# Whisper-6/DynamicTreeAttn

Measured on AMD Instinct MI355X. Metric: tree-attn fwd+bwd tokens/sec, Qwen3-0.6B tau2-16k tries, higher is better.
Workload: dtype bf16

## Files before the change

### dynamictreeattn_amd/_lib.py

```python
from __future__ import annotations

import ctypes as C
import os

from .build import LIB

_lib = None
_i32, _i64, _f32, _vp = C.c_int32, C.c_int64, C.c_float, C.c_void_p

_PROTOS = {
    "dta_version": ([], C.c_int),
    "dta_take_pending_error": ([C.c_char_p, _i32], C.c_int),
    "dta_lcp_adjacent": ([_vp, _vp, _vp, _i32, _vp, _vp, _vp], C.c_int),
    "dta_leafize": ([_vp, _vp, _i32, _vp, _vp, _vp, _vp, _vp], C.c_int),
    "dta_preorder_meta": ([_vp] * 8 + [_i32, _i32] + [_vp] * 4 + [_vp], C.c_int),
    "dta_tree_attn_fwd": ([_vp] * 8 + [_i32] * 6 + [_i64] * 8 + [_f32, _i32] + [_vp, _i32, _f32, _vp], C.c_int),
    "dta_tree_attn_bwd": ([_vp] * 14 + [_i32] * 6 + [_i64] * 12 + [_f32, _i32, _i32, _i32] + [_vp, _i32, _vp, _i32, _vp]
                          + [_vp, _i32, _f32, _vp], C.c_int),
    "dta_window_lo": ([_vp] * 4 + [_i32, _i32, _i32, _vp, _vp], C.c_int),
    "dta_logprob_entropy_fwd": ([_vp] * 8 + [_i32, _i32, _i64, _f32, _i32, _f32, _vp], C.c_int),
    "dta_logprob_entropy_shard_stats": ([_vp] * 6 + [_i32, _i32, _i64, _f32, _i32, _f32, _vp], C.c_int),
    "dta_logprob_entropy_bwd": ([_vp] * 10 + [_i32, _i32, _i64, _i64, _f32, _i32, _f32, _vp], C.c_int),
    "dta_rmsnorm_fwd": ([_vp] * 6 + [_i32, _i32, _f32, _f32, _i32, _vp], C.c_int),
    "dta_rmsnorm_bwd_blocks": ([_i32], C.c_int),
    "dta_rmsnorm_bwd": ([_vp] * 7 + [_i32, _i32, _f32, _i32, _vp], C.c_int),
    "dta_layernorm_fwd": ([_vp] * 8 + [_i32, _i32, _f32, _i32, _vp], C.c_int),
    "dta_layernorm_bwd_blocks": ([_i32], C.c_int),
    "dta_layernorm_bwd": ([_vp] * 8 + [_i32, _i32, _i32, _vp], C.c_int),
    "dta_qk_norm_rope_fwd": ([_vp] * 5 + [_i32, _i32, _i32, _i64, _f32, _i32, _vp], C.c_int),
    "dta_qk_norm_rope_bwd_blocks": ([_i64], C.c_int),
    "dta_qk_norm_rope_bwd": ([_vp] * 7 + [_i32, _i32, _i32, _i64, _i64, _i64, _i64, _i32, _vp], C.c_int),
    "dta_rope_partial_fwd": ([_vp] * 3 + [_i32] * 5 + [_i64, _i32, _vp], C.c_int),
    "dta_rope_partial_bwd": ([_vp] * 3 + [_i32] * 5 + [_i64, _i64, _i64, _i32, _vp], C.c_int),
    "dta_wide_qk_norm_rope_fwd": ([_vp] * 5 + [_i32, _i32, _i32, _i64, _f32, _i32, _vp], C.c_int),
    "dta_wide_qk_norm_rope_bwd_blocks": ([_i32], C.c_int),
    "dta_wide_qk_norm_rope_bwd": ([_vp] * 7 + [_i32, _i32, _i32, _i64, _i64, _i64, _i64, _i32, _vp], C.c_int),
    "dta_rmsnorm_add_fwd": ([_vp] * 6 + [_i32, _i32, _f32, _i32, _vp], C.c_int),
    "dta_swiglu_fwd": ([_vp] * 3 + [_i64, _i32, _i64, _i32, _vp], C.c_int),
    "dta_swiglu_bwd": ([_vp] * 5 + [_i64, _i32, _i64, _i64, _i32, _vp], C.c_int),
    "dta_geglu_fwd": ([_vp] * 3 + [_i64, _i32, _i64, _i32, _vp], C.c_int),
    "dta_geglu_bwd": ([_vp] * 5 + [_i64, _i32, _i64, _i64, _i32, _vp], C.c_int),
    "dta_transpose": ([_vp, _vp, _i64, _i64, _i64, _i64, _i32, _vp], C.c_int),
    "dta_sum_slabs": ([_vp, _i64, _i64, _i64, _vp, _vp, _i32, _vp], C.c_int),
    "dta_moe_router_fwd": ([_vp] * 4 + [_i32] * 5 + [_vp], C.c_int),
    "dta_moe_router_bwd": ([_vp] * 5 + [_i32] * 5 + [_vp], C.c_int),
    "dta_moe_permute_workspace": ([_i32, _i32], C.c_int),
    "dta_moe_tile_bound": ([_i32, _i32], C.c_int),
    "dta_moe_permute": ([_vp, _i32, _i32, _i32] + [_vp] * 5 + [_vp], C.c_int),
    "dta_moe_grouped_gemm": ([_i32] + [_vp] * 7 + [_i32] * 5 + [_vp], C.c_int),
    "dta_moe_combine_fwd": ([_vp] * 4 + [_i32] * 4 + [_vp], C.c_int),
    "dta_moe_combine_bwd": ([_vp] * 6 + [_i32] * 4 + [_vp], C.c_int),
    "dta_lora_down": ([_vp, _i64, _vp, _i64, _vp, _i64, _vp, _i32, _i32, _i32, _i32, _vp], C.c_int),
    "dta_lora_wgrad_slabs": ([_i32, _i32], C.c_int),
    "dta_lora_wgrad": ([_vp, _i64, _vp, _i64, _vp, _vp, _i32, _i32, _i32, _i32, _vp], C.c_int),
    "dta_policy_loss_blocks": ([_i32], C.c_int),
    "dta_policy_loss": ([_vp] * 10 + [_i32] + [_vp] * 5 + [_i32, _i32] + [_f32] * 4 + [_i32, _f32, _i32, _f32, _vp], C.c_int),
    "dta_policy_loss_seq_blocks": ([_i32, _i32], C.c_int),
    "dta_policy_loss_seq": ([_vp] * 14 + [_i32] + [_vp] * 6 + [_i32] * 4 + [_f32] * 4 + [_i32, _f32, _i32, _f32, _vp], C.c_int),
    "dta_preference_loss_blocks": ([_i32, _i32, _i32], C.c_int),
    "dta_preference_loss": ([_vp] * 21 + [_i32] * 6 + [_f32] * 3 + [_i32, _i32, _f32, _f32, _vp], C.c_int),
}
EXPORTS = tuple(_PROTOS)
_ERR = {-1: "DTA_EINVAL", -2: "DTA_EUNSUPPORTED", -3: "DTA_EALIGN", -4: "DTA_ELAUNCH", -5: "DTA_EPRIOR"}


def _hip_runtimes_mapped():
    try:
        with open("/proc/self/maps") as f:
            return sorted({line.split()[-1] for line in f if "libamdhip64" in line})
    except OSError:
        return []


def lib():
    global _lib
    if _lib is None:
        if not os.path.exists(LIB):
            raise RuntimeError(f"{LIB} is missing: run `python -m dynamictreeattn_amd.build` (hipcc, gfx950). "
                               "There is no CPU fallback for the hot path.")
        import torch
        l = C.CDLL(LIB)
        rts = _hip_runtimes_mapped()
        if len(rts) > 1:
            raise RuntimeError("more than one libamdhip64 is mapped into this process: " + ", ".join(rts) +
                               " — libdta_mi355x.so must resolve to the HIP runtime torch ships")
        for name, (args, res) in _PROTOS.items():
            fn = getattr(l, name)
            fn.argtypes, fn.restype = args, res
        _lib = l
    return _lib


def check(status: int, what: str):
    if status == 0:
        return
    if status == -5:
        buf = C.create_string_buffer(256)
        code = lib().dta_take_pending_error(buf, 256)
        raise RuntimeError(f"{what}: not launched, a HIP error was already pending on this thread: {buf.value.decode() or code} "
                           f"(hipError {code}; now cleared — after an asynchronous kernel fault the GPU context stays unusable)")
    raise RuntimeError(f"{what} failed: {_ERR.get(status, status)}")


def ptr(t):
    return None if t is None else t.data_ptr()
```

### dynamictreeattn_amd/csrc/elementwise_kernels.hip

```cpp
#include <hip/hip_runtime.h>
#include <stdint.h>
#include "dta_common.h"
#include "dta_device.h"

#ifndef DTA_EW_NT
#define DTA_EW_NT 1
#endif
#if DTA_EW_NT
#define DTA_SAVED_LOAD(P) __builtin_nontemporal_load(P)
#else
#define DTA_SAVED_LOAD(P) (*(P))
#endif

namespace {


template <int DT, int NA, bool OFF = false>
__global__ __launch_bounds__(256) void rmsnorm_fwd_kernel(const void* __restrict__ x_, const void* __restrict__ delta_, const void* __restrict__ w_,
                                                          void* __restrict__ xout_, void* __restrict__ y_,
                                                          float* __restrict__ rstd, int R, int H, float eps, float w_off = 0.f) {
  using e = typename Ty<DT>::e; using v8 = typename Ty<DT>::v8;
  const int lane = threadIdx.x & 63, wave = threadIdx.x >> 6;
  const e* w = reinterpret_cast<const e*>(w_);
  const int nv = H >> 3;
// ... 491 lines not shown
}

template <int DT, int NA, int D, int WPT>
__global__ __launch_bounds__(256) void wide_qk_norm_rope_fwd_kernel(const void* __restrict__ x_, const void* __restrict__ w_, const float* __restrict__ cs,
                                                                    void* __restrict__ y_, float* __restrict__ rstd, int T, int n,
                                                                    int64_t x_st, float eps) {
  using e = typename Ty<DT>::e; using v8 = typename Ty<DT>::v8;
  constexpr int LPH = D / 8, L = 64 * WPT, TPB = 4 / WPT;
  __shared__ float slot[4];
  const int lane = WPT == 1 ? (threadIdx.x & 63) : threadIdx.x, sub = lane & (LPH - 1);
  const e* w = reinterpret_cast<const e*>(w_);
  const int nv = n >> 3;
  const int per_lane = (nv + L - 1) / L;
  for (int tok = blockIdx.x * TPB + (WPT == 1 ? (threadIdx.x >> 6) : 0); tok < T; tok += gridDim.x * TPB) {
    const e* x = reinterpret_cast<const e*>(x_) + (int64_t)tok * x_st;
    e* y = reinterpret_cast<e*>(y_) + (int64_t)tok * n;
    const float* c = cs + (int64_t)tok * D + 8 * (sub & (LPH / 2 - 1));
    float cj[8], sj[8];
#pragma unroll
    for (int j = 0; j < 8; ++j) { cj[j] = c[j]; sj[j] = sub < LPH / 2 ? -c[D / 2 + j] : c[D / 2 + j]; }
    v8 keep[NA];
    float ss = 0.f;
#pragma unroll
    for (int a = 0; a < NA; ++a) {
      const int i = lane + L * a;
      if (a < per_lane && i < nv) {
        const v8 v = *reinterpret_cast<const v8*>(x + 8 * i);
#pragma unroll
        for (int j = 0; j < 8; ++j) { const float f = (float)v[j]; ss = __builtin_fmaf(f, f, ss); }
        keep[a] = v;
      }
    }
    ss = token_sum<WPT>(ss, slot);
    const float r = __builtin_amdgcn_rsqf(ss / (float)n + eps);
    if (lane == 0) rstd[tok] = r;
#pragma unroll
    for (int a = 0; a < NA; ++a) {
      if (a < per_lane) {
        const int i = lane + L * a;
        const bool live = i < nv;
        float av[8];
        if (live) {
          const v8 wv = *reinterpret_cast<const v8*>(w + 8 * i);
#pragma unroll
          for (int j = 0; j < 8; ++j) av[j] = (float)(e)((float)wv[j] * ((float)keep[a][j] * r));
        } else {
#pragma unroll
          for (int j = 0; j < 8; ++j) av[j] = 0.f;
        }
        v8 o;
#pragma unroll
        for (int j = 0; j < 8; ++j) {
          const float other = __shfl_xor(av[j], LPH / 2);
          o[j] = (e)(av[j] * cj[j] + other * sj[j]);
        }
        if (live) *reinterpret_cast<v8*>(y + 8 * i) = o;
      }
    }
  }
}

template <int DT, int NA, int D, int WPT>
__global__ __launch_bounds__(256) void wide_qk_norm_rope_bwd_kernel(const void* __restrict__ x_, const void* __restrict__ w_, const float* __restrict__ cs,
                                                                    const void* dy_, const float* __restrict__ rstd, void* dx_,
                                                                    float* __restrict__ dw_part, int T, int n, int64_t x_st, int64_t dy_st_t,
                                                                    int64_t dy_st_h, int64_t dx_st) {
  using e = typename Ty<DT>::e; using v8 = typename Ty<DT>::v8;
  constexpr int LPH = D / 8, LSH = D == 128 ? 4 : 3, L = 64 * WPT, TPB = 4 / WPT;
  __shared__ float red[WPT == 1 ? 4 * 64 * 8 : 4];
  const int lane = WPT == 1 ? (threadIdx.x & 63) : threadIdx.x, wave = threadIdx.x >> 6, sub = lane & (LPH - 1);
  const e* w = reinterpret_cast<const e*>(w_);
  const int nv = n >> 3;
  const int per_lane = (nv + L - 1) / L;
  float acc[NA][8];
#pragma unroll
  for (int a = 0; a < NA; ++a)
#pragma unroll
    for (int j = 0; j < 8; ++j) acc[a][j] = 0.f;
  for (int tok = blockIdx.x * TPB + (WPT == 1 ? wave : 0); tok < T; tok += gridDim.x * TPB) {
    const e* x = reinterpret_cast<const e*>(x_) + (int64_t)tok * x_st;
    const e* dy = reinterpret_cast<const e*>(dy_) + (int64_t)tok * dy_st_t + 8 * sub;
    e* dx = reinterpret_cast<e*>(dx_) + (int64_t)tok * dx_st;
    const float* c = cs + (int64_t)tok * D + 8 * (sub & (LPH / 2 - 1));
    float cj[8], sj[8];
#pragma unroll
    for (int j = 0; j < 8; ++j) { cj[j] = c[j]; sj[j] = sub < LPH / 2 ? c[D / 2 + j] : -c[D / 2 + j]; }
    const float r = rstd[tok];
    float dot = 0.f;
    v8 kx[NA], kg[NA];
#pragma unroll
    for (int a = 0; a < NA; ++a) {
      if (a < per_lane) {
        const int i = lane + L * a;
        const bool live = i < nv;
        v8 v, g;
        if (live) { v = DTA_SAVED_LOAD(reinterpret_cast<const v8*>(x + 8 * i)); g = *reinterpret_cast<const v8*>(dy + (int64_t)(i >> LSH) * dy_st_h); }
        else {
#pragma unroll
          for (int j = 0; j < 8; ++j) { v[j] = (e)0.f; g[j] = (e)0.f; }
        }
        if (live) {
          const v8 wv = *reinterpret_cast<const v8*>(w + 8 * i);
#pragma unroll
          for (int j = 0; j < 8; ++j) {
            const float gj = (float)g[j];
            const float da = gj * cj[j] + __shfl_xor(gj, LPH / 2) * sj[j];
            const float t = (float)v[j] * r;
            dot = __builtin_fmaf(da * (float)wv[j], t, dot); acc[a][j] = __builtin_fmaf(da, t, acc[a][j]);
          }
        }
        kx[a] = v; kg[a] = g;
      }
    }
    dot = token_sum<WPT>(dot, red) / (float)n;
#pragma unroll
    for (int a = 0; a < NA; ++a) {
      if (a < per_lane) {
        const int i = lane + L * a;
        const bool live = i < nv;
        const v8 v = kx[a], g = kg[a];
        float da[8];
#pragma unroll
        for (int j = 0; j < 8; ++j) { const float gj = (float)g[j]; da[j] = gj * cj[j] + __shfl_xor(gj, LPH / 2) * sj[j]; }
        if (live) {
          const v8 wv = *reinterpret_cast<const v8*>(w + 8 * i);
          v8 o;
#pragma unroll
          for (int j = 0; j < 8; ++j) { const float t = (float)v[j] * r; o[j] = (e)(r * (da[j] * (float)wv[j] - t * dot)); }
          *reinterpret_cast<v8*>(dx + 8 * i) = o;
        }
      }
    }
  }
  if (!dw_part) return;
  float* out = dw_part + (int64_t)blockIdx.x * n;
  if constexpr (WPT == 4) {
#pragma unroll
    for (int a = 0; a < NA; ++a) {
      const int i = lane + L * a;
      if (a < per_lane && i < nv) {
#pragma unroll
        for (int j = 0; j < 8; ++j) out[8 * i + j] = acc[a][j];
      }
    }
  } else {
#pragma unroll
    for (int a = 0; a < NA; ++a) {
      if (a < per_lane) {
        __syncthreads();
#pragma unroll
        for (int j = 0; j < 8; ++j) red[(wave * 64 + lane) * 8 + j] = acc[a][j];
        __syncthreads();
        if (wave == 0) {
          const int i = lane + 64 * a;
          if (i < nv) {
#pragma unroll
            for (int j = 0; j < 8; ++j) out[8 * i + j] = red[lane * 8 + j] + red[(64 + lane) * 8 + j] + red[(128 + lane) * 8 + j] + red[(192 + lane) * 8 + j];
          }
        }
      }
    }
  }
}

template <int DT, int NA>
__global__ __launch_bounds__(256) void rmsnorm_add_fwd_kernel(const void* __restrict__ y_, const void* __restrict__ w_, const void* __restrict__ res_,
                                                              void* __restrict__ out_, void* __restrict__ yn_, float* __restrict__ rstd,
                                                              int R, int H, float eps) {
  using e = typename Ty<DT>::e; using v8 = typename Ty<DT>::v8;
  const int lane = threadIdx.x & 63, wave = threadIdx.x >> 6;
  const e* w = reinterpret_cast<const e*>(w_);
  const int nv = H >> 3;
  for (int row = blockIdx.x * 4 + wave; row < R; row += gridDim.x * 4) {
    const e* y = reinterpret_cast<const e*>(y_) + (int64_t)row * H;
    const e* res = reinterpret_cast<const e*>(res_) + (int64_t)row * H;
    e* out = reinterpret_cast<e*>(out_) + (int64_t)row * H;
    e* yn = yn_ ? reinterpret_cast<e*>(yn_) + (int64_t)row * H : nullptr;
    float ss = 0.f;
    auto finish = [&](int i, const v8& v, float r) {
      const v8 wv = *reinterpret_cast<const v8*>(w + 8 * i);
      const v8 rv = *reinterpret_cast<const v8*>(res + 8 * i);
      v8 n8, o;
#pragma unroll
      for (int j = 0; j < 8; ++j) { n8[j] = (e)((float)wv[j] * ((float)v[j] * r)); o[j] = (e)((float)rv[j] + (float)n8[j]); }
      if (yn) *reinterpret_cast<v8*>(yn + 8 * i) = n8;
      *reinterpret_cast<v8*>(out + 8 * i) = o;
    };
    if constexpr (NA > 0) {
      v8 keep[NA];
#pragma unroll
      for (int a = 0; a < NA; ++a) {
        const int i = lane + 64 * a;
        if (i < nv) {
          const v8 v = *reinterpret_cast<const v8*>(y + 8 * i);
#pragma unroll
          for (int j = 0; j < 8; ++j) { const float f = (float)v[j]; ss = __builtin_fmaf(f, f, ss); }
          keep[a] = v;
        }
      }
      ss = wave_sum(ss);
      const float r = __builtin_amdgcn_rsqf(ss / (float)H + eps);
      if (lane == 0) rstd[row] = r;
#pragma unroll
      for (int a = 0; a < NA; ++a) {
        const int i = lane + 64 * a;
        if (i < nv) finish(i, keep[a], r);
      }
    } else {
      for (int i = lane; i < nv; i += 64) {
        const v8 v = *reinterpret_cast<const v8*>(y + 8 * i);
#pragma unroll
        for (int j = 0; j < 8; ++j) { const float f = (float)v[j]; ss = __builtin_fmaf(f, f, ss); }
      }
      ss = wave_sum(ss);
      const float r = __builtin_amdgcn_rsqf(ss / (float)H + eps);
      if (lane == 0) rstd[row] = r;
      for (int i = lane; i < nv; i += 64) finish(i, *reinterpret_cast<const v8*>(y + 8 * i), r);
    }
  }
}

template <int DT>
__global__ __launch_bounds__(256) void swiglu_fwd_kernel(const void* __restrict__ g_, const void* __restrict__ u_, void* __restrict__ y_,
                                                         int64_t n8, int c8, int64_t ld) {
  using e = typename Ty<DT>::e; using v8 = typename Ty<DT>::v8;
  for (int64_t i = (int64_t)blockIdx.x * 256 + threadIdx.x; i < n8; i += (int64_t)gridDim.x * 256) {
    const int64_t row = i / c8; const int col = (int)(i - row * c8) * 8;
    const v8 g = *reinterpret_cast<const v8*>(reinterpret_cast<const e*>(g_) + row * ld + col);
    const v8 u = *reinterpret_cast<const v8*>(reinterpret_cast<const e*>(u_) + row * ld + col);
    v8 o;
#pragma unroll
    for (int j = 0; j < 8; ++j) { const float x = (float)g[j]; const e s = (e)(x / (1.f + __expf(-x))); o[j] = (e)((float)s * (float)u[j]); }
    reinterpret_cast<v8*>(y_)[i] = o;
  }
}

template <int DT>
__global__ __launch_bounds__(256) void swiglu_bwd_kernel(const void* __restrict__ g_, const void* __restrict__ u_, const void* __restrict__ dy_,
                                                         void* __restrict__ dg_, void* __restrict__ du_, int64_t n8, int c8, int64_t ld, int64_t ldg) {
  using e = typename Ty<DT>::e; using v8 = typename Ty<DT>::v8;
  for (int64_t i = (int64_t)blockIdx.x * 256 + threadIdx.x; i < n8; i += (int64_t)gridDim.x * 256) {
    const int64_t row = i / c8; const int col = (int)(i - row * c8) * 8;
    const v8 g = DTA_SAVED_LOAD(reinterpret_cast<const v8*>(reinterpret_cast<const e*>(g_) + row * ld + col));
    const v8 u = DTA_SAVED_LOAD(reinterpret_cast<const v8*>(reinterpret_cast<const e*>(u_) + row * ld + col));
    const v8 dy = reinterpret_cast<const v8*>(dy_)[i];
    v8 dg, du;
#pragma unroll
    for (int j = 0; j < 8; ++j) {
      const float x = (float)g[j], sg = 1.f / (1.f + __expf(-x)), d = (float)dy[j];
      du[j] = (e)(d * x * sg);
      dg[j] = (e)(d * (float)u[j] * sg * (1.f + x * (1.f - sg)));
    }
    *reinterpret_cast<v8*>(reinterpret_cast<e*>(dg_) + row * ldg + col) = dg;
    *reinterpret_cast<v8*>(reinterpret_cast<e*>(du_) + row * ldg + col) = du;
  }
}

__device__ __forceinline__ float gelu_gate(float x, float* dgelu) {
  constexpr float K0 = 0.7978845608028654f, K1 = 0.044715f;
  const float x2 = x * x;
  const float z2 = 2.f * K0 * x * __builtin_fmaf(K1, x2, 1.f);
  const float E = __expf(fminf(-z2, 80.f));
  const float s = 1.f / (1.f + E);
  if (dgelu) *dgelu = s + x * s * (E * s) * (2.f * K0 * __builtin_fmaf(3.f * K1, x2, 1.f));
  return x * s;
}

template <int DT>
__global__ __launch_bounds__(256) void geglu_fwd_kernel(const void* __restrict__ g_, const void* __restrict__ u_, void* __restrict__ y_,
                                                        int64_t n8, int c8, int64_t ld) {
  using e = typename Ty<DT>::e; using v8 = typename Ty<DT>::v8;
  for (int64_t i = (int64_t)blockIdx.x * 256 + threadIdx.x; i < n8; i += (int64_t)gridDim.x * 256) {
    const int64_t row = i / c8; const int col = (int)(i - row * c8) * 8;
    const v8 g = *reinterpret_cast<const v8*>(reinterpret_cast<const e*>(g_) + row * ld + col);
    const v8 u = *reinterpret_cast<const v8*>(reinterpret_cast<const e*>(u_) + row * ld + col);
    v8 o;
#pragma unroll
    for (int j = 0; j < 8; ++j) { const e s = (e)gelu_gate((float)g[j], nullptr); o[j] = (e)((float)s * (float)u[j]); }
    reinterpret_cast<v8*>(y_)[i] = o;
  }
}

template <int DT>
__global__ __launch_bounds__(256) void geglu_bwd_kernel(const void* __restrict__ g_, const void* __restrict__ u_, const void* __restrict__ dy_,
                                                        void* __restrict__ dg_, void* __restrict__ du_, int64_t n8, int c8, int64_t ld, int64_t ldg) {
  using e = typename Ty<DT>::e; using v8 = typename Ty<DT>::v8;
  for (int64_t i = (int64_t)blockIdx.x * 256 + threadIdx.x; i < n8; i += (int64_t)gridDim.x * 256) {
    const int64_t row = i / c8; const int col = (int)(i - row * c8) * 8;
    const v8 g = DTA_SAVED_LOAD(reinterpret_cast<const v8*>(reinterpret_cast<const e*>(g_) + row * ld + col));
    const v8 u = DTA_SAVED_LOAD(reinterpret_cast<const v8*>(reinterpret_cast<const e*>(u_) + row * ld + col));
    const v8 dy = reinterpret_cast<const v8*>(dy_)[i];
    v8 dg, du;
#pragma unroll
    for (int j = 0; j < 8; ++j) {
      float dgl; const float ge = gelu_gate((float)g[j], &dgl), d = (float)dy[j];
      du[j] = (e)(d * ge);
      dg[j] = (e)(d * (float)u[j] * dgl);
    }
    *reinterpret_cast<v8*>(reinterpret_cast<e*>(dg_) + row * ldg + col) = dg;
    *reinterpret_cast<v8*>(reinterpret_cast<e*>(du_) + row * ldg + col) = du;
  }
}

template <int ESZ>
__global__ __launch_bounds__(256) void transpose_kernel(const char* __restrict__ in, char* __restrict__ out, int64_t rows, int64_t cols, int64_t ld_in, int64_t ld_out) {
  constexpr int TS = 64;
  constexpr int WPR = ESZ == 2 ? TS / 2 : TS;
  constexpr int PITCH = WPR + 4;
  __shared__ __attribute__((aligned(16))) uint32_t tile[TS * PITCH];
  const int64_t r0 = (int64_t)blockIdx.y * TS, c0 = (int64_t)blockIdx.x * TS;
  const int tid = threadIdx.x;
  if (ESZ == 2) {
    const int rp = tid >> 3, ch = tid & 7, r = 2 * rp, c = 8 * ch;
    uint4 a = make_uint4(0, 0, 0, 0), b = make_uint4(0, 0, 0, 0);
    if (c0 + c < cols) {
      if (r0 + r < rows) a = *reinterpret_cast<const uint4*>(in + ((r0 + r) * ld_in + c0 + c) * 2);
      if (r0 + r + 1 < rows) b = *reinterpret_cast<const uint4*>(in + ((r0 + r + 1) * ld_in + c0 + c) * 2);
    }
    const uint32_t aw[4] = {a.x, a.y, a.z, a.w}, bw[4] = {b.x, b.y, b.z, b.w};
#pragma unroll
    for (int j = 0; j < 4; ++j) {
      tile[(c + 2 * j) * PITCH + rp] = (aw[j] & 0xffffu) | (bw[j] << 16);
      tile[(c + 2 * j + 1) * PITCH + rp] = (aw[j] >> 16) | (bw[j] & 0xffff0000u);
    }
    __syncthreads();
    for (int i = tid; i < TS * 8; i += 256) {
      const int oc = i >> 3, k = i & 7;
      if (c0 + oc < cols && r0 + 8 * k < rows)
        *reinterpret_cast<uint4*>(out + ((c0 + oc) * ld_out + r0 + 8 * k) * 2) = *reinterpret_cast<const uint4*>(&tile[oc * PITCH + 4 * k]);
    }
  } else {
    for (int i = tid; i < TS * 16; i += 256) {
      const int r = i >> 4, c = 4 * (i & 15);
      uint4 a = make_uint4(0, 0, 0, 0);
      if (r0 + r < rows && c0 + c < cols) a = *reinterpret_cast<const uint4*>(in + ((r0 + r) * ld_in + c0 + c) * 4);
      tile[(c + 0) * PITCH + r] = a.x; tile[(c + 1) * PITCH + r] = a.y; tile[(c + 2) * PITCH + r] = a.z; tile[(c + 3) * PITCH + r] = a.w;
    }
    __syncthreads();
    for (int i = tid; i < TS * 16; i += 256) {
      const int oc = i >> 4, k = i & 15;
      if (c0 + oc < cols && r0 + 4 * k < rows)
        *reinterpret_cast<uint4*>(out + ((c0 + oc) * ld_out + r0 + 4 * k) * 4) = *reinterpret_cast<const uint4*>(&tile[oc * PITCH + 4 * k]);
    }
  }
}

template <int DT>
__global__ __launch_bounds__(1024) void sum_slabs_tall_kernel(const float* __restrict__ part, int64_t slabs, int64_t n, int64_t stride,
                                                              const float* __restrict__ extra, void* __restrict__ out_) {
  using e = typename Ty<DT>::e;
  __shared__ float red[16 * 64];
  const int lane = threadIdx.x & 63, wave = threadIdx.x >> 6;
  const int64_t col = (int64_t)blockIdx.x * 64 + lane;
  float acc[8];
#pragma unroll
  for (int u = 0; u < 8; ++u) acc[u] = 0.f;
  if (col < n) {
    int64_t s = wave;
    for (; s + 16 * 7 < slabs; s += 16 * 8) {
#pragma unroll
      for (int u = 0; u < 8; ++u) acc[u] += part[(s + 16 * u) * stride + col];
    }
    for (; s < slabs; s += 16) acc[0] += part[s * stride + col];
  }
  red[wave * 64 + lane] = ((acc[0] + acc[1]) + (acc[2] + acc[3])) + ((acc[4] + acc[5]) + (acc[6] + acc[7]));
  __syncthreads();
  if (wave == 0 && col < n) {
    float t = extra ? extra[col] : 0.f;
#pragma unroll
    for (int w = 0; w < 16; ++w) t += red[w * 64 + lane];
    reinterpret_cast<e*>(out_)[col] = (e)t;
  }
}
template <int DT>
__global__ __launch_bounds__(256) void sum_slabs_flat_kernel(const float* __restrict__ part, int slabs, int64_t n4, int64_t stride,
                                                             const float* __restrict__ extra, void* __restrict__ out_) {
  using e = typename Ty<DT>::e;
  typedef float f4 __attribute__((ext_vector_type(4)));
  typedef e e4 __attribute__((ext_vector_type(4)));
  for (int64_t i = (int64_t)blockIdx.x * 256 + threadIdx.x; i < n4; i += (int64_t)gridDim.x * 256) {
    f4 t = extra ? *reinterpret_cast<const f4*>(extra + 4 * i) : f4{0.f, 0.f, 0.f, 0.f};
    for (int s2 = 0; s2 < slabs; ++s2) t += *reinterpret_cast<const f4*>(part + s2 * stride + 4 * i);
    e4 o;
#pragma unroll
    for (int j = 0; j < 4; ++j) o[j] = (e)t[j];
    *reinterpret_cast<e4*>(reinterpret_cast<e*>(out_) + 4 * i) = o;
  }
}

template <int N> using Int = std::integral_constant<int, N>;

template <int WIDE, class F> inline void rms_form(int H, float w_offset, F&& f) {
  auto by_h = [&](auto off) {
    if (H <= 1024) f(Int<2>{}, off);
    else if (H <= 2048) f(Int<4>{}, off);
    else if (H <= 4096) f(Int<8>{}, off);
    else f(Int<WIDE>{}, off);
  };
  if (w_offset != 0.f) by_h(std::true_type{}); else by_h(std::false_type{});
}

template <class F> inline void qk_form(int NH, int head_dim, F&& f) {
  if (head_dim == 64) { if (NH % 4 == 0) f(Int<4>{}, Int<64>{}); else f(Int<1>{}, Int<64>{}); }
  else if (NH % 4 == 0) f(Int<4>{}, Int<128>{}); else f(Int<1>{}, Int<128>{});
}

template <class F> inline void wide_qk_form(int64_t n, int head_dim, F&& f) {
  auto by_n = [&](auto d) {
    if (n <= 1024) f(Int<2>{}, d, Int<1>{});
    else if (n <= 2048) f(Int<4>{}, d, Int<1>{});
    else if (n <= 4096) f(Int<2>{}, d, Int<4>{});
    else f(Int<4>{}, d, Int<4>{});
  };
  if (head_dim == 64) by_n(Int<64>{}); else by_n(Int<128>{});
}

template <class K>
int glu_fwd(const void* gate, const void* up, void* y, int64_t rows, int32_t cols, int64_t ld, int32_t dtype, void* stream, K kernel_of) {
  if (!gate || !up || !y || rows <= 0 || cols <= 0 || ld < cols) return DTA_EINVAL;
  if (!row_dtype_ok(dtype) || cols % 8 || ld % 8) return DTA_EUNSUPPORTED;
  if (!aligned16(gate) || !aligned16(up) || !aligned16(y)) return DTA_EALIGN;
  DTA_REFUSE_IF_PRIOR_ERROR();
  const int64_t n8 = rows * (cols / 8);
  dta_storage_type(dtype, [&](auto dt) {
    hipLaunchKernelGGL(kernel_of(dt), dim3(row_blocks(n8, 256, 4096)), dim3(256), 0, static_cast<hipStream_t>(stream), gate, up, y, n8, cols / 8, ld);
  });
  return DTA_LAUNCH_STATUS();
}

template <class K>
int glu_bwd(const void* gate, const void* up, const void* dy, void* dgate, void* dup, int64_t rows, int32_t cols, int64_t ld, int64_t ld_grad,
            int32_t dtype, void* stream, K kernel_of) {
  if (!gate || !up || !dy || !dgate || !dup || rows <= 0 || cols <= 0 || ld < cols || ld_grad < cols) return DTA_EINVAL;
  if (!row_dtype_ok(dtype) || cols % 8 || ld % 8 || ld_grad % 8) return DTA_EUNSUPPORTED;
  if (!aligned16(gate) || !aligned16(up) || !aligned16(dy) || !aligned16(dgate) || !aligned16(dup)) return DTA_EALIGN;
  DTA_REFUSE_IF_PRIOR_ERROR();
  const int64_t n8 = rows * (cols / 8);
  dta_storage_type(dtype, [&](auto dt) {
    hipLaunchKernelGGL(kernel_of(dt), dim3(row_blocks(n8, 256, 4096)), dim3(256), 0, static_cast<hipStream_t>(stream), gate, up, dy, dgate, dup, n8,
                       cols / 8, ld, ld_grad);
  });
  return DTA_LAUNCH_STATUS();
}

}

extern "C" int dta_rmsnorm_fwd(const void* x, const void* delta, const void* w, void* x_out, void* y, float* rstd,
                               int32_t R, int32_t H, float eps, float w_offset, int32_t dtype, void* stream) {
  if (!x || !w || !y || !rstd || R <= 0 || H <= 0 || ((delta != nullptr) != (x_out != nullptr)) || w_offset != w_offset) return DTA_EINVAL;
  if (!row_dtype_ok(dtype) || H % 8) return DTA_EUNSUPPORTED;
  if (!aligned16(x) || !aligned16(w) || !aligned16(y) || (delta && (!aligned16(delta) || !aligned16(x_out)))) return DTA_EALIGN;
  hipStream_t st_ = static_cast<hipStream_t>(stream);
  DTA_REFUSE_IF_PRIOR_ERROR();
  const dim3 grid(row_blocks(R, 4, 8192)), block(256);
  rms_form<0>(H, w_offset, [&](auto na, auto off) {
    dta_storage_type(dtype, [&](auto dt) {
      hipLaunchKernelGGL((rmsnorm_fwd_kernel<decltype(dt)::value, decltype(na)::value, decltype(off)::value>), grid, block, 0, st_,
                         x, delta, w, x_out, y, rstd, R, H, eps, w_offset);
    });
  });
  return DTA_LAUNCH_STATUS();
}

extern "C" int dta_rmsnorm_bwd_blocks(int32_t R) { return row_blocks(R, 4, 2048); }
extern "C" int dta_rmsnorm_bwd(const void* x, const void* w, const void* dy, const void* dres, const float* rstd, void* dx, float* dw_partial,
                               int32_t R, int32_t H, float w_offset, int32_t dtype, void* stream) {
  if (!x || !w || !dy || !rstd || !dx || R <= 0 || H <= 0 || w_offset != w_offset) return DTA_EINVAL;
  if (!row_dtype_ok(dtype) || H % 8 || H > 8192) return DTA_EUNSUPPORTED;
  if (!aligned16(x) || !aligned16(w) || !aligned16(dy) || !aligned16(dx) || (dres && !aligned16(dres))) return DTA_EALIGN;
  hipStream_t st_ = static_cast<hipStream_t>(stream);
  DTA_REFUSE_IF_PRIOR_ERROR();
  const dim3 grid(row_blocks(R, 4, 2048)), block(256);
  rms_form<16>(H, w_offset, [&](auto na, auto off) {
    dta_storage_type(dtype, [&](auto dt) {
      hipLaunchKernelGGL((rmsnorm_bwd_kernel<decltype(dt)::value, decltype(na)::value, decltype(off)::value>), grid, block, 0, st_,
                         x, w, dy, dres, rstd, dx, dw_partial, R, H, w_offset);
    });
  });
  return DTA_LAUNCH_STATUS();
}

namespace {
template <class F> inline void ln_form(int H, F&& f) {
  if (H <= 1024) f(Int<2>{}); else if (H <= 2048) f(Int<4>{}); else if (H <= 4096) f(Int<8>{}); else f(Int<16>{});
}
}

extern "C" int dta_layernorm_fwd(const void* x, const void* delta_a, const void* delta_b, const void* w, void* x_out, void* y,
                                 float* mean, float* rstd, int32_t R, int32_t H, float eps, int32_t dtype, void* stream) {
  if (!x || !w || !y || !mean || !rstd || R <= 0 || H <= 0 || (delta_b && !delta_a) || ((delta_a != nullptr) != (x_out != nullptr)) || eps != eps)
    return DTA_EINVAL;
  if (!row_dtype_ok(dtype) || H % 8 || H > 8192) return DTA_EUNSUPPORTED;
  if (!aligned16(x) || !aligned16(w) || !aligned16(y) || (delta_a && (!aligned16(delta_a) || !aligned16(x_out))) || (delta_b && !aligned16(delta_b)))
    return DTA_EALIGN;
  hipStream_t st_ = static_cast<hipStream_t>(stream);
  DTA_REFUSE_IF_PRIOR_ERROR();
  const dim3 grid(row_blocks(R, 4, 8192)), block(256);
  ln_form(H, [&](auto na) {
    dta_storage_type(dtype, [&](auto dt) {
      hipLaunchKernelGGL((layernorm_fwd_kernel<decltype(dt)::value, decltype(na)::value>), grid, block, 0, st_,
                         x, delta_a, delta_b, w, x_out, y, mean, rstd, R, H, eps);
    });
  });
  return DTA_LAUNCH_STATUS();
}

extern "C" int dta_layernorm_bwd_blocks(int32_t R) { return row_blocks(R, 4, 2048); }
extern "C" int dta_layernorm_bwd(const void* x, const void* w, const void* dy, const void* dres, const float* mean, const float* rstd,
                                 void* dx, float* dw_partial, int32_t R, int32_t H, int32_t dtype, void* stream) {
  if (!x || !w || !dy || !mean || !rstd || !dx || R <= 0 || H <= 0) return DTA_EINVAL;
  if (!row_dtype_ok(dtype) || H % 8 || H > 8192) return DTA_EUNSUPPORTED;
  if (!aligned16(x) || !aligned16(w) || !aligned16(dy) || !aligned16(dx) || (dres && !aligned16(dres))) return DTA_EALIGN;
  hipStream_t st_ = static_cast<hipStream_t>(stream);
  DTA_REFUSE_IF_PRIOR_ERROR();
  const dim3 grid(row_blocks(R, 4, 2048)), block(256);
  ln_form(H, [&](auto na) {
    dta_storage_type(dtype, [&](auto dt) {
      hipLaunchKernelGGL((layernorm_bwd_kernel<decltype(dt)::value, decltype(na)::value>), grid, block, 0, st_,
                         x, w, dy, dres, mean, rstd, dx, dw_partial, R, H);
    });
  });
  return DTA_LAUNCH_STATUS();
}

extern "C" int dta_qk_norm_rope_fwd(const void* x, const void* w, const float* cos_sin, void* y, float* rstd,
                                    int32_t T, int32_t NH, int32_t head_dim, int64_t x_stride_t, float eps, int32_t dtype, void* stream) {
  if (!x || !cos_sin || !y || T <= 0 || NH <= 0 || (w && !rstd)) return DTA_EINVAL;
  if (!row_dtype_ok(dtype) || (head_dim != 128 && head_dim != 64)) return DTA_EUNSUPPORTED;
  if (!aligned16(x) || !aligned16(y) || (w && !aligned16(w)) || x_stride_t % 8) return DTA_EALIGN;
  hipStream_t st_ = static_cast<hipStream_t>(stream);
  DTA_REFUSE_IF_PRIOR_ERROR();
  qk_form(NH, head_dim, [&](auto hpl, auto d) {
    constexpr int HPL = decltype(hpl)::value, D = decltype(d)::value, UPB = 4 * (64 / (D / 8));
    const int64_t n = (int64_t)T * (NH / HPL);
    const dim3 grid((unsigned)((n + UPB - 1) / UPB)), block(256);
    dta_storage_type(dtype, [&](auto dt) {
      hipLaunchKernelGGL((qk_norm_rope_fwd_kernel<decltype(dt)::value, HPL, D>), grid, block, 0, st_, x, w, cos_sin, y, rstd, n, NH, x_stride_t, eps);
    });
  });
  return DTA_LAUNCH_STATUS();
}

extern "C" int dta_qk_norm_rope_bwd_blocks(int64_t n_heads_total) { return row_blocks(n_heads_total, 16, 1024); }
extern "C" int dta_qk_norm_rope_bwd(const void* x, const void* w, const float* cos_sin, const void* dy, const float* rstd,
                                    void* dx, float* dw_partial, int32_t T, int32_t NH, int32_t head_dim,
                                    int64_t x_stride_t, int64_t dy_stride_t, int64_t dy_stride_h, int64_t dx_stride_t, int32_t dtype, void* stream) {
  if (!cos_sin || !dy || !dx || T <= 0 || NH <= 0 || (w && (!x || !rstd))) return DTA_EINVAL;
  if (!row_dtype_ok(dtype) || (head_dim != 128 && head_dim != 64)) return DTA_EUNSUPPORTED;
  if (!aligned16(dy) || !aligned16(dx) || (w && (!aligned16(w) || !aligned16(x))) || x_stride_t % 8 || dy_stride_t % 8 || dy_stride_h % 8 || dx_stride_t % 8) return DTA_EALIGN;
  if (dx_stride_t < (int64_t)NH * head_dim) return DTA_EINVAL;
  hipStream_t st_ = static_cast<hipStream_t>(stream);
  DTA_REFUSE_IF_PRIOR_ERROR();
  const dim3 grid(row_blocks((int64_t)T * NH, 16, 1024)), block(256);
  qk_form(NH, head_dim, [&](auto hpl, auto d) {
    constexpr int HPL = decltype(hpl)::value, D = decltype(d)::value;
    const int64_t n = (int64_t)T * (NH / HPL);
    dta_storage_type(dtype, [&](auto dt) {
      hipLaunchKernelGGL((qk_norm_rope_bwd_kernel<decltype(dt)::value, HPL, D>), grid, block, 0, st_, x, w, cos_sin, dy, rstd, dx, dw_partial, n, NH,
                         x_stride_t, dy_stride_t, dy_stride_h, dx_stride_t);
    });
  });
  return DTA_LAUNCH_STATUS();
}

namespace {
int rope_partial(const void* in, const float* cos_sin, void* out, int32_t T, int32_t NH, int32_t head_dim, int32_t rotary_dim, int32_t pairing,
                 int64_t in_st_t, int64_t in_st_h, int64_t out_st_t, float sgn, int grid_cap, int32_t dtype, void* stream) {
  if (!in || !cos_sin || !out || T <= 0 || NH <= 0 || rotary_dim <= 0 || (pairing != 0 && pairing != 1)) return DTA_EINVAL;
  if (!row_dtype_ok(dtype) || (head_dim != 128 && head_dim != 64) || rotary_dim > head_dim || rotary_dim % (pairing == 0 ? 16 : 8)) return DTA_EUNSUPPORTED;
  if (!aligned16(in) || !aligned16(out) || !aligned16(cos_sin) || in_st_t % 8 || in_st_h % 8 || out_st_t % 8) return DTA_EALIGN;
  if (in_st_t < 0 || in_st_h < head_dim || out_st_t < (int64_t)NH * head_dim) return DTA_EINVAL;
  hipStream_t st_ = static_cast<hipStream_t>(stream);
  DTA_REFUSE_IF_PRIOR_ERROR();
  qk_form(NH, head_dim, [&](auto hpl, auto d) {
    constexpr int HPL = decltype(hpl)::value, D = decltype(d)::value, UPB = 4 * (64 / (D / 8));
    const int64_t n = (int64_t)T * (NH / HPL);
    const dim3 grid(grid_cap ? (unsigned)row_blocks((int64_t)T * NH, 16, grid_cap) : ceil_blocks(n, UPB)), block(256);
    auto launch = [&](auto dt, auto pair, auto one_pass) {
      hipLaunchKernelGGL((rope_partial_kernel<decltype(dt)::value, HPL, D, decltype(pair)::value, decltype(one_pass)::value>), grid, block, 0, st_,
                         in, cos_sin, out, n, NH, rotary_dim, in_st_t, in_st_h, out_st_t, sgn);
    };
    dta_storage_type(dtype, [&](auto dt) {
      if (grid_cap) { if (pairing == 0) launch(dt, Int<0>{}, std::false_type{}); else launch(dt, Int<1>{}, std::false_type{}); }
      else if (pairing == 0) launch(dt, Int<0>{}, std::true_type{}); else launch(dt, Int<1>{}, std::true_type{});
    });
  });
  return DTA_LAUNCH_STATUS();
}
}

extern "C" int dta_rope_partial_fwd(const void* x, const float* cos_sin, void* y, int32_t T, int32_t NH, int32_t head_dim, int32_t rotary_dim,
                                    int32_t pairing, int64_t x_stride_t, int32_t dtype, void* stream) {
  return rope_partial(x, cos_sin, y, T, NH, head_dim, rotary_dim, pairing, x_stride_t, head_dim, (int64_t)NH * head_dim, 1.f, 0, dtype, stream);
}

extern "C" int dta_rope_partial_bwd(const float* cos_sin, const void* dy, void* dx, int32_t T, int32_t NH, int32_t head_dim, int32_t rotary_dim,
                                    int32_t pairing, int64_t dy_stride_t, int64_t dy_stride_h, int64_t dx_stride_t, int32_t dtype, void* stream) {
  return rope_partial(dy, cos_sin, dx, T, NH, head_dim, rotary_dim, pairing, dy_stride_t, dy_stride_h, dx_stride_t, -1.f, 1024, dtype, stream);
}

extern "C" int dta_wide_qk_norm_rope_fwd(const void* x, const void* w, const float* cos_sin, void* y, float* rstd,
                                         int32_t T, int32_t NH, int32_t head_dim, int64_t x_stride_t, float eps, int32_t dtype, void* stream) {
  if (!x || !w || !cos_sin || !y || !rstd || T <= 0 || NH <= 0 || eps != eps) return DTA_EINVAL;
  if (!row_dtype_ok(dtype) || (head_dim != 128 && head_dim != 64) || (int64_t)NH * head_dim > 8192) return DTA_EUNSUPPORTED;
  if (!aligned16(x) || !aligned16(w) || !aligned16(y) || x_stride_t % 8) return DTA_EALIGN;
  const int n = NH * head_dim;
  if (x_stride_t < n) return DTA_EINVAL;
  hipStream_t st_ = static_cast<hipStream_t>(stream);
  DTA_REFUSE_IF_PRIOR_ERROR();
  const dim3 grid(row_blocks(T, 4, 8192)), block(256);
  wide_qk_form(n, head_dim, [&](auto na, auto d, auto wpt) {
    dta_storage_type(dtype, [&](auto dt) {
      hipLaunchKernelGGL((wide_qk_norm_rope_fwd_kernel<decltype(dt)::value, decltype(na)::value, decltype(d)::value, decltype(wpt)::value>), grid, block, 0, st_,
                         x, w, cos_sin, y, rstd, T, n, x_stride_t, eps);
    });
  });
  return DTA_LAUNCH_STATUS();
}

extern "C" int dta_wide_qk_norm_rope_bwd_blocks(int32_t T) { return row_blocks(T, 4, 2048); }
extern "C" int dta_wide_qk_norm_rope_bwd(const void* x, const void* w, const float* cos_sin, const void* dy, const float* rstd,
                                         void* dx, float* dw_partial, int32_t T, int32_t NH, int32_t head_dim,
                                         int64_t x_stride_t, int64_t dy_stride_t, int64_t dy_stride_h, int64_t dx_stride_t, int32_t dtype, void* stream) {
  if (!x || !w || !cos_sin || !dy || !rstd || !dx || T <= 0 || NH <= 0) return DTA_EINVAL;
  if (!row_dtype_ok(dtype) || (head_dim != 128 && head_dim != 64) || (int64_t)NH * head_dim > 8192) return DTA_EUNSUPPORTED;
  if (!aligned16(x) || !aligned16(w) || !aligned16(dy) || !aligned16(dx) || x_stride_t % 8 || dy_stride_t % 8 || dy_stride_h % 8 || dx_stride_t % 8)
    return DTA_EALIGN;
  const int n = NH * head_dim;
  if (x_stride_t < n || dx_stride_t < n) return DTA_EINVAL;
  hipStream_t st_ = static_cast<hipStream_t>(stream);
  DTA_REFUSE_IF_PRIOR_ERROR();
  const dim3 grid(row_blocks(T, 4, 2048)), block(256);
  wide_qk_form(n, head_dim, [&](auto na, auto d, auto wpt) {
    dta_storage_type(dtype, [&](auto dt) {
      hipLaunchKernelGGL((wide_qk_norm_rope_bwd_kernel<decltype(dt)::value, decltype(na)::value, decltype(d)::value, decltype(wpt)::value>), grid, block, 0, st_,
                         x, w, cos_sin, dy, rstd, dx, dw_partial, T, n, x_stride_t, dy_stride_t, dy_stride_h, dx_stride_t);
    });
  });
  return DTA_LAUNCH_STATUS();
}

extern "C" int dta_rmsnorm_add_fwd(const void* y, const void* w, const void* res, void* out, void* yn, float* rstd,
                                   int32_t R, int32_t H, float eps, int32_t dtype, void* stream) {
  if (!y || !w || !res || !out || !rstd || R <= 0 || H <= 0 || eps != eps) return DTA_EINVAL;
  if (!row_dtype_ok(dtype) || H % 8) return DTA_EUNSUPPORTED;
  if (!aligned16(y) || !aligned16(w) || !aligned16(res) || !aligned16(out) || (yn && !aligned16(yn))) return DTA_EALIGN;
  hipStream_t st_ = static_cast<hipStream_t>(stream);
  DTA_REFUSE_IF_PRIOR_ERROR();
  const dim3 grid(row_blocks(R, 4, 8192)), block(256);
  rms_form<0>(H, 0.f, [&](auto na, auto) {
    dta_storage_type(dtype, [&](auto dt) {
      hipLaunchKernelGGL((rmsnorm_add_fwd_kernel<decltype(dt)::value, decltype(na)::value>), grid, block, 0, st_, y, w, res, out, yn, rstd, R, H, eps);
    });
  });
  return DTA_LAUNCH_STATUS();
}

extern "C" int dta_swiglu_fwd(const void* gate, const void* up, void* y, int64_t rows, int32_t cols, int64_t ld, int32_t dtype, void* stream) {
  return glu_fwd(gate, up, y, rows, cols, ld, dtype, stream, [](auto dt) { return swiglu_fwd_kernel<decltype(dt)::value>; });
}
extern "C" int dta_geglu_fwd(const void* gate, const void* up, void* y, int64_t rows, int32_t cols, int64_t ld, int32_t dtype, void* stream) {
  return glu_fwd(gate, up, y, rows, cols, ld, dtype, stream, [](auto dt) { return geglu_fwd_kernel<decltype(dt)::value>; });
}
extern "C" int dta_geglu_bwd(const void* gate, const void* up, const void* dy, void* dgate, void* dup,
                             int64_t rows, int32_t cols, int64_t ld, int64_t ld_grad, int32_t dtype, void* stream) {
  return glu_bwd(gate, up, dy, dgate, dup, rows, cols, ld, ld_grad, dtype, stream, [](auto dt) { return geglu_bwd_kernel<decltype(dt)::value>; });
}
extern "C" int dta_swiglu_bwd(const void* gate, const void* up, const void* dy, void* dgate, void* dup,
                              int64_t rows, int32_t cols, int64_t ld, int64_t ld_grad, int32_t dtype, void* stream) {
  return glu_bwd(gate, up, dy, dgate, dup, rows, cols, ld, ld_grad, dtype, stream, [](auto dt) { return swiglu_bwd_kernel<decltype(dt)::value>; });
}

extern "C" int dta_transpose(const void* in, void* out, int64_t rows, int64_t cols, int64_t ld_in, int64_t ld_out, int32_t elem_size, void* stream) {
  if (!in || !out || rows <= 0 || cols <= 0 || ld_in < cols || ld_out < rows) return DTA_EINVAL;
  if (elem_size != 2 && elem_size != 4) return DTA_EUNSUPPORTED;
  const int V = 16 / elem_size;
  if (rows % V || cols % V || ld_in % V || ld_out % V) return DTA_EUNSUPPORTED;
  if (!aligned16(in) || !aligned16(out)) return DTA_EALIGN;
  hipStream_t st_ = static_cast<hipStream_t>(stream);
  DTA_REFUSE_IF_PRIOR_ERROR();
  const dim3 grid((unsigned)((cols + 63) / 64), (unsigned)((rows + 63) / 64)), block(256);
  if (grid.y > 65535) return DTA_EUNSUPPORTED;
  if (elem_size == 2) hipLaunchKernelGGL(transpose_kernel<2>, grid, block, 0, st_, (const char*)in, (char*)out, rows, cols, ld_in, ld_out);
  else hipLaunchKernelGGL(transpose_kernel<4>, grid, block, 0, st_, (const char*)in, (char*)out, rows, cols, ld_in, ld_out);
  return DTA_LAUNCH_STATUS();
}

extern "C" int dta_sum_slabs(const float* part, int64_t slabs, int64_t n, int64_t slab_stride, const float* extra, void* out, int32_t out_dtype,
                             void* stream) {
  if (!part || !out || slabs <= 0 || n <= 0 || slab_stride < n) return DTA_EINVAL;
  if (!row_dtype_ok(out_dtype)) return DTA_EUNSUPPORTED;
  hipStream_t st_ = static_cast<hipStream_t>(stream);
  DTA_REFUSE_IF_PRIOR_ERROR();
  const bool flat = slabs <= 16 && n % 4 == 0 && slab_stride % 4 == 0 && aligned16(part) && aligned16(out) && (!extra || aligned16(extra));
  if (flat) {
    const dim3 grid(row_blocks(n / 4, 256, 8192)), block(256);
    dta_storage_type(out_dtype, [&](auto dt) {
      hipLaunchKernelGGL(sum_slabs_flat_kernel<decltype(dt)::value>, grid, block, 0, st_, part, (int)slabs, n / 4, slab_stride, extra, out);
    });
  } else {
    if ((n + 63) / 64 > 0x7fffffff) return DTA_EUNSUPPORTED;
    const dim3 grid((unsigned)((n + 63) / 64)), block(1024);
    dta_storage_type(out_dtype, [&](auto dt) {
      hipLaunchKernelGGL(sum_slabs_tall_kernel<decltype(dt)::value>, grid, block, 0, st_, part, slabs, n, slab_stride, extra, out);
    });
  }
  return DTA_LAUNCH_STATUS();
}
```

### dynamictreeattn_amd/dense.py

```python
from __future__ import annotations

from typing import List

import torch

from . import ops
from .model import ensure_supported, final_softcap_of, head_weight, is_longrope, logit_scale_of, longrope_boundary, packed_hidden_states
from .tree_training_engine import packed_logprob_entropy


def _one(model, ids: torch.Tensor, want_entropy: bool, checkpoint_layers: bool):
    n = ids.numel()
    depth = torch.arange(n, device=ids.device, dtype=torch.int32)
    long = is_longrope(model.config) and n > longrope_boundary(model.config)
    h = packed_hidden_states(model, ids, depth, ops.stack_meta(0), checkpoint_layers, longrope_long=long)
    parent = depth.to(torch.long) - 1
    return packed_logprob_entropy(h, head_weight(model), ids, parent, want_entropy, softcap=final_softcap_of(model), logit_scale=logit_scale_of(model))


@torch.no_grad()
def forward(model, token_seqs: List[torch.LongTensor], use_tqdm: bool = False) -> List[torch.Tensor]:
    out = []
    ensure_supported(model)
    with ops.weight_cache():
        for ids in token_seqs:
            lp, _ = _one(model, ids.to(model.device), False, False)
            out.append(lp[1:])
    return out


def backward(model, token_seqs: List[torch.LongTensor], attachs, loss_fn, act_ckpt: bool = False, use_tqdm: bool = False) -> float:
    total = 0.0
    ensure_supported(model)
    with ops.weight_cache():
        for ids, att in zip(token_seqs, attachs):
            lp, ent = _one(model, ids.to(model.device), True, act_ckpt)
            loss = loss_fn(lp[1:], ent, att)
            loss.backward()
            total += loss.item()
    return total
```

### dynamictreeattn_amd/model.py

```python
from __future__ import annotations

import weakref
from types import SimpleNamespace

import torch
import torch.nn as nn
import torch.nn.functional as F

from . import lora, ops


class _Norm(nn.Module):
    def __init__(self, n):
        super().__init__()
        self.weight = nn.Parameter(torch.ones(n))


class _Lin(nn.Module):
    def __init__(self, i, o):
        super().__init__()
        self.weight = nn.Parameter(torch.empty(o, i))


class _Attn(nn.Module):
# ... 113 lines not shown
def is_phi3(config) -> bool:
    return getattr(config, "model_type", None) == "phi3"


def is_glm4(config) -> bool:
    return getattr(config, "model_type", None) == "glm4"


def _head_dim(c) -> int:
    return getattr(c, "head_dim", None) or c.hidden_size // c.num_attention_heads


def rotary_dim(config) -> int:
    rp = getattr(config, "rope_parameters", None) or getattr(config, "rope_scaling", None) or {}
    prf = rp.get("partial_rotary_factor") if isinstance(rp, dict) else None
    if prf is None:
        prf = getattr(config, "partial_rotary_factor", None)
    return int(_head_dim(config) * (1.0 if prf is None else float(prf)))


def rope_layer_types(c):
    if getattr(c, "model_type", None) != "olmo3":
        return None
    types = getattr(c, "layer_types", None)
    if not types:
        raise ValueError("config.layer_types is missing: an olmo3 configuration keeps its rope_parameters per layer type")
    return sorted(set(types))


def _rope_dict(c, layer_type=None) -> dict:
    rp = getattr(c, "rope_parameters", None) or getattr(c, "rope_scaling", None) or {}
    if not isinstance(rp, dict):
        raise ValueError(f"config.rope_parameters must be a dict, got {type(rp).__name__}")
    types = rope_layer_types(c)
    if types is not None:
        if sorted(map(str, rp)) != types or not all(isinstance(v, dict) for v in rp.values()):
            raise ValueError(f"config.rope_parameters of an olmo3 configuration must be nested per layer type with exactly the keys "
                             f"{', '.join(types)} (config.layer_types); got {', '.join(map(str, rp)) or 'nothing'}")
        if layer_type not in rp:
            raise ValueError(f"config.rope_parameters is nested per layer type ({', '.join(types)}): name one of them, got {layer_type!r}")
        rp = rp[layer_type]
    elif rp and all(isinstance(v, dict) for v in rp.values()):
        raise ValueError(f"config.rope_parameters is nested per layer type ({', '.join(map(str, rp))}): one RoPE table per model is supported")
    rp = dict(rp)
    rp["rope_type"] = rp.get("rope_type", rp.get("type")) or "default"
    if rp.get("rope_theta") is None:
        theta = getattr(c, "rope_theta", None)
        rp["rope_theta"] = 1e6 if theta is None else theta
    if getattr(c, "original_max_position_embeddings", None) is not None:
        rp["original_max_position_embeddings"] = c.original_max_position_embeddings
    return rp


_ROPE: dict = {}


def is_longrope(c) -> bool:
    return is_phi3(c) and _rope_dict(c)["rope_type"] == "longrope"


def longrope_boundary(c) -> int:
    return int(_rope_dict(c)["original_max_position_embeddings"])


def rope_of(c, layer_type=None, long=False):
    rp = _rope_dict(c, layer_type)
    D = rotary_dim(c) if is_phi3(c) or is_glm4(c) else _head_dim(c)
    max_pos = getattr(c, "max_position_embeddings", None)
    longrope = is_phi3(c) and rp["rope_type"] == "longrope"
    key = (D, max_pos, bool(long) and longrope, tuple(sorted((k, repr(v)) for k, v in rp.items())))
    hit = _ROPE.get(key)
    if hit is None:
        hit = _ROPE[key] = ops.longrope_inv_freq(D, rp, max_pos, bool(long)) if longrope else ops.rope_inv_freq(D, rp, max_pos)
    return hit


_SOFTCAP_SINK_FIELDS = ("attn_logit_softcapping", "final_logit_softcapping", "attn_softcap", "logit_softcap", "attention_sink",
                        "attention_sinks", "use_attention_sinks", "num_sink_tokens")


def is_gemma2(config) -> bool:
    return getattr(config, "model_type", None) == "gemma2"


def gemma2_arith(config):
    c = config
    return float(c.query_pre_attn_scalar) ** -0.5, float(getattr(c, "attn_logit_softcapping", None) or 0.0), \
        float(getattr(c, "final_logit_softcapping", None) or 0.0)


def final_softcap_of(model) -> float:
    return gemma2_arith(model.config)[2] if is_gemma2(model.config) else 0.0


def _check_gemma2(c) -> None:
    act = getattr(c, "hidden_activation", None)
    if act != "gelu_pytorch_tanh":
        raise ValueError(f"config.hidden_activation = {act!r} is not supported for gemma2: the MLP kernel computes gelu_pytorch_tanh(gate) * up")
    D = _head_dim(c)
    if D not in (64, 128):
        raise ValueError(f"config.head_dim = {D} is not supported: the attention kernels cover head_dim 64 and 128 (Gemma-2-27B; the 2B / 9B use 256)")
    qs = getattr(c, "query_pre_attn_scalar", None)
    if qs is None or not float(qs) > 0:
        raise ValueError(f"config.query_pre_attn_scalar = {qs!r} is not supported: gemma2 attention scales by query_pre_attn_scalar ** -0.5")
    for f in ("attn_logit_softcapping", "final_logit_softcapping"):
        v = getattr(c, f, None)
        if v is not None and not (0.0 <= float(v) < float("inf")):
            raise ValueError(f"config.{f} = {v!r} is not supported: a soft-cap is a finite number >= 0 (None or 0: no cap)")


def _check_olmo(c) -> None:
    D = _head_dim(c)
    if D not in (64, 128):
        raise ValueError(f"config.head_dim = {D} is not supported for {c.model_type}: the projection-wide q/k norm kernels cover head_dim 64 and 128")
    for f in ("num_attention_heads", "num_key_value_heads"):
        if getattr(c, f) * D > 8192:
            raise ValueError(f"config.{f} * head_dim = {getattr(c, f)} * {D} is not supported: the projection-wide q/k norm kernels hold "
                             f"one row of at most 8192 elements")


def _check_cohere(c) -> None:
    mt, D, H = c.model_type, _head_dim(c), c.hidden_size
    if D not in (64, 128):
        raise ValueError(f"config.head_dim = {D} is not supported for {mt}: the attention and RoPE kernels cover head_dim 64 and 128")
    if H % 8 or H > 8192:
        raise ValueError(f"config.hidden_size = {H} is not supported for {mt}: the LayerNorm kernel holds one row of a multiple of 8 and at "
                         f"most 8192 elements (Command-R+ and Command-A are wider)")
    if getattr(c, "use_qk_norm", False):
        raise ValueError(f"config.use_qk_norm = True is not supported for {mt} (Command-R+): there is no per-head LayerNorm kernel")
    ls = getattr(c, "logit_scale", None)
    if isinstance(ls, bool) or not isinstance(ls, (int, float)) or not 0.0 < float(ls) < float("inf"):
        raise ValueError(f"config.logit_scale = {ls!r} is not supported for {mt}: the head scales its logits by a finite number > 0")
    act = getattr(c, "hidden_act", None)
    if act != "silu":
        raise ValueError(f"config.hidden_act = {act!r} is not supported for {mt}: the MLP kernels compute silu(gate) * up")
    if mt == "cohere2":
        types = getattr(c, "layer_types", None)
        if not types or len(types) != c.num_hidden_layers:
            raise ValueError(f"config.layer_types has {len(types or [])} entries for {c.num_hidden_layers} layers: a cohere2 layer rotates "
                             f"(sliding_attention) or not (full_attention) by its type")
        for t in types:
            if t not in ("full_attention", "sliding_attention"):
                raise ValueError(f"config.layer_types entry {t!r} is not supported for cohere2 (full_attention / sliding_attention)")
        W = getattr(c, "sliding_window", None)
        if "sliding_attention" in types and not (isinstance(W, int) and not isinstance(W, bool) and W > 0):
            raise ValueError(f"config.sliding_window = {W!r} is not supported for cohere2: a sliding_attention layer needs its window")


def _check_partial_rope(c, training: bool) -> None:
    mt, D = c.model_type, _head_dim(c)
    if D not in (64, 128):
        raise ValueError(f"config.head_dim = {D} is not supported for {mt}: the attention and RoPE kernels cover head_dim 64 and 128"
                         + (" (Phi-3-mini and Phi-3.5-mini use 96)" if D == 96 else ""))
    R, step = rotary_dim(c), 16 if is_phi3(c) else 8
    if not 0 < R <= D or R % step:
        raise ValueError(f"config partial_rotary_factor gives a rotary dimension of {R} of head_dim {D}, which is not supported for {mt}: "
                         f"the {'half-split' if is_phi3(c) else 'interleaved'} RoPE kernel rotates a multiple of {step} elements, at most head_dim")
    rp = _rope_dict(c)
    if rp["rope_type"] == "longrope" and is_phi3(c):
        if rp.get("original_max_position_embeddings") is None:
            raise ValueError("config.original_max_position_embeddings is missing: longrope picks its factors by it")
        for f in ("short_factor", "long_factor"):
            v = rp.get(f)
            if not isinstance(v, (list, tuple)) or len(v) != R // 2:
                raise ValueError(f"config.rope_parameters[{f!r}] must be a list of {R // 2} numbers (rotary dimension {R}), got "
                                 f"{len(v) if isinstance(v, (list, tuple)) else v!r}")
    for f in ("resid_pdrop", "embd_pdrop"):
        if training and float(getattr(c, f, 0.0) or 0.0) > 0:
            raise ValueError(f"config.{f} = {getattr(c, f)} on a model in training mode is not supported (model.eval(), or set it to 0)")


def check_supported(config, training: bool = True) -> None:
    c = config
    gemma = is_gemma2(c)
    partial = is_phi3(c) or is_glm4(c)
    if partial:
        _check_partial_rope(c, training)
    if gemma:
        _check_gemma2(c)
    if getattr(c, "model_type", None) == "olmo":
        raise ValueError("config.model_type = 'olmo' (OLMo-1: LayerNorm without weights, clip_qkv) is not supported; olmo2 and olmo3 are")
    if is_olmo(c):
        _check_olmo(c)
    if is_cohere(c):
        _check_cohere(c)
    for lt in rope_layer_types(c) or [None]:
        rp = _rope_dict(c, lt)
        if rp["rope_type"] not in ops.ROPE_TYPES and not (is_phi3(c) and rp["rope_type"] == "longrope"):
            raise ValueError(f"config.rope_parameters['rope_type'] = {rp['rope_type']!r} is not supported ({' / '.join(ops.ROPE_TYPES)})")
        prf = rp.get("partial_rotary_factor", getattr(c, "partial_rotary_factor", None))
        if not partial and prf is not None and float(prf) != 1.0:
            raise ValueError(f"config partial_rotary_factor = {prf} is not supported: the rotary kernels rotate the whole head")
    act = getattr(c, "hidden_act", None)
    if not gemma and act is not None and act != "silu":
        raise ValueError(f"config.hidden_act = {act!r} is not supported: the MLP kernels compute silu(gate) * up")
    if training and float(getattr(c, "attention_dropout", 0.0) or 0.0) > 0:
        raise ValueError(f"config.attention_dropout = {c.attention_dropout} on a model in training mode is not supported (model.eval(), or set it to 0)")
    if float(getattr(c, "router_jitter_noise", 0.0) or 0.0) > 0:
        raise ValueError(f"config.router_jitter_noise = {c.router_jitter_noise} is not supported")
    for f in _SOFTCAP_SINK_FIELDS:
        if gemma and f in ("attn_logit_softcapping", "final_logit_softcapping"):
            continue
        if getattr(c, f, None):
            raise ValueError(f"config.{f} = {getattr(c, f)!r} is not supported: the attention kernels have neither soft-capping nor sinks")


_CHECKED = weakref.WeakKeyDictionary()


def _check_olmo_norms(model) -> None:
    c = model.config
    D = _head_dim(c)
    for l, layer in enumerate(model.model.layers):
        for name, heads in (("q_norm", c.num_attention_heads), ("k_norm", c.num_key_value_heads)):
            w = getattr(getattr(layer.self_attn, name, None), "weight", None)
            if w is None or w.numel() != heads * D:
                raise ValueError(f"model.layers.{l}.self_attn.{name}.weight has {None if w is None else w.numel()} elements: "
                                 f"{c.model_type} normalises the whole projection row of {heads} * {D}")


def ensure_supported(model) -> None:
    training = bool(getattr(model, "training", True))
    if hasattr(model, "named_modules"):
        lora.check_supported(model)
    if is_olmo(model.config) and hasattr(getattr(model, "model", None), "layers"):
        _check_olmo_norms(model)
    try:
        seen = _CHECKED.setdefault(model, set())
    except TypeError:
        return check_supported(model.config, training)
    if training not in seen:
        check_supported(model.config, training)
        seen.add(training)


def _cfg_of(model, longrope_long=False):
    c = model.config
    D = _head_dim(c)
    types = rope_layer_types(c)
    rope = (rope_of(c, long=True) if longrope_long else rope_of(c)) if types is None else [rope_of(c, t) for t in c.layer_types]
    eps = getattr(c, "layer_norm_eps", 1e-5) if is_cohere(c) else getattr(c, "rms_norm_eps", 1e-6)
    return c.num_attention_heads, c.num_key_value_heads, D, float(eps), rope


def _windows_of(model):
    c = model.config
    n = c.num_hidden_layers
    W = getattr(c, "sliding_window", None) or 0
    if getattr(c, "model_type", None) in ("mistral", "mixtral", "phi3"):
        return [int(W)] * n
    types = getattr(c, "layer_types", None)
    if types is not None:
        if len(types) != n:
            raise ValueError(f"config.layer_types has {len(types)} entries for {n} layers")
        bad = [t for t in types if t not in ("full_attention", "sliding_attention")]
        if bad:
            raise ValueError(f"unsupported attention layer type {bad[0]!r} (full_attention / sliding_attention)")
        sliding = [t == "sliding_attention" for t in types]
    else:
        first = getattr(c, "max_window_layers", n)
        sliding = [bool(getattr(c, "use_sliding_window", False)) and l >= (first if first is not None else n) for l in range(n)]
    return [int(W) if s_ else 0 for s_ in sliding]


def layer_metas(meta, windows, for_window=None):
    out, cache = [], {}
    for W in windows:
        if W <= 0 or meta is None:
            out.append(meta)
            continue
        if W not in cache:
            if for_window is not None:
                cache[W] = for_window(W)
            elif meta.subtree_end is None and meta.runs is None:
                cache[W] = ops.stack_meta(meta.q_offset, W)
            else:
                raise ValueError("a sliding-window layer needs its windowed meta (ops.window_meta); none was given")
        out.append(cache[W])
    return out


def _bias(*mods):
    bs = [getattr(m_, "bias", None) for m_ in mods]
    if bs[0] is None:
        return None
    return bs[0] if len(bs) == 1 else torch.cat(bs)


def _project(x, *mods):
    bases, ads = zip(*(lora.resolve(m_) for m_ in mods))
    w = bases[0].weight if len(bases) == 1 else ops.stack_rows(*(b_.weight for b_ in bases))
    bias = _bias(*bases)
    if not any(a_ is not None for a_ in ads):
        return ops.linear(x, w, bias)
    adapters, n0 = [], 0
    for b_, a_ in zip(bases, ads):
        n = b_.weight.shape[0]
        if a_ is not None:
            adapters.append((n0, n, *a_))
        n0 += n
    return ops.lora_linear(x, w, bias, adapters)


def _gemma2_layer_forward(layer, res, delta, cos_sin, attn, Hq, Hkv, D, eps):
    T = res.shape[0]
    a, m = layer.self_attn, layer.mlp
    res, h = ops.add_rms_norm(res, delta, layer.input_layernorm.weight, eps, 1.0)
    qkv = _project(h, a.q_proj, a.k_proj, a.v_proj).view(T, Hq + 2 * Hkv, D)
    q, k, v = ops.qkv_prep(qkv, None, None, cos_sin, eps, Hq, Hkv)
    o = attn(q, k, v)
    delta = ops.rms_norm(_project(o.reshape(T, Hq * D), a.o_proj), layer.post_attention_layernorm.weight, eps, 1.0)
    res, h = ops.add_rms_norm(res, delta, layer.pre_feedforward_layernorm.weight, eps, 1.0)
    act = ops.geglu_fused(_project(h, m.gate_proj, m.up_proj))
    return res, ops.rms_norm(_project(act, m.down_proj), layer.post_feedforward_layernorm.weight, eps, 1.0)


def _olmo_layer_forward(layer, res, delta, cos_sin, attn, Hq, Hkv, D, eps):
    T = res.shape[0]
    a, m = layer.self_attn, layer.mlp
    x = res if delta is None else res + delta
    qkv = _project(x, a.q_proj, a.k_proj, a.v_proj).view(T, Hq + 2 * Hkv, D)
    q, k, v = ops.qkv_prep_wide(qkv, a.q_norm.weight, a.k_norm.weight, cos_sin, eps, Hq, Hkv)
    o = attn(q, k, v)
    h = ops.rms_norm_add(x, _project(o.reshape(T, Hq * D), a.o_proj), layer.post_attention_layernorm.weight, eps)
    act = ops.swiglu_fused(_project(h, m.gate_proj, m.up_proj))
    return ops.rms_norm_add(h, _project(act, m.down_proj), layer.post_feedforward_layernorm.weight, eps), None


def _phi3_layer_forward(layer, res, delta, cos_sin, attn, Hq, Hkv, D, eps):
    T = res.shape[0]
    a, m = layer.self_attn, layer.mlp
    res, h = ops.add_rms_norm(res, delta, layer.input_layernorm.weight, eps)
    qkv = _project(h, a.qkv_proj).view(T, Hq + 2 * Hkv, D)
    if cos_sin.shape[1] < D:
        q, k, v = ops.qkv_prep_partial(qkv, cos_sin, Hq, Hkv, False)
    else:
        q, k, v = ops.qkv_prep(qkv, None, None, cos_sin, eps, Hq, Hkv)
    o = attn(q, k, v)
    res, h = ops.add_rms_norm(res, _project(o.reshape(T, Hq * D), a.o_proj), layer.post_attention_layernorm.weight, eps)
    act = ops.swiglu_fused(_project(h, m.gate_up_proj))
    return res, _project(act, m.down_proj)


def _glm4_layer_forward(layer, res, delta, cos_sin, attn, Hq, Hkv, D, eps):
    T = res.shape[0]
    a, m = layer.self_attn, layer.mlp
    res, h = ops.add_rms_norm(res, delta, layer.input_layernorm.weight, eps)
    qkv = _project(h, a.q_proj, a.k_proj, a.v_proj).view(T, Hq + 2 * Hkv, D)
    q, k, v = ops.qkv_prep_partial(qkv, cos_sin, Hq, Hkv, True)
    o = attn(q, k, v)
    delta = ops.rms_norm(_project(o.reshape(T, Hq * D), a.o_proj), layer.post_self_attn_layernorm.weight, eps)
    res, h = ops.add_rms_norm(res, delta, layer.post_attention_layernorm.weight, eps)
    act = ops.swiglu_fused(_project(h, m.gate_up_proj))
    return res, ops.rms_norm(_project(act, m.down_proj), layer.post_mlp_layernorm.weight, eps)


def _cohere_layer_forward(layer, res, delta_a, delta_b, cos_sin, attn, Hq, Hkv, D, eps):
    T = res.shape[0]
    a, m = layer.self_attn, layer.mlp
    res, h = ops.add_layer_norm(res, delta_a, delta_b, layer.input_layernorm.weight, eps)
    qkv = _project(h, a.q_proj, a.k_proj, a.v_proj).view(T, Hq + 2 * Hkv, D)
    q, k, v = ops.qkv_prep_nope(qkv, Hq, Hkv) if cos_sin is None else ops.qkv_prep_partial(qkv, cos_sin, Hq, Hkv, True)
    o = attn(q, k, v)
    act = ops.swiglu_fused(_project(h, m.gate_proj, m.up_proj))
    return res, _project(o.reshape(T, Hq * D), a.o_proj), _project(act, m.down_proj)


def _layer_forward(layer, res, delta, cos_sin, attn, Hq, Hkv, D, eps):
    T = res.shape[0]
    a = layer.self_attn
    res, h = ops.add_rms_norm(res, delta, layer.input_layernorm.weight, eps)
    qkv = _project(h, a.q_proj, a.k_proj, a.v_proj).view(T, Hq + 2 * Hkv, D)
    qn = getattr(a, "q_norm", None); kn = getattr(a, "k_norm", None)
    q, k, v = ops.qkv_prep(qkv, qn.weight if qn is not None else None, kn.weight if kn is not None else None, cos_sin, eps, Hq, Hkv)
    o = attn(q, k, v)
    attn_out = _project(o.reshape(T, Hq * D), a.o_proj)
    res, h = ops.add_rms_norm(res, attn_out, layer.post_attention_layernorm.weight, eps)
    m = layer.mlp
    if hasattr(m, "experts") and hasattr(m, "gate"):
        g = m.gate
        norm = getattr(g, "norm_topk_prob", None)
        if norm is None:
            if not hasattr(m, "jitter_noise"):
                raise AttributeError(f"{type(g).__name__} has no norm_topk_prob and {type(m).__name__} is not a Mixtral block")
            norm = True
        return res, ops.moe_mlp(h, g.weight, m.experts.gate_up_proj, m.experts.down_proj, g.top_k, norm)
    act = ops.swiglu_fused(_project(h, m.gate_proj, m.up_proj))
    return res, _project(act, m.down_proj)


class _ScaleRows(torch.autograd.Function):

    @staticmethod
    def forward(ctx, x, s):
        ctx.s = float(torch.tensor(s, dtype=x.dtype))
        return x * ctx.s

    @staticmethod
    def backward(ctx, g):
        return g * ctx.s, None


def attn_args_of(model):
    if not is_gemma2(model.config):
        return {}
    scale, cap, _ = gemma2_arith(model.config)
    return {"scale": scale, "softcap": cap}


class _LayerRecompute(torch.autograd.Function):

    @staticmethod
    def forward(ctx, fn, keep_attn, res, *deltas):
        ctx.fn, ctx.has_delta = fn, tuple(d is not None for d in deltas)
        items = []
        with torch.no_grad():
            if keep_attn:
                with ops.AttentionTape("record", items):
                    out = fn(res, *deltas)
            else:
                out = fn(res, *deltas)
        ctx.items = items
        ctx.save_for_backward(res, *(d for d in deltas if d is not None))
        return out

    @staticmethod
    def backward(ctx, g_res, *g_deltas):
        res, *kept = ctx.saved_tensors
        r = res.detach().requires_grad_(True)
        kept = iter(kept)
        ds = [next(kept).detach().requires_grad_(True) if has else None for has in ctx.has_delta]
        with torch.enable_grad():
            if ctx.items:
                with ops.AttentionTape("replay", ctx.items):
                    outs = ctx.fn(r, *ds)
            else:
                outs = ctx.fn(r, *ds)
        ctx.items = None
        live = [(o, g) for o, g in zip(outs, (g_res, *g_deltas)) if o is not None]
        torch.autograd.backward(tuple(o for o, _ in live), tuple(g for _, g in live))
        return (None, None, r.grad, *(d.grad if d is not None else None for d in ds))


def packed_hidden_states(model, tokens: torch.Tensor, depth: torch.Tensor, meta, checkpoint_layers: bool = False,
                         attn_keep_bytes: int = 0, attn_of_layer=None, full_layers=0, kept_out=None, embed=None,
                         meta_for_window=None, longrope_long: bool = False) -> torch.Tensor:
    Hq, Hkv, D, eps, rope = _cfg_of(model, longrope_long)
    metas = layer_metas(meta, _windows_of(model), meta_for_window) if attn_of_layer is None else None
    body = model.model
    gemma = is_gemma2(model.config)
    cohere = is_cohere(model.config)
    layer_fwd = (_gemma2_layer_forward if gemma else _olmo_layer_forward if is_olmo(model.config) else _phi3_layer_forward if is_phi3(model.config)
                 else _glm4_layer_forward if is_glm4(model.config) else _cohere_layer_forward if cohere else _layer_forward)
    R = rotary_dim(model.config) if is_phi3(model.config) or is_glm4(model.config) else D
    akw = attn_args_of(model)
    res = embed(tokens) if embed is not None else F.embedding(tokens, body.embed_tokens.weight)
    deltas = (None, None) if cohere else (None,)
    if gemma:
        res = _ScaleRows.apply(res, float(model.config.hidden_size) ** 0.5)
    if isinstance(rope, list):
        tables = {id(r_): ops.rope_cos_sin(depth, D, r_) for r_ in {id(r_): r_ for r_ in rope}.values()}
        cos_sins = [tables[id(r_)] for r_ in rope]
    else:
        cos_sins = [ops.rope_cos_sin(depth, R, rope)] * len(body.layers)
    if cohere and model.config.model_type == "cohere2":
        cos_sins = [cs if t == "sliding_attention" else None for cs, t in zip(cos_sins, model.config.layer_types)]
    per_layer = tokens.shape[0] * Hq * (D * res.element_size() + 4)
    n_full = full_layers if isinstance(full_layers, int) else 1
    for li, layer in enumerate(body.layers):
        cos_sin = cos_sins[li]
        attn = attn_of_layer(li) if attn_of_layer is not None else (lambda m_: lambda q, k, v: ops.tree_attention(q, k, v, m_, **akw))(metas[li])
        if li == 0 and callable(full_layers) and checkpoint_layers and torch.is_grad_enabled() and res.is_cuda:
            m0 = torch.cuda.memory_allocated(res.device)
            res, *deltas = layer_fwd(layer, res, *deltas, cos_sin, attn, Hq, Hkv, D, eps)
            n_full = int(full_layers(torch.cuda.memory_allocated(res.device) - m0))
            continue
        if checkpoint_layers and li >= n_full and torch.is_grad_enabled() and (res.requires_grad or any(d is not None and d.requires_grad for d in deltas)):
            keep = attn_of_layer is None and attn_keep_bytes >= per_layer
            if keep:
                attn_keep_bytes -= per_layer
            fn = (lambda layer_, attn_, cs_: lambda r_, *d_: layer_fwd(layer_, r_, *d_, cs_, attn_, Hq, Hkv, D, eps))(layer, attn, cos_sin)
            res, *deltas = _LayerRecompute.apply(fn, keep, res, *deltas)
        else:
            res, *deltas = layer_fwd(layer, res, *deltas, cos_sin, attn, Hq, Hkv, D, eps)
    if kept_out is not None:
        kept_out.append(n_full if checkpoint_layers else len(body.layers))
    if cohere:
        return ops.add_layer_norm(res, *deltas, body.norm.weight, eps)[1]
    return ops.add_rms_norm(res, deltas[0], body.norm.weight, eps, *((1.0,) if gemma else ()))[1]


def head_weight(model) -> torch.Tensor:
    lm = getattr(model, "lm_head", None)
    return lm.weight if lm is not None else model.model.embed_tokens.weight
```

### dynamictreeattn_amd/ops.py

```python
from __future__ import annotations

import math
from dataclasses import dataclass
from typing import Optional

import numpy as np
import torch
import torch.nn.functional as F

from . import packing
from ._lib import check, lib, ptr

_DT = {torch.bfloat16: 0, torch.float16: 1, torch.float32: 2}


class _on:
    __slots__ = ("dev", "_guard")

    def __init__(self, *ts):
        dev = None
        for t in ts:
            if t is None:
                continue
            if not t.is_cuda:
# ... 110 lines not shown
    (qs, qh), (ks, kh), (vs, vh), (os_, oh) = _strides(q), _strides(k), _strides(v), _strides(out)
    _launch("dta_tree_attn_fwd", (q, k, v, meta.subtree_end, meta.runs, meta.win_lo),
            ptr(q), ptr(k), ptr(v), ptr(out), ptr(lse), ptr(meta.subtree_end), ptr(meta.run_ptr), ptr(meta.runs),
            Tq, Tk, meta.q_offset, Hq, Hkv, D, qs, qh, ks, kh, vs, vh, os_, oh, float(scale), _DT[q.dtype],
            ptr(meta.win_lo) if meta.window > 0 else None, int(meta.window), softcap, span="fwd")
    return out, lse, k, v


def attn_bwd_raw(q, k, v, out, dout, lse, meta: TreeAttnMeta, scale: float, dk=None, dv=None, accumulate=False, dq=None, softcap: float = 0.0):
    softcap = _cap_of(softcap)
    Tq, Hq, D = q.shape
    Tk, Hkv, _ = k.shape
    if dout.stride() != out.stride():
        dout = dout.contiguous(); out = out.contiguous()
    if dq is None:
        dq = torch.empty((Tq, Hq, D), dtype=q.dtype, device=q.device)
    if dk is None:
        dk = torch.empty((Tk, Hkv, D), dtype=q.dtype, device=q.device); dv = torch.empty_like(dk)
    delta = torch.empty((Hq, Tq), dtype=torch.float32, device=q.device)
    (qs, qh), (ks, kh), (vs, vh), (os_, oh), (dqs, dqh), (dks, dkh) = _strides(q), _strides(k), _strides(v), _strides(out), _strides(dq), _strides(dk)
    units, splits = meta.dkv_units, meta.dkv_splits
    n_units = units.shape[0] if units is not None else 0
    n_splits = splits.shape[0] if splits is not None else 0
    if q.dtype == torch.float32:
        units = splits = None; n_units = n_splits = 0
    ws = torch.empty((meta.n_slabs, Hkv, 2, packing.KTILE, D), dtype=torch.float32, device=q.device) if (units is not None and meta.n_slabs) else None

    def launch(which, span=None):
        _launch("dta_tree_attn_bwd", (q, k, v, out, dout, lse, dk, dv, meta.subtree_end, units, meta.win_lo),
                ptr(q), ptr(k), ptr(v), ptr(out), ptr(dout), ptr(lse), ptr(delta), ptr(dq), ptr(dk), ptr(dv),
                ptr(meta.subtree_end), ptr(meta.run_ptr), ptr(meta.runs), ptr(meta.ktile_qend),
                Tq, Tk, meta.q_offset, Hq, Hkv, D, qs, qh, ks, kh, vs, vh, os_, oh, dqs, dqh, dks, dkh,
                float(scale), _DT[q.dtype], int(accumulate), which,
                ptr(units), n_units, ptr(splits) if n_splits else None, n_splits, ptr(ws),
                ptr(meta.win_lo) if meta.window > 0 else None, int(meta.window), softcap, span=span)
    if KernelTimer.active is None:
        launch(3)
    else:
        launch(1, "bwd_dq"); launch(2 | 8, "bwd_dkv")
        if n_splits:
            launch(4, "bwd_dkv_finalize")
    return dq, dk, dv


class AttentionTape:
    current = None

    def __init__(self, mode: str, items=None):
        assert mode in ("record", "replay")
        self.mode, self.items, self.pos = mode, ([] if items is None else items), 0

    def __enter__(self):
        self._prev, AttentionTape.current = AttentionTape.current, self
        return self

    def __exit__(self, *exc):
        AttentionTape.current = self._prev
        return False


class _TreeAttention(torch.autograd.Function):
    @staticmethod
    def forward(ctx, q, k, v, meta: TreeAttnMeta, scale: float, softcap: float = 0.0):
        tape = AttentionTape.current
        if tape is not None and tape.mode == "replay" and tape.pos < len(tape.items):
            out, lse, *cap = tape.items[tape.pos]; tape.pos += 1
            if out.shape != q.shape:
                raise RuntimeError("attention replay: recorded output does not match the recomputed query")
            if cap and cap[0] != softcap:
                raise RuntimeError(f"attention replay: recorded under softcap {cap[0]}, replayed under {softcap}")
        else:
            out, lse, k, v = attn_fwd_raw(q, k, v, meta, scale, softcap)
            if tape is not None and tape.mode == "record":
                tape.items.append((out, lse, softcap))
        ctx.save_for_backward(q, k, v, out, lse)
        ctx.meta, ctx.scale, ctx.softcap = meta, scale, softcap
        return out

    @staticmethod
    def backward(ctx, dout):
        q, k, v, out, lse = ctx.saved_tensors
        Hq, Hkv = q.shape[1], k.shape[1]
        if q.shape[0] == k.shape[0]:
            fused = torch.empty((q.shape[0], Hq + 2 * Hkv, q.shape[2]), dtype=q.dtype, device=q.device)
            dq, dk, dv = fused[:, :Hq], fused[:, Hq:Hq + Hkv], fused[:, Hq + Hkv:]
            attn_bwd_raw(q, k, v, out, dout, lse, ctx.meta, ctx.scale, dk=dk, dv=dv, dq=dq, softcap=ctx.softcap)
        else:
            dq, dk, dv = attn_bwd_raw(q, k, v, out, dout, lse, ctx.meta, ctx.scale, softcap=ctx.softcap)
        return dq, dk, dv, None, None, None


class _StackAttention(torch.autograd.Function):

    @staticmethod
    def forward(ctx, q, k_new, v_new, kst, vst, gk, gv, start, scale, window, softcap=0.0):
        B = q.shape[0]
        end = start + B
        kst[start:end].copy_(k_new); vst[start:end].copy_(v_new)
        meta = stack_meta(start, window)
        out, lse, _, _ = attn_fwd_raw(q, kst[:end], vst[:end], meta, scale, softcap)
        ctx.save_for_backward(q, out, lse)
        ctx.stacks, ctx.meta, ctx.scale, ctx.span, ctx.softcap = (kst, vst, gk, gv), meta, scale, (start, end), softcap
        return out

    @staticmethod
    def backward(ctx, dout):
        q, out, lse = ctx.saved_tensors
        kst, vst, gk, gv = ctx.stacks
        start, end = ctx.span
        dq, _, _ = attn_bwd_raw(q, kst[:end], vst[:end], out, dout, lse, ctx.meta, ctx.scale, dk=gk[:end], dv=gv[:end], accumulate=2,
                                softcap=ctx.softcap)
        return dq, gk[start:end].to(q.dtype), gv[start:end].to(q.dtype), None, None, None, None, None, None, None, None


def stack_attention(q, k_new, v_new, kst, vst, gk, gv, start: int, scale: Optional[float] = None, window: int = 0, softcap: float = 0.0):
    if q.dtype not in _DT:
        raise TypeError("stack_attention supports bf16 / f16 / f32 (got %s)" % q.dtype)
    scale = q.shape[-1] ** -0.5 if scale is None else scale
    return _StackAttention.apply(q, k_new, v_new, kst, vst, gk, gv, start, scale, int(window), _cap_of(softcap))


def tree_attention(q: torch.Tensor, k: torch.Tensor, v: torch.Tensor, meta: TreeAttnMeta, scale: Optional[float] = None,
                   softcap: float = 0.0) -> torch.Tensor:
    if q.dtype not in _DT:
        raise TypeError("tree_attention supports bf16 / f16 / f32 (got %s)" % q.dtype)
    scale = q.shape[-1] ** -0.5 if scale is None else scale
    return _TreeAttention.apply(q, k, v, meta, scale, _cap_of(softcap))


def stack_meta(start: int, window: int = 0) -> TreeAttnMeta:
    return TreeAttnMeta(T=0, subtree_end=None, run_ptr=None, runs=None, ktile_qend=None, q_offset=start, window=max(int(window), 0))


def attach_dkv_units(meta: TreeAttnMeta, Hkv: int) -> TreeAttnMeta:
    kq = meta.ktile_qend.cpu().numpy()
    units, splits, n_slabs = packing.plan_dkv_units(kq, meta.T, meta.T, meta.q_offset, Hkv)
    dev = meta.ktile_qend.device
    meta.dkv_units = torch.from_numpy(units).to(dev).contiguous()
    meta.dkv_splits = torch.from_numpy(splits).to(dev).contiguous() if splits.shape[0] else None
    meta.n_slabs = n_slabs
    return meta


def meta_from_plan(plan: packing.SegmentPlan, subtree_end: torch.Tensor, device, Hkv: int = 8) -> TreeAttnMeta:
    rp, runs = packing.plan_qtile_runs(plan)
    meta = TreeAttnMeta(T=plan.T, subtree_end=subtree_end,
                        run_ptr=torch.from_numpy(rp).to(device), runs=torch.from_numpy(runs).to(device).contiguous(),
                        ktile_qend=ktile_qend_from(subtree_end))
    return attach_dkv_units(meta, Hkv)


def window_lo_device(depth: torch.Tensor, seg_off: torch.Tensor, seg_depth0: torch.Tensor, parent_of_seg: torch.Tensor,
                     window: int) -> torch.Tensor:
    T, M = depth.numel(), parent_of_seg.numel()
    out = torch.empty(T, dtype=torch.int32, device=depth.device)
    _launch("dta_window_lo", (depth,), ptr(depth), ptr(seg_off), ptr(seg_depth0), ptr(parent_of_seg), M, T, int(window), ptr(out))
    return out


def window_meta(meta: TreeAttnMeta, plan: packing.SegmentPlan, depth: torch.Tensor, window: int, Hkv: int = 8, seg_tables=None) -> TreeAttnMeta:
    if window <= 0 or window > packing.max_depth(plan):
        return meta
    dev = depth.device
    up = lambda a: torch.from_numpy(np.ascontiguousarray(a, np.int32)).to(dev)
    if seg_tables is None:
        seg_tables = (up(plan.seg_off), up(plan.seg_depth0), up(plan.parent_of_seg))
    win_lo = window_lo_device(depth, *seg_tables, window)
    wl_host = packing.window_lo_host(plan, window)
    rp, runs = packing.plan_qtile_runs_window(plan, wl_host)
    kq = packing.ktile_qend_window(packing.ktile_qend_host(plan), wl_host)
    units, splits, n_slabs = packing.plan_dkv_units(kq, plan.T, plan.T, 0, Hkv)
    return TreeAttnMeta(T=plan.T, subtree_end=meta.subtree_end, run_ptr=up(rp), runs=up(runs).view(-1, 4), ktile_qend=up(kq),
                        dkv_units=up(units).view(-1, 4), dkv_splits=up(splits).view(-1, 4) if splits.shape[0] else None, n_slabs=n_slabs,
                        win_lo=win_lo, window=int(window))


def logprob_entropy_fwd_raw(logits, labels, want_entropy=True, temperature=1.0, extra_ptr=None, extra_labels=None, extra_out=None, softcap=0.0):
    R, V = logits.shape
    lse = torch.empty(R, dtype=torch.float32, device=logits.device)
    ent = torch.empty_like(lse) if want_entropy else None
    lp = torch.empty_like(lse) if labels is not None else None
    _launch("dta_logprob_entropy_fwd", (logits, labels, extra_ptr, extra_labels, extra_out),
            ptr(logits), ptr(labels), ptr(extra_ptr), ptr(extra_labels), ptr(lse), ptr(ent), ptr(lp), ptr(extra_out),
            R, V, logits.stride(0), float(temperature), _DT[logits.dtype], float(softcap), nbytes=R * V * logits.element_size())
    return lse, ent, lp


def logprob_entropy_bwd_raw(logits, labels, lse, ent, g_lp, g_ent, temperature=1.0, extra_ptr=None, extra_labels=None, g_extra=None, out=None,
                            softcap=0.0):
    R, V = logits.shape
    out = logits if out is None else out
    _launch("dta_logprob_entropy_bwd", (logits, out, labels, extra_ptr, extra_labels, lse, g_lp, g_extra, g_ent),
            ptr(logits), ptr(out), ptr(labels), ptr(extra_ptr), ptr(extra_labels), ptr(lse), ptr(ent), ptr(g_lp), ptr(g_extra), ptr(g_ent),
            R, V, logits.stride(0), out.stride(0), float(temperature), _DT[logits.dtype], float(softcap), nbytes=2 * R * V * logits.element_size())
    return out


def logprob_entropy_shard_stats_raw(logits, labels_local, temperature=1.0, extra_ptr=None, extra_labels=None, extra_out=None, softcap=0.0):
    R, V = logits.shape
    stats = torch.empty((R, 4), dtype=torch.float32, device=logits.device)
    _launch("dta_logprob_entropy_shard_stats", (logits, labels_local, extra_ptr, extra_labels, extra_out),
            ptr(logits), ptr(labels_local), ptr(extra_ptr), ptr(extra_labels), ptr(stats), ptr(extra_out),
            R, V, logits.stride(0), float(temperature), _DT[logits.dtype], float(softcap), nbytes=R * V * logits.element_size())
    return stats


_LN2 = 0.6931471805599453


def combine_shard_stats(stats, extra_sum, group):
    import torch.distributed as dist
    m = stats[:, 0].contiguous()
    M = m.clone()
    dist.all_reduce(M, op=dist.ReduceOp.MAX, group=group)
    f = torch.exp2(m - M)
    R = stats.shape[0]
    packed = torch.cat([stats[:, 1] * f, stats[:, 2] * f, stats[:, 3], extra_sum])
    dist.all_reduce(packed, op=dist.ReduceOp.SUM, group=group)
    S, Tt, picked, extra = packed[:R], packed[R:2 * R], packed[2 * R:3 * R], packed[3 * R:]
    lse = (M + torch.log2(S)) * _LN2
    ent = lse - (Tt / S) * _LN2
    return lse, ent, picked, extra


def local_labels(t, vocab_offset, V):
    return torch.where((t >= vocab_offset) & (t < vocab_offset + V), t - vocab_offset, torch.full_like(t, -1))


def _head_logits(h, W):
    V = W.shape[0]
    if V % 8 == 0:
        return torch.mm(h, W.t())
    buf = torch.empty((h.shape[0], (V + 7) // 8 * 8), dtype=h.dtype, device=h.device)
    return torch.mm(h, W.t(), out=buf[:, :V])


HEAD_WGRAD_FUSED_ACCUMULATE = False


class _HeadRows(torch.autograd.Function):

    @staticmethod
    def forward(ctx, h, W, next_tok, fork_ptr, fork_tok, fork_rows, fork_bounds, want_entropy, chunk, keep_bytes, tp_group, vocab_offset, softcap=0.0,
                temperature=1.0):
        T = h.shape[0]
        dev = h.device
        V = W.shape[0]
        F_ = fork_tok.numel()
        keep = T * V * h.element_size() <= keep_bytes
        step = T if keep else chunk
        lse = torch.empty(T, dtype=torch.float32, device=dev)
        ent = torch.empty(T, dtype=torch.float32, device=dev) if (want_entropy or tp_group is not None) else None
        lp_next = torch.empty(T, dtype=torch.float32, device=dev)
        lp_fork = torch.empty(F_, dtype=torch.float32, device=dev)
        if tp_group is not None:
            next_loc, fork_loc = local_labels(next_tok, vocab_offset, V), local_labels(fork_tok, vocab_offset, V)
        else:
            next_loc, fork_loc = next_tok, fork_tok
        xp = fork_ptr if F_ else None
        kept = None
        for ci, a in enumerate(range(0, T, step)):
            b = min(a + step, T)
            logits = _head_logits(h[a:b], W)
            if tp_group is None:
                l, e, p = logprob_entropy_fwd_raw(logits, next_loc[a:b], want_entropy, temperature,
                                                  xp[a:b + 1] if F_ else None, fork_loc if F_ else None, lp_fork if F_ else None, softcap)
            else:
                f0, f1 = (0, F_) if keep else (fork_bounds[ci], fork_bounds[ci + 1])
                stats = logprob_entropy_shard_stats_raw(logits, next_loc[a:b], temperature, xp[a:b + 1] if F_ else None, fork_loc if F_ else None,
                                                        lp_fork if F_ else None, softcap)
                l, e, picked, raw = combine_shard_stats(stats, lp_fork[f0:f1], tp_group)
                p = picked - l
                if f1 > f0:
                    lp_fork[f0:f1] = raw - l[fork_rows[f0:f1] - a]
            lse[a:b] = l; lp_next[a:b] = p
            if ent is not None:
                ent[a:b] = e
            if keep:
                kept = logits
        ctx.save_for_backward(h, W, next_loc, fork_loc, lse, ent if ent is not None else lse, xp if F_ else lse)
        ctx.kept, ctx.chunk, ctx.want_entropy, ctx.tp_group, ctx.has_forks, ctx.softcap = kept, chunk, want_entropy, tp_group, bool(F_), softcap
        ctx.temperature = temperature
        return lp_next, lp_fork, (ent if want_entropy else lse.new_zeros(0))

    @staticmethod
    def backward(ctx, g_next, g_fork, g_ent):
        h, W, next_loc, fork_loc, lse, ent, xp = ctx.saved_tensors
        T = h.shape[0]
        g_next = g_next.contiguous().float()
        g_ent = g_ent.contiguous().float() if ctx.want_entropy else None
        g_fork = g_fork.contiguous().float() if ctx.has_forks else None
        kept = ctx.kept
        step = T if kept is not None else ctx.chunk
        dh = torch.empty_like(h)
        need_w = ctx.needs_input_grad[1]
        dW = None if (kept is not None or not need_w) else torch.zeros(W.shape, dtype=torch.float32, device=W.device)
        pending = []
        for a in range(0, T, step):
            b = min(a + step, T)
            logits = kept if kept is not None else _head_logits(h[a:b], W)
            logprob_entropy_bwd_raw(logits, next_loc[a:b], lse[a:b], ent[a:b] if ctx.want_entropy else None, g_next[a:b],
                                    g_ent[a:b] if ctx.want_entropy else None, ctx.temperature,
                                    xp[a:b + 1] if ctx.has_forks else None, fork_loc if ctx.has_forks else None, g_fork, softcap=ctx.softcap)
            if W.dtype in (torch.bfloat16, torch.float16) and (b - a) >= 4096 and W.shape[0] % 8 == 0 and W.shape[1] % 8 == 0:
                torch.mm(logits, _TransposedWeights.get(W).t(), out=dh[a:b])
            else:
                torch.mm(logits, W, out=dh[a:b])
            if ctx.tp_group is not None:
                import torch.distributed as dist
                pending.append(dist.all_reduce(dh[a:b], op=dist.ReduceOp.SUM, group=ctx.tp_group, async_op=True))
            if not need_w:
                pass
            elif kept is not None:
                dW = torch.mm(logits.t(), h)
            elif HEAD_WGRAD_FUSED_ACCUMULATE:
                dW = torch.addmm(dW, logits.t(), h[a:b], out_dtype=torch.float32)
            else:
                dW += torch.mm(logits.t(), h[a:b])
        ctx.kept = None
        for w in pending:
            w.wait()
        return dh, (dW.to(W.dtype) if need_w else None), None, None, None, None, None, None, None, None, None, None, None, None


MAX_CAPPED_PICKS_PER_ROW = 2048


def lm_head_rows(h, W, next_tok, fork_ptr, fork_tok, fork_rows, fork_bounds, want_entropy, chunk, keep_bytes=None, tp_group=None, vocab_offset=0,
                 softcap: float = 0.0, max_picks_per_row: Optional[int] = None, temperature: float = 1.0):
    _require_cuda(h, W)
    temperature = float(temperature)
    if not (0.0 < temperature < float("inf")):
        raise ValueError(f"temperature must be a finite number > 0 (got {temperature!r})")
    softcap = _cap_of(softcap)
    if softcap > 0 and max_picks_per_row is not None and max_picks_per_row > MAX_CAPPED_PICKS_PER_ROW:
        raise ValueError(f"a row with {max_picks_per_row} fork picks exceeds the capped log-prob kernel's {MAX_CAPPED_PICKS_PER_ROW} per row")
    if keep_bytes is None:
        keep_bytes = free_hbm(h.device) // 4
    if tp_group is not None:
        import torch.distributed as dist
        ok = torch.tensor([1 if h.shape[0] * W.shape[0] * h.element_size() <= keep_bytes else 0], device=h.device, dtype=torch.int32)
        dist.all_reduce(ok, op=dist.ReduceOp.MIN, group=tp_group)
        keep_bytes = (1 << 62) if int(ok.item()) else 0
    lp_next, lp_fork, ent = _HeadRows.apply(h, W, next_tok, fork_ptr, fork_tok, fork_rows, fork_bounds, want_entropy, chunk, keep_bytes,
                                            tp_group, vocab_offset, softcap, temperature)
    return lp_next, lp_fork, (ent if want_entropy else None)


class _LogProbEntropyHIP(torch.autograd.Function):

    @staticmethod
    def forward(ctx, logits, labels, temperature, want_entropy):
        lse, ent, lp = logprob_entropy_fwd_raw(logits, labels, want_entropy, temperature)
        ctx.save_for_backward(logits, labels, lse, ent if ent is not None else lse)
        ctx.temperature, ctx.want_entropy = temperature, want_entropy
        return lp, (ent if want_entropy else lse.new_zeros(0))

    @staticmethod
    def backward(ctx, g_lp, g_ent):
        logits, labels, lse, ent = ctx.saved_tensors
        out = torch.empty_strided(logits.shape, logits.stride(), dtype=logits.dtype, device=logits.device)
        logprob_entropy_bwd_raw(logits, labels, lse, ent if ctx.want_entropy else None, g_lp.contiguous().float(),
                                g_ent.contiguous().float() if ctx.want_entropy else None, ctx.temperature, out=out)
        return out, None, None, None


class _ShardedLogProbEntropyHIP(torch.autograd.Function):

    @staticmethod
    def forward(ctx, logits, labels_local, temperature, want_entropy, group):
        stats = logprob_entropy_shard_stats_raw(logits, labels_local, temperature)
        lse, ent, picked, _ = combine_shard_stats(stats, stats.new_zeros(0), group)
        ctx.save_for_backward(logits, labels_local, lse, ent)
        ctx.temperature, ctx.want_entropy = temperature, want_entropy
        return picked - lse, (ent if want_entropy else lse.new_zeros(0))

    @staticmethod
    def backward(ctx, g_lp, g_ent):
        logits, labels_local, lse, ent = ctx.saved_tensors
        out = torch.empty_strided(logits.shape, logits.stride(), dtype=logits.dtype, device=logits.device)
        logprob_entropy_bwd_raw(logits, labels_local, lse, ent if ctx.want_entropy else None, g_lp.contiguous().float(),
                                g_ent.contiguous().float() if ctx.want_entropy else None, ctx.temperature, out=out)
        return out, None, None, None, None


def _rows_for_kernel(logits2d):
    if logits2d.stride(-1) != 1:
        logits2d = logits2d.contiguous()
    if logits2d.stride(0) % 8 or logits2d.data_ptr() % 32:
        R, V = logits2d.shape
        buf = torch.empty((R, (V + 7) // 8 * 8), dtype=logits2d.dtype, device=logits2d.device)
        view = buf[:, :V]
        view.copy_(logits2d)
        return view
    return logits2d


def logprob_entropy(logits2d, labels1d, temperature=1.0, want_entropy=True, tp_group=None):
    if logits2d.dtype not in _DT:
        raise TypeError("logprob_entropy supports bf16 / f16 / f32 logits (got %s)" % logits2d.dtype)
    x = _rows_for_kernel(logits2d)
    if tp_group is None:
        lp, ent = _LogProbEntropyHIP.apply(x, labels1d, float(temperature), want_entropy)
    else:
        import torch.distributed as dist
        V = x.shape[1]
        lab = local_labels(labels1d, dist.get_rank(tp_group) * V, V)
        lp, ent = _ShardedLogProbEntropyHIP.apply(x, lab, float(temperature), want_entropy, tp_group)
    return lp, (ent if want_entropy else None)


def _norm_bwd(entry, x2, w, dy, g_res, stats, tail, need_w):
    R, H = x2.shape
    dy2 = dy.contiguous().view(R, H)
    gr = g_res.contiguous().view(R, H) if g_res is not None else None
    dx = torch.empty_like(x2)
    part = torch.empty(getattr(lib(), entry + "_blocks")(R), H, dtype=torch.float32, device=x2.device) if need_w else None
    _launch(entry, (x2, w, dy2, gr), ptr(x2), ptr(w), ptr(dy2), ptr(gr), *map(ptr, stats), ptr(dx), ptr(part), R, H, *tail, _DT[x2.dtype],
            nbytes=R * H * x2.element_size() * (4 if gr is not None else 3))
    return dx.view(dy.shape), (sum_slabs(part, w.dtype) if need_w else None)


class _RMSNorm(torch.autograd.Function):

    @staticmethod
    def forward(ctx, x, delta, w, eps, w_offset=0.0):
        _require_cuda(x, w)
        x2 = x.contiguous().view(-1, x.shape[-1])
        R, H = x2.shape
        y = torch.empty_like(x2)
        rstd = torch.empty(R, dtype=torch.float32, device=x.device)
        if delta is not None:
            d2 = delta.contiguous().view(R, H)
            xo = torch.empty_like(x2)
        else:
            d2, xo = None, None
        off = float(w_offset)
        _launch("dta_rmsnorm_fwd", (x2, d2, w), ptr(x2), ptr(d2), ptr(w), ptr(xo), ptr(y), ptr(rstd), R, H, float(eps), off, _DT[x.dtype],
                nbytes=R * H * x2.element_size() * (4 if delta is not None else 2))
        xin = xo if xo is not None else x2
        ctx.save_for_backward(xin, w, rstd)
        ctx.has_delta, ctx.off = delta is not None, off
        return xin.view(x.shape), y.view(x.shape)

    @staticmethod
    def backward(ctx, g_res, dy):
        x2, w, rstd = ctx.saved_tensors
        dx, dw = _norm_bwd("dta_rmsnorm_bwd", x2, w, dy, g_res, (rstd,), (ctx.off,), ctx.needs_input_grad[2])
        return dx, (dx if ctx.has_delta else None), dw, None, None


def rms_norm(x: torch.Tensor, w: torch.Tensor, eps: float, w_offset: float = 0.0) -> torch.Tensor:
    return _RMSNorm.apply(x, None, w, eps, float(w_offset))[1]


def add_rms_norm(x: torch.Tensor, delta: Optional[torch.Tensor], w: torch.Tensor, eps: float, w_offset: float = 0.0):
    return _RMSNorm.apply(x, delta, w, eps, float(w_offset))


class _LayerNorm(torch.autograd.Function):

    @staticmethod
    def forward(ctx, x, delta_a, delta_b, w, eps):
        _require_cuda(x, w)
        if delta_b is not None and delta_a is None:
            raise ValueError("layer norm: delta_b without delta_a")
        x2 = x.contiguous().view(-1, x.shape[-1])
        R, H = x2.shape
        y = torch.empty_like(x2)
        mean = torch.empty(R, dtype=torch.float32, device=x.device)
        rstd = torch.empty(R, dtype=torch.float32, device=x.device)
        a2 = delta_a.contiguous().view(R, H) if delta_a is not None else None
        b2 = delta_b.contiguous().view(R, H) if delta_b is not None else None
        xo = torch.empty_like(x2) if a2 is not None else None
        n_in = 1 + (a2 is not None) + (b2 is not None)
        _launch("dta_layernorm_fwd", (x2, a2, b2, w), ptr(x2), ptr(a2), ptr(b2), ptr(w), ptr(xo), ptr(y), ptr(mean), ptr(rstd), R, H, float(eps),
                _DT[x.dtype], nbytes=R * H * x2.element_size() * (n_in + 1 + (xo is not None)))
        xin = xo if xo is not None else x2
        ctx.save_for_backward(xin, w, mean, rstd)
        ctx.deltas = (delta_a is not None, delta_b is not None)
        return xin.view(x.shape), y.view(x.shape)

    @staticmethod
    def backward(ctx, g_res, dy):
        x2, w, mean, rstd = ctx.saved_tensors
        dx, dw = _norm_bwd("dta_layernorm_bwd", x2, w, dy, g_res, (mean, rstd), (), ctx.needs_input_grad[3])
        return dx, (dx if ctx.deltas[0] else None), (dx if ctx.deltas[1] else None), dw, None


def layer_norm(x: torch.Tensor, w: torch.Tensor, eps: float) -> torch.Tensor:
    return _LayerNorm.apply(x, None, None, w, eps)[1]


def add_layer_norm(x: torch.Tensor, delta_a: Optional[torch.Tensor], delta_b: Optional[torch.Tensor], w: torch.Tensor, eps: float):
    return _LayerNorm.apply(x, delta_a, delta_b, w, eps)


class _RMSNormAdd(torch.autograd.Function):

    @staticmethod
    def forward(ctx, res, y, w, eps):
        _require_cuda(res, y, w)
        H = y.shape[-1]
        y2, r2 = y.contiguous().view(-1, H), res.contiguous().view(-1, H)
        R = y2.shape[0]
        out = torch.empty_like(y2)
        rstd = torch.empty(R, dtype=torch.float32, device=y.device)
        _launch("dta_rmsnorm_add_fwd", (y2, w, r2), ptr(y2), ptr(w), ptr(r2), ptr(out), None, ptr(rstd), R, H, float(eps), _DT[y.dtype],
                nbytes=3 * R * H * y2.element_size())
        ctx.save_for_backward(y2, w, rstd)
        return out.view(y.shape)

    @staticmethod
    def backward(ctx, dout):
        y2, w, rstd = ctx.saved_tensors
        dy, dw = _norm_bwd("dta_rmsnorm_bwd", y2, w, dout, None, (rstd,), (0.0,), ctx.needs_input_grad[2])
        return dout, dy, dw, None


def rms_norm_add(res: torch.Tensor, y: torch.Tensor, w: torch.Tensor, eps: float) -> torch.Tensor:
    return _RMSNormAdd.apply(res, y, w, eps)


def _wide_qk_norm_rope_fwd(x, w, cos_sin, eps):
    T, NH, D = x.shape
    if w.numel() != NH * D:
        raise ValueError(f"projection-wide norm weight has {w.numel()} elements for {NH} heads of {D}")
    y = torch.empty((T, NH, D), dtype=x.dtype, device=x.device)
    rstd = torch.empty(T, dtype=torch.float32, device=x.device)
    _launch("dta_wide_qk_norm_rope_fwd", (x, w, cos_sin), ptr(x), ptr(w), ptr(cos_sin), ptr(y), ptr(rstd), T, NH, D, x.stride(0), float(eps),
            _DT[x.dtype], nbytes=2 * T * NH * D * x.element_size() + T * D * 4)
    return y, rstd


def _wide_qk_norm_rope_bwd(x, w, cos_sin, dy, rstd, dx, need_w, eps=None):
    T, NH, D = x.shape
    if dy.stride(2) != 1:
        dy = dy.contiguous()
    part = torch.empty(lib().dta_wide_qk_norm_rope_bwd_blocks(T), NH * D, dtype=torch.float32, device=x.device) if need_w else None
    _launch("dta_wide_qk_norm_rope_bwd", (x, w, cos_sin, dy), ptr(x), ptr(w), ptr(cos_sin), ptr(dy), ptr(rstd), ptr(dx), ptr(part), T, NH, D,
            x.stride(0), dy.stride(0), dy.stride(1), dx.stride(0), _DT[x.dtype], nbytes=3 * T * NH * D * x.element_size() + T * D * 4)
    return sum_slabs(part, w.dtype) if part is not None else None


def _qk_norm_rope_fwd(x, w, cos_sin, eps):
    T, NH, D = x.shape
    y = torch.empty((T, NH, D), dtype=x.dtype, device=x.device)
    rstd = torch.empty(T * NH, dtype=torch.float32, device=x.device) if w is not None else None
    _launch("dta_qk_norm_rope_fwd", (x, w, cos_sin), ptr(x), ptr(w), ptr(cos_sin), ptr(y), ptr(rstd), T, NH, D, x.stride(0), float(eps),
            _DT[x.dtype], nbytes=2 * T * NH * D * x.element_size() + T * D * 4)
    return y, rstd


def _qk_norm_rope_bwd(x, w, cos_sin, dy, rstd, dx, need_w, eps=None):
    T, NH, D = x.shape
    if dy.stride(2) != 1:
        dy = dy.contiguous()
    part = torch.empty(lib().dta_qk_norm_rope_bwd_blocks(T * NH), D, dtype=torch.float32, device=x.device) if w is not None and need_w else None
    _launch("dta_qk_norm_rope_bwd", (x, cos_sin, dy), ptr(x), ptr(w), ptr(cos_sin), ptr(dy), ptr(rstd) if w is not None else None,
            ptr(dx), ptr(part), T, NH, D, x.stride(0), dy.stride(0), dy.stride(1), dx.stride(0), _DT[x.dtype],
            nbytes=(3 if w is not None else 2) * T * NH * D * x.element_size() + T * D * 4)
    return sum_slabs(part, w.dtype) if part is not None else None


def _rope_partial_fwd(x, w, cos_sin, interleaved):
    T, NH, D = x.shape
    R = cos_sin.shape[1]
    y = torch.empty((T, NH, D), dtype=x.dtype, device=x.device)
    _launch("dta_rope_partial_fwd", (x, cos_sin), ptr(x), ptr(cos_sin), ptr(y), T, NH, D, R, int(interleaved), x.stride(0), _DT[x.dtype],
            nbytes=2 * T * NH * D * x.element_size() + T * R * 4)
    return y, None


def _rope_partial_bwd(x, w, cos_sin, dy, stat, dx, need_w, interleaved):
    T, NH, D = dx.shape
    if dy.stride(2) != 1:
        dy = dy.contiguous()
    _launch("dta_rope_partial_bwd", (cos_sin, dy), ptr(cos_sin), ptr(dy), ptr(dx), T, NH, D, cos_sin.shape[1], int(interleaved),
            dy.stride(0), dy.stride(1), dx.stride(0), _DT[dx.dtype], nbytes=2 * T * NH * D * dx.element_size() + T * cos_sin.shape[1] * 4)


def _check_partial_table(x, cos_sin):
    if cos_sin.dim() != 2 or cos_sin.shape[0] != x.shape[0] or cos_sin.dtype != torch.float32 or not cos_sin.is_contiguous():
        raise ValueError(f"partial RoPE: cos_sin must be a contiguous fp32 [T, R] table for x {tuple(x.shape)}, got {cos_sin.dtype} {tuple(cos_sin.shape)}")


_HEAD_NORM = (_qk_norm_rope_fwd, _qk_norm_rope_bwd)
_WIDE_NORM = (_wide_qk_norm_rope_fwd, _wide_qk_norm_rope_bwd)
_PARTIAL = (_rope_partial_fwd, _rope_partial_bwd)


class _Rotate(torch.autograd.Function):

    @staticmethod
    def forward(ctx, x, w, cos_sin, form, arg):
        _require_cuda(x, cos_sin)
        if form is _PARTIAL:
            _check_partial_table(x, cos_sin)
        if x.stride(2) != 1 or x.stride(1) != x.shape[2]:
            x = x.contiguous()
        y, stat = form[0](x, w, cos_sin, arg)
        ctx.save_for_backward(None if form is _PARTIAL else x, w, cos_sin, stat)
        ctx.form, ctx.arg = form, arg
        return y

    @staticmethod
    def backward(ctx, dy):
        x, w, cos_sin, stat = ctx.saved_tensors
        dx = torch.empty(dy.shape, dtype=dy.dtype, device=dy.device)
        return dx, ctx.form[1](x, w, cos_sin, dy, stat, dx, ctx.needs_input_grad[1], ctx.arg), None, None, None


def _fused_grad_buffer(dq, dk, dv, T, Hq, Hkv, D, dtype):
    H3 = Hq + 2 * Hkv
    base = dv._base
    in_place = (base is not None and dq._base is base and dk._base is base and base.shape == (T, H3, D) and base.is_contiguous()
                and base.dtype == dtype and dq.shape == (T, Hq, D) and dk.shape == (T, Hkv, D) and dv.shape == (T, Hkv, D)
                and dq.stride() == dk.stride() == dv.stride() == (H3 * D, D, 1)
                and (dq.storage_offset(), dk.storage_offset(), dv.storage_offset()) == (0, Hq * D, (Hq + Hkv) * D))
    return base if in_place else None


class _QKVPrep(torch.autograd.Function):

    @staticmethod
    def forward(ctx, qkv, wq, wk, cos_sin, Hq, Hkv, form, arg):
        T, H3, D = qkv.shape
        ctx.geom, ctx.form, ctx.arg = (T, Hq, Hkv, D, qkv.dtype), form, arg
        xq, xk, v = qkv[:, :Hq], qkv[:, Hq:Hq + Hkv], qkv[:, Hq + Hkv:]
        if form is not None:
            _require_cuda(qkv, cos_sin)
        assert H3 == Hq + 2 * Hkv and qkv.is_contiguous()
        if form is None:
            return xq, xk, v
        if form is _PARTIAL:
            _check_partial_table(qkv, cos_sin)
        (q, sq), (k, sk) = form[0](xq, wq, cos_sin, arg), form[0](xk, wk, cos_sin, arg)
        ctx.save_for_backward(None if form is _PARTIAL else qkv, wq, wk, cos_sin, sq, sk)
        return q, k, v

    @staticmethod
    def backward(ctx, dq, dk, dv):
        T, Hq, Hkv, D, dtype = ctx.geom
        fused = _fused_grad_buffer(dq, dk, dv, T, Hq, Hkv, D, dtype)
        d = fused if fused is not None else torch.empty((T, Hq + 2 * Hkv, D), dtype=dtype, device=dv.device)
        dwq = dwk = None
        if ctx.form is not None:
            qkv, wq, wk, cos_sin, sq, sk = ctx.saved_tensors
            xq, xk = (qkv[:, :Hq], qkv[:, Hq:Hq + Hkv]) if qkv is not None else (None, None)
            dwq = ctx.form[1](xq, wq, cos_sin, dq, sq, d[:, :Hq], ctx.needs_input_grad[1], ctx.arg)
            dwk = ctx.form[1](xk, wk, cos_sin, dk, sk, d[:, Hq:Hq + Hkv], ctx.needs_input_grad[2], ctx.arg)
        elif fused is None:
            d[:, :Hq].copy_(dq); d[:, Hq:Hq + Hkv].copy_(dk)
        if fused is None:
            d[:, Hq + Hkv:].copy_(dv)
        return d, dwq, dwk, None, None, None, None, None


def qkv_prep(qkv: torch.Tensor, wq: Optional[torch.Tensor], wk: Optional[torch.Tensor], cos_sin: torch.Tensor, eps: float,
             Hq: int, Hkv: int):
    return _QKVPrep.apply(qkv, wq, wk, cos_sin, Hq, Hkv, _HEAD_NORM, eps)


def qkv_prep_wide(qkv: torch.Tensor, wq: torch.Tensor, wk: torch.Tensor, cos_sin: torch.Tensor, eps: float, Hq: int, Hkv: int):
    assert wq is not None and wk is not None
    return _QKVPrep.apply(qkv, wq, wk, cos_sin, Hq, Hkv, _WIDE_NORM, eps)


def qkv_prep_partial(qkv: torch.Tensor, cos_sin: torch.Tensor, Hq: int, Hkv: int, interleaved: bool):
    return _QKVPrep.apply(qkv, None, None, cos_sin, Hq, Hkv, _PARTIAL, bool(interleaved))


def qkv_prep_nope(qkv: torch.Tensor, Hq: int, Hkv: int):
    return _QKVPrep.apply(qkv, None, None, None, Hq, Hkv, None, None)


def rope_partial(x: torch.Tensor, cos_sin: torch.Tensor, interleaved: bool) -> torch.Tensor:
    return _Rotate.apply(x, None, cos_sin, _PARTIAL, bool(interleaved))


def qk_norm_rope(x: torch.Tensor, w: Optional[torch.Tensor], cos_sin: torch.Tensor, eps: float) -> torch.Tensor:
    return _Rotate.apply(x, w, cos_sin, _HEAD_NORM, eps)


ROPE_TYPES = ("default", "linear", "llama3", "yarn")


def rope_inv_freq(D: int, rope_parameters: dict, max_position_embeddings: Optional[int] = None):
    rp = rope_parameters
    kind = rp.get("rope_type", rp.get("type")) or "default"
    if kind not in ROPE_TYPES:
        raise ValueError(f"rope_parameters: rope_type {kind!r} is not supported ({' / '.join(ROPE_TYPES)})")
    base = float(rp["rope_theta"])
    steps = torch.arange(0, D, 2, dtype=torch.int64).to(torch.float32)
    if kind == "default":
        return 1.0 / (base ** (steps / D)), 1.0
    if kind == "linear":
        inv = 1.0 / (base ** (steps / D))
        inv /= rp["factor"]
        return inv, 1.0
    orig = rp.get("original_max_position_embeddings") or max_position_embeddings
    if orig is None:
        raise ValueError(f"rope_parameters: rope_type {kind!r} needs original_max_position_embeddings (or max_position_embeddings)")
    if kind == "llama3":
        inv = 1.0 / (base ** (steps / D))
        factor, low_f, high_f = rp["factor"], rp["low_freq_factor"], rp["high_freq_factor"]
        low_wavelen, high_wavelen = orig / low_f, orig / high_f
        wavelen = 2 * math.pi / inv
        scaled = torch.where(wavelen > low_wavelen, inv / factor, inv)
        smooth = (orig / wavelen - low_f) / (high_f - low_f)
        smoothed = (1 - smooth) * scaled / factor + smooth * scaled
        medium = ~(wavelen < high_wavelen) * ~(wavelen > low_wavelen)
        return torch.where(medium, smoothed, scaled), 1.0
    factor = rp.get("factor")
    if factor is None:
        if max_position_embeddings is None:
            raise ValueError("rope_parameters: yarn needs factor (or max_position_embeddings)")
        factor = max_position_embeddings / orig
    mscale_of = lambda scale, m=1: 1.0 if scale <= 1 else 0.1 * m * math.log(scale) + 1.0
    att = rp.get("attention_factor")
    if att is None:
        ms, ms_all = rp.get("mscale"), rp.get("mscale_all_dim")
        att = float(mscale_of(factor, ms) / mscale_of(factor, ms_all)) if ms and ms_all else mscale_of(factor)
    beta_fast, beta_slow = rp.get("beta_fast") or 32, rp.get("beta_slow") or 1
    corr_dim = lambda rot: (D * math.log(orig / (rot * 2 * math.pi))) / (2 * math.log(base))
    low, high = corr_dim(beta_fast), corr_dim(beta_slow)
    if rp.get("truncate", True):
        low, high = math.floor(low), math.ceil(high)
    low, high = max(low, 0), min(high, D - 1)
    if low == high:
        high += 0.001
    pos_freqs = base ** (steps / D)
    extrapolation, interpolation = 1.0 / pos_freqs, 1.0 / (factor * pos_freqs)
    keep = 1 - torch.clamp((torch.arange(D // 2, dtype=torch.float32) - low) / (high - low), 0, 1)
    return interpolation * (1 - keep) + extrapolation * keep, att


def longrope_inv_freq(R: int, rope_parameters: dict, max_position_embeddings: Optional[int], long: bool):
    rp = rope_parameters
    orig = rp.get("original_max_position_embeddings")
    if orig is None:
        raise ValueError("rope_parameters: longrope needs original_max_position_embeddings")
    name = "long_factor" if long else "short_factor"
    ext = rp.get(name)
    if ext is None or len(ext) != R // 2:
        raise ValueError(f"rope_parameters: longrope needs {name} with {R // 2} entries (rotary dimension {R}), got "
                         f"{'none' if ext is None else len(ext)}")
    factor = rp.get("factor")
    if factor is None:
        if max_position_embeddings is None:
            raise ValueError("rope_parameters: longrope needs factor (or max_position_embeddings)")
        factor = max_position_embeddings / orig
    att = rp.get("attention_factor")
    if att is None:
        att = 1.0 if factor <= 1.0 else math.sqrt(1 + math.log(factor) / math.log(orig))
    base = rp["rope_theta"]
    shape = torch.arange(0, R, 2, dtype=torch.int64).float() / R
    return 1.0 / (torch.tensor(ext, dtype=torch.float32) * base ** shape), att


_INV_FREQ: dict = {}


def rope_cos_sin(depth: torch.Tensor, D: int, rope) -> torch.Tensor:
    if isinstance(rope, (int, float)):
        key, host, factor = (D, float(rope), depth.device), None, 1.0
    else:
        host, factor = rope
        if host.shape != (D // 2,) or host.dtype != torch.float32 or host.device.type != "cpu":
            raise ValueError(f"rope_cos_sin: inv_freq must be a host fp32 [{D // 2}] tensor, got {host.dtype} {tuple(host.shape)} on {host.device}")
        key = (D, host.numpy().tobytes(), depth.device)
    inv = _INV_FREQ.get(key)
    if inv is None:
        if host is None:
            host = rope_inv_freq(D, {"rope_theta": float(rope)})[0]
        inv = host.to(depth.device)
        _INV_FREQ[key] = inv
    ang = depth.float()[:, None] * inv[None, :]
    table = torch.cat([ang.cos(), ang.sin()], dim=-1)
    if float(factor) != 1.0:
        table = table * float(factor)
    return table.contiguous()


class _SwiGLU(torch.autograd.Function):

    @staticmethod
    def forward(ctx, gu, g, u, kernel="dta_swiglu"):
        ctx.kernel = kernel
        if gu is not None:
            _require_cuda(gu)
            gu = gu if gu.stride(-1) == 1 and gu.dim() == 2 else gu.contiguous().view(-1, gu.shape[-1])
            C = gu.shape[1] // 2
            g, u, ld = gu[:, :C], gu[:, C:], gu.stride(0)
        else:
            _require_cuda(g, u)
            g = g.contiguous().view(-1, g.shape[-1]); u = u.contiguous().view(-1, u.shape[-1])
            C, ld = g.shape[1], g.shape[1]
        rows = g.shape[0]
        y = torch.empty((rows, C), dtype=g.dtype, device=g.device)
        _launch(ctx.kernel + "_fwd", (g, u), ptr(g), ptr(u), ptr(y), rows, C, ld, _DT[g.dtype], nbytes=3 * rows * C * g.element_size())
        ctx.save_for_backward(g, u)
        ctx.fused, ctx.ld = gu is not None, ld
        return y

    @staticmethod
    def backward(ctx, dy):
        g, u = ctx.saved_tensors
        rows, C = g.shape
        dy = dy.contiguous()
        if ctx.fused:
            dgu = torch.empty((rows, 2 * C), dtype=g.dtype, device=g.device)
            dg, du, ldg = dgu[:, :C], dgu[:, C:], 2 * C
        else:
            dg, du, ldg = torch.empty_like(g), torch.empty_like(u), C
        _launch(ctx.kernel + "_bwd", (g, u, dy), ptr(g), ptr(u), ptr(dy), ptr(dg), ptr(du), rows, C, ctx.ld, ldg, _DT[g.dtype],
                nbytes=5 * rows * C * g.element_size())
        return (dgu, None, None, None) if ctx.fused else (None, dg, du, None)


def swiglu(g: torch.Tensor, u: torch.Tensor) -> torch.Tensor:
    return _SwiGLU.apply(None, g, u, "dta_swiglu")


def swiglu_fused(gu: torch.Tensor) -> torch.Tensor:
    return _SwiGLU.apply(gu, None, None, "dta_swiglu")


def geglu(g: torch.Tensor, u: torch.Tensor) -> torch.Tensor:
    return _SwiGLU.apply(None, g, u, "dta_geglu")


def geglu_fused(gu: torch.Tensor) -> torch.Tensor:
    return _SwiGLU.apply(gu, None, None, "dta_geglu")


class weight_cache:
    depth = 0

    def __enter__(self):
        weight_cache.depth += 1
        return self

    def __exit__(self, *exc):
        weight_cache.depth -= 1
        if weight_cache.depth == 0:
            clear_weight_caches()
        return False


class _StackRows(torch.autograd.Function):

    CACHE_BYTES = 8 << 30
    _cache: dict = {}
    _cached_bytes = 0

    @staticmethod
    def _fused(ws):
        rows = [w.shape[0] for w in ws]
        key = tuple((id(w), w.data_ptr(), w._version) for w in ws)
        if weight_cache.depth > 0:
            hit = _StackRows._cache.get(key)
            if hit is not None:
                return hit
        out = torch.empty((sum(rows),) + tuple(ws[0].shape[1:]), dtype=ws[0].dtype, device=ws[0].device)
        o = 0
        for w, r in zip(ws, rows):
            out[o:o + r].copy_(w); o += r
        nbytes = out.numel() * out.element_size()
        if weight_cache.depth > 0 and _StackRows._cached_bytes + nbytes <= _StackRows.CACHE_BYTES:
            _StackRows._cache[key] = out; _StackRows._cached_bytes += nbytes
        return out

    @staticmethod
    def forward(ctx, *ws):
        ctx.rows = [w.shape[0] for w in ws]
        return _StackRows._fused(ws).detach()

    @staticmethod
    def backward(ctx, g):
        outs, o = [], 0
        for r in ctx.rows:
            outs.append(g[o:o + r]); o += r
        return tuple(outs)


def stack_rows(*ws: torch.Tensor) -> torch.Tensor:
    return _StackRows.apply(*ws)


def clear_stack_rows_cache() -> None:
    _StackRows._cache.clear(); _StackRows._cached_bytes = 0


def sum_slabs(part: torch.Tensor, out_dtype: torch.dtype, extra: torch.Tensor = None) -> torch.Tensor:
    assert part.dtype == torch.float32 and part.is_contiguous() and (extra is None or (extra.dtype == torch.float32 and extra.is_contiguous()))
    S, n = part.shape[0], part[0].numel()
    assert extra is None or extra.numel() == n
    out = torch.empty(part.shape[1:], dtype=out_dtype, device=part.device)
    _launch("dta_sum_slabs", (part, extra, out), ptr(part), S, n, n, ptr(extra), ptr(out), _DT[out_dtype], nbytes=(S + (extra is not None)) * n * 4)
    return out


def transpose_2d(w: torch.Tensor) -> torch.Tensor:
    R, C = w.shape
    if w.stride(1) != 1:
        w = w.contiguous()
    out = torch.empty((C, R), dtype=w.dtype, device=w.device)
    _launch("dta_transpose", (w, out), ptr(w), ptr(out), R, C, w.stride(0), R, w.element_size(), nbytes=2 * R * C * w.element_size())
    return out


class _TransposedWeights:
    cache: dict = {}
    nbytes = 0

    @staticmethod
    def get(w: torch.Tensor) -> torch.Tensor:
        if weight_cache.depth == 0:
            return transpose_2d(w)
        key = (w.data_ptr(), tuple(w.shape), tuple(w.stride()), w.dtype, w._version)
        hit = _TransposedWeights.cache.get(key)
        if hit is not None:
            return hit
        wt = transpose_2d(w)
        n = wt.numel() * wt.element_size()
        if _TransposedWeights.nbytes + n <= _StackRows.CACHE_BYTES:
            _TransposedWeights.cache[key] = wt; _TransposedWeights.nbytes += n
        return wt


def clear_weight_caches() -> None:
    clear_stack_rows_cache()
    _TransposedWeights.cache.clear(); _TransposedWeights.nbytes = 0


def _dgrad(dy: torch.Tensor, w: torch.Tensor) -> torch.Tensor:
    if dy.is_cuda and w.dtype in (torch.bfloat16, torch.float16) and dy.shape[0] >= 4096 and w.shape[0] % 8 == 0 and w.shape[1] % 8 == 0:
        return dy @ _TransposedWeights.get(w).t()
    return dy @ w


WGRAD_SPLIT_K = 4


def _wgrad(x: torch.Tensor, dy: torch.Tensor, transposed: bool) -> torch.Tensor:
    T = x.shape[0]
    a, b = (x, dy) if transposed else (dy, x)
    S = WGRAD_SPLIT_K
    tiles = -(-a.shape[1] // 256) * -(-b.shape[1] // 256)
    per = (T // S) // 64 * 64
    if tiles > 64 or per < 2048 or not x.is_cuda or x.dtype == torch.float32:
        out = a.t() @ b
    else:
        body = per * S
        part = torch.bmm(a[:body].reshape(S, per, a.shape[1]).transpose(1, 2), b[:body].reshape(S, per, b.shape[1]), out_dtype=torch.float32)
        rest = torch.mm(a[body:].t(), b[body:], out_dtype=torch.float32) if body < T else None
        out = sum_slabs(part, x.dtype, rest)
    if not transposed:
        return out
    V = 16 // out.element_size()
    return transpose_2d(out) if out.is_cuda and out.shape[0] % V == 0 and out.shape[1] % V == 0 else out.t()


class _Linear(torch.autograd.Function):

    @staticmethod
    def forward(ctx, x, w, b):
        ctx.save_for_backward(x, w)
        ctx.has_bias = b is not None
        return F.linear(x, w, b)

    @staticmethod
    def backward(ctx, dy):
        x, w = ctx.saved_tensors
        dx = _dgrad(dy, w) if ctx.needs_input_grad[0] else None
        dw = None
        if ctx.needs_input_grad[1]:
            dw = _wgrad(x, dy, w.shape[1] >= 2 * w.shape[0])
        db = dy.sum(0) if ctx.has_bias and ctx.needs_input_grad[2] else None
        return dx, dw, db


def linear(x: torch.Tensor, w: torch.Tensor, b: Optional[torch.Tensor] = None) -> torch.Tensor:
    return _Linear.apply(x, w, b)


MOE_FWD, MOE_DGRAD, MOE_WGRAD = 0, 1, 2


@dataclass
class MoeRouting:
    T: int
    k: int
    E: int
    expert_offsets: torch.Tensor
    row_of_pair: torch.Tensor
    src_token: torch.Tensor
    tiles: torch.Tensor


def moe_router_fwd_raw(logits: torch.Tensor, k: int, norm: bool):
    T, E_ = logits.shape
    logits = logits.contiguous()
    ids = torch.empty((T, k), dtype=torch.int32, device=logits.device)
    w = torch.empty((T, k), dtype=logits.dtype, device=logits.device)
    lse = torch.empty(T, dtype=torch.float32, device=logits.device)
    _launch("dta_moe_router_fwd", (logits,), ptr(logits), ptr(ids), ptr(w), ptr(lse), T, E_, k, int(bool(norm)), _DT[logits.dtype],
            nbytes=T * E_ * logits.element_size())
    return ids, w, lse


def moe_router_bwd_raw(logits, lse, ids, dw, norm: bool):
    T, E_ = logits.shape
    dw = dw.contiguous().to(logits.dtype)
    dl = torch.empty_like(logits)
    _launch("dta_moe_router_bwd", (logits, dw), ptr(logits), ptr(lse), ptr(ids), ptr(dw), ptr(dl), T, E_, ids.shape[1], int(bool(norm)),
            _DT[logits.dtype], nbytes=2 * T * E_ * logits.element_size())
    return dl


def moe_permute(ids: torch.Tensor, E_: int) -> MoeRouting:
    T, k = ids.shape
    P = T * k
    L = lib()
    dev = ids.device
    ws = torch.empty(max(int(L.dta_moe_permute_workspace(P, E_)), 1), dtype=torch.int32, device=dev)
    bound = int(L.dta_moe_tile_bound(P, E_))
    offs = torch.empty(E_ + 1, dtype=torch.int32, device=dev)
    rop = torch.empty(max(P, 1), dtype=torch.int32, device=dev)
    src = torch.empty(max(P, 1), dtype=torch.int32, device=dev)
    tiles = torch.empty(2 * bound, dtype=torch.int32, device=dev)
    ids = ids.contiguous()
    _launch("dta_moe_permute", (ids,), ptr(ids), T, k, E_, ptr(ws), ptr(offs), ptr(rop), ptr(src), ptr(tiles), nbytes=12 * P)
    return MoeRouting(T, k, E_, offs, rop[:P], src[:P], tiles)


def moe_grouped_gemm(mode: int, route: MoeRouting, w_shape, out_dtype, x=None, w=None, dy=None, gather: bool = False) -> torch.Tensor:
    E_, N, K = w_shape
    R = route.T * route.k
    ref = x if x is not None else dy
    shape = (R, N) if mode == MOE_FWD else (R, K) if mode == MOE_DGRAD else (E_, N, K)
    out = torch.empty(shape, dtype=out_dtype, device=ref.device)
    if R == 0 and mode != MOE_WGRAD:
        return out
    x, w, dy = (None if t is None else t.contiguous() for t in (x, w, dy))
    esz = out.element_size()
    _launch("dta_moe_grouped_gemm", tuple(t for t in (x, w, dy) if t is not None), mode, ptr(x), ptr(w), ptr(dy), ptr(out),
            ptr(route.src_token) if gather else None, ptr(route.expert_offsets), ptr(route.tiles), R, E_, N, K, _DT[out_dtype],
            nbytes=esz * (R * N + R * K + E_ * N * K), span=f"moe_gemm_{('fwd', 'dgrad', 'wgrad')[mode]}_{N}x{K}")
    return out


def moe_combine_fwd_raw(y, w, route: MoeRouting):
    H = y.shape[1]
    out = torch.empty((route.T, H), dtype=y.dtype, device=y.device)
    _launch("dta_moe_combine_fwd", (y,), ptr(y), ptr(w), ptr(route.row_of_pair), ptr(out), route.T, route.k, H, _DT[y.dtype],
            nbytes=(route.k + 1) * route.T * H * y.element_size())
    return out


def moe_combine_bwd_raw(dout, y, w, route: MoeRouting):
    H = y.shape[1]
    dout = dout.contiguous()
    dy = torch.empty_like(y)
    dw = torch.empty_like(w)
    _launch("dta_moe_combine_bwd", (dout, y, w), ptr(dout), ptr(y), ptr(w), ptr(route.row_of_pair), ptr(dy), ptr(dw), route.T, route.k, H,
            _DT[y.dtype], nbytes=(3 * route.k + 1) * route.T * H * y.element_size())
    return dy, dw


class _MoeRouter(torch.autograd.Function):

    @staticmethod
    def forward(ctx, logits, k, norm):
        ids, w, lse = moe_router_fwd_raw(logits, k, norm)
        ctx.save_for_backward(logits, lse, ids)
        ctx.norm = norm
        ctx.mark_non_differentiable(ids)
        return w, ids

    @staticmethod
    def backward(ctx, dw, _dids):
        logits, lse, ids = ctx.saved_tensors
        return moe_router_bwd_raw(logits, lse, ids, dw, ctx.norm), None, None


class _MoeLinear(torch.autograd.Function):

    @staticmethod
    def forward(ctx, x, w, route, gather):
        ctx.save_for_backward(x, w)
        ctx.route, ctx.gather = route, gather
        return moe_grouped_gemm(MOE_FWD, route, w.shape, x.dtype, x=x, w=w, gather=gather)

    @staticmethod
    def backward(ctx, dy):
        x, w = ctx.saved_tensors
        route, gather = ctx.route, ctx.gather
        dy = dy.contiguous()
        dx = dw = None
        if ctx.needs_input_grad[0]:
            dxs = moe_grouped_gemm(MOE_DGRAD, route, w.shape, x.dtype, w=w, dy=dy)
            dx = moe_combine_fwd_raw(dxs, None, route) if gather else dxs
        if ctx.needs_input_grad[1]:
            dw = moe_grouped_gemm(MOE_WGRAD, route, w.shape, w.dtype, x=x, dy=dy, gather=gather)
        return dx, dw, None, None


class _MoeCombine(torch.autograd.Function):
    @staticmethod
    def forward(ctx, y, w, route):
        ctx.save_for_backward(y, w)
        ctx.route = route
        return moe_combine_fwd_raw(y, w, route)

    @staticmethod
    def backward(ctx, dout):
        y, w = ctx.saved_tensors
        dy, dw = moe_combine_bwd_raw(dout, y, w, ctx.route)
        return dy, dw, None


def moe_mlp(h: torch.Tensor, router_w: torch.Tensor, gate_up_w: torch.Tensor, down_w: torch.Tensor, top_k: int,
            norm_topk_prob: bool) -> torch.Tensor:
    if not h.is_cuda:
        raise RuntimeError("moe_mlp runs on the MI355X only; there is no CPU path")
    E_ = gate_up_w.shape[0]
    logits = linear(h, router_w)
    w, ids = _MoeRouter.apply(logits, int(top_k), bool(norm_topk_prob))
    route = moe_permute(ids, E_)
    gu = _MoeLinear.apply(h, gate_up_w, route, True)
    act = swiglu_fused(gu)
    y = _MoeLinear.apply(act, down_w, route, False)
    return _MoeCombine.apply(y, w, route)


def _host_f32(vals):
    return None if vals is None else np.ascontiguousarray(vals, np.float32)


def lora_down(x: torch.Tensor, m: torch.Tensor, rscale=None) -> torch.Tensor:
    T, K = x.shape
    R = m.shape[0]
    assert x.stride(1) == 1 and m.stride(1) == 1 and m.shape[1] == K and m.dtype == x.dtype
    out = torch.empty((T, R), dtype=x.dtype, device=x.device)
    rs = _host_f32(rscale)
    _launch("dta_lora_down", (x, m), ptr(x), x.stride(0), ptr(m), m.stride(0), ptr(out), R, None if rs is None else rs.ctypes.data,
            T, R, K, _DT[x.dtype], nbytes=(T * K + R * K + T * R) * x.element_size())
    return out


def lora_wgrad(l: torch.Tensor, x: torch.Tensor, out_dtype: torch.dtype, rscale=None) -> torch.Tensor:
    T, K = x.shape
    R = l.shape[1]
    assert l.shape[0] == T and l.stride(1) == 1 and x.stride(1) == 1 and l.dtype == x.dtype
    S = int(lib().dta_lora_wgrad_slabs(T, K))
    part = torch.empty((S, R, K), dtype=torch.float32, device=x.device)
    rs = _host_f32(rscale)
    _launch("dta_lora_wgrad", (l, x), ptr(l), l.stride(0), ptr(x), x.stride(0), ptr(part), None if rs is None else rs.ctypes.data,
            T, R, K, _DT[x.dtype], nbytes=(T * K + T * R) * x.element_size() + S * R * K * 4)
    return part[0] if (S == 1 and out_dtype == torch.float32) else sum_slabs(part, out_dtype)


WGRAD_KERNEL_MAX_K = 12288


def _down_by_kernel(K: int, R: int) -> bool:
    return K <= 1024 and R <= 32


def _wgrad_by_kernel(K: int) -> bool:
    return K <= WGRAD_KERNEL_MAX_K


def _lora_wgrad(l: torch.Tensor, x: torch.Tensor, out_dtype: torch.dtype, seg_scale=None) -> torch.Tensor:
    K = x.shape[1]
    if _wgrad_by_kernel(K):
        rs = None
        if seg_scale is not None:
            rs = np.ones(l.shape[1], np.float32)
            for r0, r, sc in seg_scale:
                rs[r0:r0 + r] = sc
        return lora_wgrad(l, x, out_dtype, rs)
    g = torch.mm(l.t(), x, out_dtype=torch.float32)
    for r0, r, sc in seg_scale or ():
        if sc != 1.0:
            g[r0:r0 + r] *= sc
    return g if out_dtype == torch.float32 else g.to(out_dtype)


class _LoraLinear(torch.autograd.Function):

    @staticmethod
    def forward(ctx, x, w, b, spec, *ab):
        dt = x.dtype
        As, Bs = ab[0::2], ab[1::2]
        y = F.linear(x, w, b)
        a_cat = torch.cat([a.to(dt) for a in As]) if len(As) > 1 else As[0].to(dt)
        if not a_cat.is_contiguous():
            a_cat = a_cat.contiguous()
        xa = lora_down(x, a_cat) if _down_by_kernel(x.shape[1], a_cat.shape[0]) else x @ a_cat.t()
        bs = [B_.to(dt) for B_ in Bs]
        r0 = 0
        for (n0, nlen, r, s), B_ in zip(spec, bs):
            y[:, n0:n0 + nlen].addmm_(xa[:, r0:r0 + r], B_.t(), alpha=s); r0 += r
        ctx.save_for_backward(x, w, xa, a_cat, *bs)
        ctx.spec, ctx.has_bias, ctx.ab_dtypes = spec, b is not None, [t.dtype for t in ab]
        return y

    @staticmethod
    def backward(ctx, dy):
        x, w, xa, a_cat = ctx.saved_tensors[:4]
        bs = ctx.saved_tensors[4:]
        spec, dt = ctx.spec, x.dtype
        dy = dy.contiguous()
        R, N = a_cat.shape[0], dy.shape[1]
        seg_scale, r0 = [], 0
        for n0, nlen, r, s in spec:
            seg_scale.append((r0, r, s)); r0 += r
        if _down_by_kernel(N, R):
            bd = torch.zeros((R, N), dtype=dt, device=x.device)
            rs = np.ones(R, np.float32)
            for (n0, nlen, r, s), (q0, _, _), B_ in zip(spec, seg_scale, bs):
                bd[q0:q0 + r, n0:n0 + nlen] = B_.t(); rs[q0:q0 + r] = s
            dxa = lora_down(dy, bd, rs)
        else:
            dxa = torch.empty((dy.shape[0], R), dtype=dt, device=x.device)
            for (n0, nlen, r, s), (q0, _, _), B_ in zip(spec, seg_scale, bs):
                torch.addmm(dxa[:, q0:q0 + r], dy[:, n0:n0 + nlen], B_, beta=0, alpha=s, out=dxa[:, q0:q0 + r])
        dx = None
        if ctx.needs_input_grad[0]:
            dx = _dgrad(dy, w)
            dx = dx.addmm_(dxa, a_cat) if dx.is_contiguous() else dx + dxa @ a_cat
        dw = _wgrad(x, dy, w.shape[1] >= 2 * w.shape[0]) if ctx.needs_input_grad[1] else None
        db = dy.sum(0) if ctx.has_bias and ctx.needs_input_grad[2] else None
        need = ctx.needs_input_grad[4:]
        g32 = lambda i: torch.float32 if ctx.ab_dtypes[i] == torch.float32 else dt
        dA = dB = None
        if any(need[0::2]):
            dA = _lora_wgrad(dxa, x, torch.float32 if any(ctx.ab_dtypes[i] == torch.float32 for i in range(0, len(need), 2)) else dt)
        if any(need[1::2]):
            dB = _lora_wgrad(xa, dy, torch.float32 if any(ctx.ab_dtypes[i] == torch.float32 for i in range(1, len(need), 2)) else dt, seg_scale)
        out, r0 = [], 0
        for i, (n0, nlen, r, _) in enumerate(spec):
            out.append(dA[r0:r0 + r].to(g32(2 * i)) if need[2 * i] else None)
            out.append(dB[r0:r0 + r, n0:n0 + nlen].t().to(g32(2 * i + 1)).contiguous() if need[2 * i + 1] else None)
            r0 += r
        return (dx, dw, db, None, *out)


def lora_linear(x: torch.Tensor, w: torch.Tensor, b: Optional[torch.Tensor], adapters) -> torch.Tensor:
    if not adapters:
        return linear(x, w, b)
    if x.is_cuda and x.dtype in (torch.bfloat16, torch.float16):
        spec = tuple((int(n0), int(nlen), int(A.shape[0]), float(s)) for n0, nlen, A, B_, s in adapters)
        ab = [t for _, _, A, B_, _ in adapters for t in (A, B_)]
        return _LoraLinear.apply(x, w, b, spec, *ab)
    y = linear(x, w, b)
    cols, o = [], 0
    for n0, nlen, A, B_, s in adapters:
        if n0 > o:
            cols.append(y[:, o:n0])
        cols.append(y[:, n0:n0 + nlen] + float(s) * ((x @ A.to(x.dtype).t()) @ B_.to(x.dtype).t()))
        o = n0 + nlen
# ... 159 lines not shown
```

### dynamictreeattn_amd/tree_training_engine.py

```python
from __future__ import annotations

from typing import Callable, List, Optional

import numpy as np
import torch

from . import ops, packing
from .losses import PREFERENCE_STATS, STATS as LOSS_STATS, PolicyLoss, PreferenceLoss
from .model import (_head_dim, ensure_supported, final_softcap_of, head_weight, is_cohere, is_gemma2, is_glm4, is_longrope, is_moe_layer, logit_scale_of, moe_geometry,
                    longrope_boundary, packed_hidden_states)
from .trie import pop_block_starts

__all__ = ["TreeTrainingEngine", "_get_forkpos", "packed_logprob_entropy"]


def _get_forkpos(lens, lcp_lens, block_size: Optional[int]) -> list:
    pos = {c - 1 for c in lcp_lens if c > 0}
    if block_size is not None:
        for i, end in enumerate(lens):
            start = lcp_lens[i] if i < len(lcp_lens) else 0
            pos.update(s - 1 for s in pop_block_starts(start, end, block_size) if s > 0)
    return sorted(pos)


def fork_tables_host(fork_child, fork_parent, T: int):
    fork_child, fork_parent = np.asarray(fork_child, np.int64), np.asarray(fork_parent, np.int64)
    order = np.argsort(fork_parent, kind="stable")
    fc, fp = fork_child[order], fork_parent[order]
    ptr = np.zeros(T + 1, np.int64)
    if fp.size:
        np.cumsum(np.bincount(fp, minlength=T), out=ptr[1:])
    return fc, fp, ptr


def head_call_args(W: torch.Tensor, tp_group, softcap: float, logit_scale: float, pick_rows):
    kw = {}
    if tp_group is not None:
        import torch.distributed as dist
        tp, rk = dist.get_world_size(tp_group), dist.get_rank(tp_group)
        Vp = W.shape[0] // tp
        assert Vp * tp == W.shape[0], "vocabulary must divide by the tensor-parallel size"
        W = W[rk * Vp:(rk + 1) * Vp]
        kw.update(tp_group=tp_group, vocab_offset=rk * Vp)
    if softcap:
        kw.update(softcap=softcap, max_picks_per_row=int(np.bincount(pick_rows).max()) if len(pick_rows) else 0)
    if logit_scale != 1.0:
        kw.update(temperature=1.0 / float(logit_scale))
    return W, kw


def packed_logprob_entropy(h: torch.Tensor, W: torch.Tensor, tokens: torch.Tensor, parent: torch.Tensor,
                           want_entropy: bool, chunk: int = 2048, fork_child: Optional[np.ndarray] = None,
                           fork_parent: Optional[np.ndarray] = None, tp_group=None, fork_dev=None, softcap: float = 0.0,
                           logit_scale: float = 1.0):
    T = h.shape[0]
    dev = h.device
    if fork_child is None:
        fork_child = np.zeros(0, np.int64); fork_parent = np.zeros(0, np.int64)
    if fork_dev is None:
        fork_child, fork_parent, ptr = fork_tables_host(fork_child, fork_parent, T)
        fc_dev, fp_dev = torch.from_numpy(fork_child).to(dev), torch.from_numpy(fork_parent).to(dev)
        fork_ptr = torch.from_numpy(ptr.astype(np.int32)).to(dev) if fork_child.size else None
    else:
        fc_dev, fp_dev, fork_ptr = fork_dev
    nF = int(np.asarray(fork_child).size)
    ftok = tokens[fc_dev] if nF else tokens.new_zeros(0)
    if not nF:
        fork_ptr = None
    nxt = torch.cat([tokens[1:], tokens.new_zeros(1)])
    bounds = np.searchsorted(np.asarray(fork_parent), np.arange(0, T + chunk, chunk)).tolist()
    W, kw = head_call_args(W, tp_group, softcap, logit_scale, np.asarray(fork_parent, np.int64))
    lp_next, lp_fork, ent = ops.lm_head_rows(h, W, nxt, fork_ptr, ftok, fp_dev, bounds, want_entropy, chunk, **kw)
    chain = torch.zeros(T, dtype=torch.bool, device=dev)
    chain[1:] = parent[1:] == torch.arange(0, T - 1, device=dev, dtype=parent.dtype)
    lp = torch.cat([lp_next.new_zeros(1), lp_next[:-1]]) * chain
    if nF:
        lp = lp.index_copy(0, fc_dev, lp_fork)
    return lp, ent


def sum_loss_terms(terms, device):
    if not terms:
        return None
    ts = [t if isinstance(t, torch.Tensor) else torch.as_tensor(float(t), dtype=torch.float32, device=device) for t in terms]
    return ts[0].reshape(()) if len(ts) == 1 else torch.stack([t.reshape(()).float() for t in ts]).sum()


class _PackedTrie:

    PAD_FROM = 2048
    PAD_TO = 256

    def __init__(self, trie, device, n_kv_heads: int = 8):
        device = torch.device(device)
        if device.type == "cuda" and device.index is None:
            device = torch.device("cuda", torch.cuda.current_device())
        if trie._dev.device != device:
            raise RuntimeError(f"TokenTrie holds its tokens on {trie._dev.device} but the engine runs on {device}: build it with "
                               f"TokenTrie(..., device={str(device)!r}) (or torch.cuda.set_device) so that one GPU owns the whole pass")
        plan = packing.plan_segments(trie.lens, trie.lcp_lens)
        self.n_real_tokens = plan.T
        M_real = plan.M
        leaf_off = [trie._dev.starts[s] for s in trie._leaf_src]
        if plan.T >= self.PAD_FROM and plan.T % self.PAD_TO:
            plan = packing.pad_plan(plan, self.PAD_TO)
            leaf_off = leaf_off + [0]
        self.plan = plan
        M, T = plan.M, plan.T
        run_ptr, runs = packing.plan_qtile_runs(plan)
        leaf_off = np.asarray(leaf_off, np.int64)
        kq = packing.ktile_qend_host(plan)
        units, splits, n_slabs = packing.plan_dkv_units(kq, T, T, 0, n_kv_heads)
        first = plan.seg_off[:-1].astype(np.int64)
        nonempty = np.diff(plan.seg_off) > 0
        par = plan.parent_of_seg.astype(np.int64)
        is_fork = nonempty & (par >= 0) & (par != first - 1)
        self.fork_child, self.fork_parent, fork_ptr = fork_tables_host(first[is_fork], par[is_fork], T)
        paths = []
        for i in range(M_real):
            pieces = [np.arange(b, e, dtype=np.int64) for b, e in plan.path_runs[i]]
            pieces.append(np.arange(plan.seg_off[i], plan.seg_off[i + 1], dtype=np.int64))
            paths.append(np.concatenate(pieces))
        self.path_sizes = [p.size for p in paths]
        self._paths_host = paths
        from ._staging import upload
        (seg_off, seg_d0, par_seg, brk_ptr, brk_depth, brk_end, run_ptr_d, runs_d, kq_d, units_d, splits_d, fptr_d) = upload(
            [plan.seg_off, plan.seg_depth0, plan.parent_of_seg, plan.brk_ptr, plan.brk_depth, plan.brk_end, run_ptr, runs.reshape(-1),
             kq, units.reshape(-1), splits.reshape(-1), fork_ptr], device, np.int32)
        leaf_off_d, self.path_cat, fc_d, fp_d = upload(
            [leaf_off, np.concatenate(paths) if paths else np.zeros(0, np.int64), self.fork_child, self.fork_parent], device, np.int64)
        self.fork_dev = (fc_d, fp_d, fptr_d)
        self.paths = list(torch.split(self.path_cat, self.path_sizes))
        self.tokens = torch.empty(T, dtype=torch.long, device=device)
        meta_i = torch.empty(3, T, dtype=torch.int32, device=device)
        self.depth, self.parent, self.subtree_end = meta_i[0], meta_i[1], meta_i[2]
        self._expand(trie._dev.tokens, leaf_off_d, seg_off, seg_d0, par_seg, brk_ptr, brk_depth, brk_end, M, T)
        self.meta = ops.TreeAttnMeta(T=T, subtree_end=self.subtree_end, run_ptr=run_ptr_d, runs=runs_d.view(-1, 4), ktile_qend=kq_d,
                                     dkv_units=units_d.view(-1, 4), dkv_splits=splits_d.view(-1, 4) if splits.shape[0] else None,
                                     n_slabs=n_slabs)
        self._seg_tables, self._n_kv_heads, self._win_metas = (seg_off, seg_d0, par_seg), n_kv_heads, {}

    def for_window(self, window: int):
        if window not in self._win_metas:
            self._win_metas[window] = ops.window_meta(self.meta, self.plan, self.depth, window, self._n_kv_heads, self._seg_tables)
        return self._win_metas[window]

    def sequence_rows(self, attach_lists):
        lp_rows, ent_rows = [], []
        for i, attach_list in enumerate(attach_lists):
            path = self._paths_host[i]
            for _, length in attach_list:
                lp_rows.append(path[1:length]); ent_rows.append(path[:length])
        from ._staging import upload
        empty = np.zeros(0, np.int64)
        return upload([np.concatenate(lp_rows) if lp_rows else empty, np.concatenate(ent_rows) if ent_rows else empty], self.tokens.device, np.int64)

    def _expand(self, tokens, leaf_off, seg_off, seg_d0, par_seg, brk_ptr, brk_depth, brk_end, M, T):
        from ._lib import check, lib, ptr
        with ops._on(tokens, leaf_off, seg_off, self.tokens) as stream:
            st = lib().dta_preorder_meta(ptr(tokens), ptr(leaf_off), ptr(seg_off), ptr(seg_d0), ptr(par_seg), ptr(brk_ptr), ptr(brk_depth),
                                         ptr(brk_end), M, T, ptr(self.tokens), ptr(self.depth), ptr(self.parent), ptr(self.subtree_end), stream)
        check(st, "dta_preorder_meta")


def _mlp_elems_per_token(c, l: int) -> float:
    if is_moe_layer(c, l):
        E, I, _ = moe_geometry(c)
        return c.num_experts_per_tok * (3 * I + c.hidden_size) + 2 * E
    return 4 * c.intermediate_size


def _has_moe(c) -> bool:
    return any(is_moe_layer(c, l) for l in range(c.num_hidden_layers))


def _stack_sink_fits(model, budget: int) -> bool:
    n = sum(p.numel() for p in model.parameters() if p.requires_grad)
    return n * 6 <= budget // 5


class TreeTrainingEngine:
    def __init__(self, model_config, device, dtype: torch.dtype, max_seq_len: int, forward_only: bool = False):
        if torch.device(device).type == "cuda" and dtype not in (torch.bfloat16, torch.float16, torch.float32):
            raise TypeError(f"TreeTrainingEngine supports dtype torch.bfloat16 / torch.float16 (MFMA kernels) and torch.float32 (the reference's "
                            f"--dtype fp32, run.py:122-132: plain-FMA attention kernels, a gradient-check path), got {dtype}")
        self.model = None
        self.device = torch.device(device)
        if self.device.type == "cuda" and self.device.index is None:
            self.device = torch.device("cuda", torch.cuda.current_device())
        self.dtype = dtype
        self.max_seq_len = max_seq_len
        self.forward_only = forward_only
        self.n_layers = model_config.num_hidden_layers
        self.n_kv_heads = getattr(model_config, "num_key_value_heads", 8)
        self.cur_len = 0
        self.forkpos_list: List[int] = []
        self._loss_host = None
        self.returns: List[Optional[torch.Tensor]] = []
        self.last_packed: Optional[_PackedTrie] = None
        self.head_chunk = 2048
        self.checkpoint_layers: Optional[bool] = None
        self.mode = "auto"
        self.memory_budget_bytes: Optional[int] = None
        self.last_mode: Optional[str] = None
        self.attn_keep_fraction = 0.25
        self.partial_recompute = True
        self.tp_group = None
        self._attn_keep_planned = 0
        self.stack_fp32_grads = True
        self.longrope_factors = "auto"
        self.last_loss_path: Optional[str] = None
        self.loss_stats: Optional[torch.Tensor] = None

    def _pack(self, token_trie) -> _PackedTrie:
        longest = max(token_trie.lens) if token_trie.lens else 0
        assert longest <= self.max_seq_len, (
            f"Exceeds max_seq_len: cur_len=0, new_tokens={longest}, max={self.max_seq_len}")
        p0 = next(iter(self.model.parameters()), None) if hasattr(self.model, "parameters") else None
        if p0 is not None and (p0.dtype != self.dtype or p0.device != self.device):
            raise RuntimeError(f"model parameters are {p0.dtype} on {p0.device}; this engine was built for {self.dtype} on {self.device}")
        packed = _PackedTrie(token_trie, self.device, self.n_kv_heads)
        self.last_packed = packed
        return packed

    def _longrope_long(self, model, token_trie) -> bool:
        if not is_longrope(model.config):
            return False
        how = self.longrope_factors
        if how in ("short", "long"):
            return how == "long"
        if how != "auto":
            raise ValueError(f"longrope_factors = {how!r}: 'auto', 'short' or 'long'")
        orig = longrope_boundary(model.config)
        lens = [int(ids.size(0)) for ids in token_trie.inputs]
        n_long = sum(n > orig for n in lens)
        if 0 < n_long < len(lens):
            raise ValueError(f"this trie holds sequences on both sides of original_max_position_embeddings = {orig} ({len(lens) - n_long} up to "
                             f"it, {n_long} longer): HF rotates the two groups by different longrope factors, and their shared prefix rows "
                             f"cannot have both - set engine.longrope_factors to 'short' or 'long' (the set the sampler used)")
        return n_long > 0

    def _should_checkpoint(self, model, T: int) -> bool:
        if self.checkpoint_layers is not None:
            return self.checkpoint_layers
        need = self._per_token_layer_bytes(model) * self.n_layers * T
        if self.device.type != "cuda":
            return False
        free = self._free_hbm()
        return need > 0.75 * free

    def _free_hbm(self) -> int:
        return ops.free_hbm(self.device)

    def _per_token_layer_bytes(self, model) -> int:
        c = model.config
        D = _head_dim(c)
        L = c.num_hidden_layers
        mlp = sum(_mlp_elems_per_token(c, l) for l in range(L)) / max(L, 1)
        from . import lora
        ranks = lora.rank_elems_per_token(model)
        norms = 2 * c.hidden_size if is_gemma2(c) or is_glm4(c) else 0
        rows = 8 if is_cohere(c) else 10
        return int(2 * (rows * c.hidden_size + norms + mlp + ranks + 4 * (c.num_attention_heads + c.num_key_value_heads) * D))

    def _budget(self) -> Optional[int]:
        if self.memory_budget_bytes is not None:
            return int(self.memory_budget_bytes)
        if self.device.type != "cuda":
            return None
        free = self._free_hbm()
        return int(0.8 * free)

    def _stack_block_rows(self, model, T: int, block_size: Optional[int]) -> Optional[int]:
        if self.mode == "packed":
            return None
        budget = self._budget()
        per_layer = self._per_token_layer_bytes(model)
        c = model.config
        if self.mode != "stack":
            if budget is None:
                return None
            need = T * (2 * 2 * c.hidden_size * self.n_layers + 2 * per_layer)
            if need <= budget:
                return None
        if self.mode != "stack" and budget is not None and self.stack_fp32_grads and _has_moe(c) and not _stack_sink_fits(model, budget):
            return None
        bs = block_size or 2048
        if budget is None:
            return bs
        rows = int(0.5 * budget / max(per_layer * self.n_layers, 1)) // 256 * 256
        return int(max(bs, min(rows, 16384)))

    def _backward_stack(self, model, token_trie, loss_fn, block_rows: int) -> float:
        from . import dp
        from .stack_engine import StackWalk
        dp.defer_active_reducers()
        budget = self._budget()
        walk = StackWalk(model, token_trie, self.device, self.dtype, block_rows, self.head_chunk, self.tp_group,
                         grad_budget_bytes=0 if not self.stack_fp32_grads else (None if budget is None else budget // 5),
                         longrope_long=self._longrope_long(model, token_trie))
        total = walk.run(loss_fn)
        self.last_mode = f"stack[{block_rows}]x{walk.n_blocks}"
        self.cur_len = 0
        return float(total.item()) if total is not None else 0.0

    @staticmethod
    def packed_rows(n_tree_tokens: int) -> int:
        T = int(n_tree_tokens)
        if T >= _PackedTrie.PAD_FROM and T % _PackedTrie.PAD_TO:
            T += (-T) % _PackedTrie.PAD_TO
        return T

    def warm_gemm_shapes(self, model, row_counts) -> None:
        from types import SimpleNamespace
        body = model.model
        one = SimpleNamespace(config=model.config, model=SimpleNamespace(embed_tokens=body.embed_tokens, layers=[body.layers[0]], norm=body.norm))
        ident = lambda l: (lambda q, k, v: q)
        for T in sorted({int(t) for t in row_counts if t > 0}):
            tokens = torch.zeros(T, dtype=torch.long, device=self.device)
            depth = torch.arange(T, device=self.device, dtype=torch.int32) % 64
            parent = torch.arange(-1, T - 1, device=self.device, dtype=torch.int32)
            with torch.enable_grad():
                h = packed_hidden_states(one, tokens, depth, None, False, 0, ident)
                lp, ent = packed_logprob_entropy(h, head_weight(model), tokens, parent, True, self.head_chunk, softcap=final_softcap_of(model),
                                                 logit_scale=logit_scale_of(model))
                (lp.sum() + ent.sum()).backward()
        for p in model.parameters():
            p.grad = None
        if self.device.type == "cuda":
            torch.cuda.synchronize(self.device)

    def _full_layers(self, model, T: int):
        if self.device.type != "cuda" or not self.partial_recompute or self.checkpoint_layers is not None:
            return 0
        c = model.config
        head = int(2.0 * T * c.vocab_size * 2 + 2 * 4 * c.vocab_size * c.hidden_size)
        esz = torch.empty(0, dtype=self.dtype).element_size()
        D = _head_dim(c)
        stash_l = 2 * T * c.hidden_size * esz
        attn_l = T * c.num_attention_heads * (D * esz + 4)
        attn_keep = self._attn_keep_planned
        L = self.n_layers

        def plan(layer0_bytes: int) -> int:
            d0 = max(int(layer0_bytes), 1)
            avail = int(0.7 * self._free_hbm()) - 2 * d0 - head
            for n in range(L, 1, -1):
                rec = L - n
                if (n - 1) * d0 + rec * stash_l + min(attn_keep, rec * attn_l) <= avail:
                    return n
            return 1
        return plan

    def _attn_keep_bytes(self) -> int:
        self._attn_keep_planned = 0
        if self.device.type != "cuda" or self.attn_keep_fraction <= 0:
            return 0
        free = self._free_hbm()
        self._attn_keep_planned = int(self.attn_keep_fraction * free)
        return self._attn_keep_planned

    def _path_losses(self, packed, token_trie, lp, ent, loss_fn):
        lp_all, ent_all = lp.detach()[packed.path_cat], ent.detach()[packed.path_cat]
        terms, leaves, o = [], [], 0
        want = torch.is_grad_enabled() and (lp.requires_grad or ent.requires_grad)
        for i, attach_list in enumerate(token_trie.attach_lists):
            for attachment, length in attach_list:
                a, e = lp_all[o + 1:o + length], ent_all[o:o + length]
                if want:
                    a.requires_grad_(lp.requires_grad); e.requires_grad_(ent.requires_grad)
                terms.append(loss_fn(a, e, attachment)); leaves += [a, e]
            o += packed.path_sizes[i]
        return sum_loss_terms(terms, lp.device), leaves

    @staticmethod
    def _backprop_paths(packed, token_trie, lp, ent, total, leaves):
        total.backward()
        rows = None
        roots, grads = [], []
        for k, src in ((0, lp), (1, ent)):
            gs = [t.grad for t in leaves[k::2]]
            if not src.requires_grad or all(g is None for g in gs):
                continue
            if rows is None:
                rows = packed.sequence_rows(token_trie.attach_lists)
            vals = torch.cat([g if g is not None else torch.zeros_like(t) for g, t in zip(gs, leaves[k::2])])
            acc = torch.zeros_like(src)
            acc.index_put_((rows[k],), vals.to(acc.dtype), accumulate=True)
            roots.append(src); grads.append(acc)
        if roots:
            torch.autograd.backward(roots, grads)

    @staticmethod
    def _policy_rows(packed, token_trie, lp, ent, loss):
        from ._staging import upload
        row_lo, row_hi, seq_ptr, _ = packing.policy_row_tables(packed.plan, token_trie.attach_lists)
        tables = [row_lo, row_hi, seq_ptr]
        if loss.ratio == "sequence":
            tables += packing.policy_path_tables(packed.plan, token_trie.attach_lists)
        dev = packed.tokens.device
        row_lo_d, row_hi_d, seq_ptr_d, *path_d = upload(tables, dev, np.int32)
        old, ref, mask, adv, adv_per_seq = ops.policy_token_inputs(loss, token_trie.attach_lists, seq_ptr, dev)
        dlp, dent, stats, _ = ops.policy_loss(loss, lp, ent, packed.depth, row_lo_d, row_hi_d, seq_ptr_d, old, ref, mask, adv, adv_per_seq,
                                              tuple(path_d) or None)
        return dlp, dent, stats

    @staticmethod
    def _preference_rows(packed, token_trie, lp, loss):
        from ._staging import upload
        row_lo, row_hi, seq_ptr, _ = packing.policy_row_tables(packed.plan, token_trie.attach_lists)
        tables = [row_lo, row_hi, seq_ptr, *packing.policy_path_tables(packed.plan, token_trie.attach_lists),
                  *packing.preference_pair_tables(token_trie.attach_lists)]
        dev = packed.tokens.device
        row_lo_d, row_hi_d, seq_ptr_d, *rest = upload(tables, dev, np.int32)
        ref_lp, ref_sum, mask = ops.preference_token_inputs(loss, token_trie.attach_lists, seq_ptr, dev)
        dlp, stats, _, _ = ops.preference_loss(loss, lp, packed.depth, row_lo_d, row_hi_d, seq_ptr_d, tuple(rest[:4]), tuple(rest[4:]),
                                               ref_lp, ref_sum, mask)
        return dlp, stats

    def _backward_stack_two_pass(self, model, token_trie, loss, block_rows: int) -> float:
        forkpos = self.forkpos_list
        logprobs = self.forward(model, token_trie)
        self.forkpos_list = forkpos
        atts = [None] * len(logprobs)
        for attach_list in token_trie.attach_lists:
            for att, _ in attach_list:
                atts[att["_sequence_batch_id"]] = att
        total, g, stats = loss.coefficients(logprobs, atts)
        del logprobs
        self._backward_stack(model, token_trie, loss.surrogate(g), block_rows)
        self.last_loss_path, self.loss_stats = "two_pass", stats
        return float(total.item())

    @torch.no_grad()
    def forward(self, model, token_trie) -> List[torch.Tensor]:
        self.model = model
        ensure_supported(model)
        self.returns = [None] * token_trie.n_sequences
        self.forkpos_list = _get_forkpos(None, token_trie.lcp_lens, None)
        if token_trie.n_sequences == 0:
            return self.returns
        with ops.weight_cache():
            return self._forward(model, token_trie)

    def _forward(self, model, token_trie):
        packed = self._pack(token_trie)
        h = packed_hidden_states(model, packed.tokens, packed.depth, packed.meta, False, meta_for_window=packed.for_window,
                                 longrope_long=self._longrope_long(model, token_trie))
        lp, _ = packed_logprob_entropy(h, head_weight(model), packed.tokens, packed.parent, False, self.head_chunk,
                                       packed.fork_child, packed.fork_parent, self.tp_group, packed.fork_dev, final_softcap_of(model),
                                       logit_scale_of(model))
        for i, attach_list in enumerate(token_trie.attach_lists):
            lp_path = lp[packed.paths[i][1:]]
            for attachment, length in attach_list:
                self.returns[attachment["_sequence_batch_id"]] = lp_path[:length - 1].clone()
        self.cur_len = 0
        return self.returns

    def backward(self, model, token_trie, loss_fn: Callable, block_size: int, cut_f1_tail: bool = True) -> float:
        self.model = model
        ensure_supported(model)
        lens = [int(ids.size(0)) for ids in token_trie.inputs]
        self.forkpos_list = _get_forkpos(lens, token_trie.lcp_lens, block_size)
        self.last_loss_path, self.loss_stats = "callback", None
        if token_trie.n_sequences == 0:
            return 0.0
        with ops.weight_cache():
            return self._backward(model, token_trie, loss_fn, block_size)

    def _backward(self, model, token_trie, loss_fn, block_size):
        n_tree = sum(token_trie.lens) - sum(token_trie.lcp_lens)
        rows = self._stack_block_rows(model, n_tree, block_size)
        if self.tp_group is not None:
            import torch.distributed as dist
            v = torch.tensor([rows if rows is not None else (1 << 30)], device=self.device, dtype=torch.int32)
            dist.all_reduce(v, op=dist.ReduceOp.MIN, group=self.tp_group)
            rows = None if int(v.item()) >= (1 << 30) else int(v.item())
        if rows is not None:
            longest = max(token_trie.lens)
            assert longest <= self.max_seq_len, f"Exceeds max_seq_len: cur_len=0, new_tokens={longest}, max={self.max_seq_len}"
            if isinstance(loss_fn, PreferenceLoss):
                return self._backward_stack_two_pass(model, token_trie, loss_fn, rows)
            return self._backward_stack(model, token_trie, loss_fn, rows)
        packed = self._pack(token_trie)
        chunk = min(self.head_chunk, block_size) if block_size else self.head_chunk
        ckpt = self._should_checkpoint(model, packed.plan.T)
        self.last_mode = "packed+recompute" if ckpt else "packed"
        attn_keep = self._attn_keep_bytes() if ckpt else 0
        full = self._full_layers(model, packed.plan.T) if ckpt else 0
        kept = []
        h = packed_hidden_states(model, packed.tokens, packed.depth, packed.meta, ckpt, attn_keep, None, full, kept,
                                 meta_for_window=packed.for_window, longrope_long=self._longrope_long(model, token_trie))
        if ckpt and kept:
            self.last_mode = "packed" if kept[0] >= self.n_layers else f"packed+recompute[{self.n_layers - kept[0]}/{self.n_layers}]"
        lp, ent = packed_logprob_entropy(h, head_weight(model), packed.tokens, packed.parent, True, max(chunk, 1),
                                         packed.fork_child, packed.fork_parent, self.tp_group, packed.fork_dev, final_softcap_of(model),
                                       logit_scale_of(model))
        fused = isinstance(loss_fn, (PolicyLoss, PreferenceLoss))
        if isinstance(loss_fn, PreferenceLoss):
            self.last_loss_path = "fused"
            dlp, stats = self._preference_rows(packed, token_trie, lp, loss_fn)
            dent = None
            self.loss_stats = stats[:len(PREFERENCE_STATS)]
            total = stats[0]
        elif fused:
            self.last_loss_path = "fused"
            dlp, dent, stats = self._policy_rows(packed, token_trie, lp, ent, loss_fn)
            self.loss_stats = stats[:len(LOSS_STATS)]
            total = stats[0]
        else:
            total, leaves = self._path_losses(packed, token_trie, lp, ent, loss_fn)
        if total is None:
            return 0.0
        landed = None
        if total.is_cuda:
            if self._loss_host is None:
                self._loss_host = torch.empty(1, dtype=torch.float32).pin_memory()
            self._loss_host.copy_(total.detach().reshape(1).float(), non_blocking=True)
            landed = torch.cuda.Event(); landed.record()
        if fused:
            roots = [(lp, dlp)] + ([(ent, dent)] if dent is not None and loss_fn.entropy_coef != 0 else [])
            roots = [(t, g) for t, g in roots if t.requires_grad]
            if roots and torch.is_grad_enabled():
                torch.autograd.backward([t for t, _ in roots], [g for _, g in roots])
        elif total.requires_grad:
            self._backprop_paths(packed, token_trie, lp, ent, total, leaves)
        self.cur_len = 0
        if landed is None:
            return float(total.item())
        landed.synchronize()
        return float(self._loss_host.item())
```

### include/dta.h

```cpp
#ifndef DTA_H
#define DTA_H
#include <stdint.h>

#ifdef __cplusplus
extern "C" {
#endif

#define DTA_OK 0
#define DTA_EINVAL (-1)
#define DTA_EUNSUPPORTED (-2)
#define DTA_EALIGN (-3)
#define DTA_ELAUNCH (-4)
#define DTA_EPRIOR (-5)

#define DTA_BF16 0
#define DTA_F16 1
#define DTA_F32 2

#define DTA_QTILE 128
#define DTA_KTILE 128

int dta_version(void);

int dta_take_pending_error(char* msg, int32_t cap);


int dta_lcp_adjacent(const int64_t* tokens, const int64_t* starts, const int32_t* lens, int32_t S,
                     int32_t* out_lcp, int32_t* out_unsorted, void* stream);

int dta_leafize(const int32_t* lens, const int32_t* lcp, int32_t S,
                int32_t* out_leaf_pos, int32_t* out_leaf_lcp, int32_t* out_seq_leaf, int32_t* out_M,
                void* stream);

int dta_preorder_meta(const int64_t* tokens, const int64_t* leaf_tok_off,
                      const int32_t* seg_off, const int32_t* seg_depth0, const int32_t* parent_of_seg,
                      const int32_t* brk_ptr, const int32_t* brk_depth, const int32_t* brk_end,
                      int32_t M, int32_t T,
                      int64_t* out_token, int32_t* out_depth, int32_t* out_parent, int32_t* out_subtree_end,
                      void* stream);

int dta_tree_attn_fwd(const void* q, const void* k, const void* v, void* out, float* lse,
                      const int32_t* subtree_end, const int32_t* run_ptr, const int32_t* runs,
                      int32_t Tq, int32_t Tk, int32_t q_offset, int32_t Hq, int32_t Hkv, int32_t head_dim,
                      int64_t q_stride_t, int64_t q_stride_h, int64_t k_stride_t, int64_t k_stride_h,
                      int64_t v_stride_t, int64_t v_stride_h,
                      int64_t o_stride_t, int64_t o_stride_h, float scale, int32_t dtype,
                      const int32_t* win_lo, int32_t window, float softcap, void* stream);

int dta_tree_attn_bwd(const void* q, const void* k, const void* v, const void* out, const void* dout,
                      const float* lse, float* delta, void* dq, void* dk, void* dv,
                      const int32_t* subtree_end, const int32_t* run_ptr, const int32_t* runs,
                      const int32_t* ktile_qend,
                      int32_t Tq, int32_t Tk, int32_t q_offset, int32_t Hq, int32_t Hkv, int32_t head_dim,
                      int64_t q_stride_t, int64_t q_stride_h, int64_t k_stride_t, int64_t k_stride_h,
                      int64_t v_stride_t, int64_t v_stride_h,
                      int64_t o_stride_t, int64_t o_stride_h, int64_t dq_stride_t, int64_t dq_stride_h,
                      int64_t dkv_stride_t, int64_t dkv_stride_h,
                      float scale, int32_t dtype, int32_t accumulate,
                      int32_t which ,
                      const int32_t* dkv_units, int32_t n_units, const int32_t* dkv_splits, int32_t n_splits, float* dkv_ws,
                      const int32_t* win_lo, int32_t window, float softcap, void* stream);

int dta_window_lo(const int32_t* depth, const int32_t* seg_off, const int32_t* seg_depth0, const int32_t* parent_of_seg,
                  int32_t M, int32_t T, int32_t window, int32_t* out_win_lo, void* stream);

int dta_logprob_entropy_fwd(const void* logits, const int64_t* labels, const int32_t* extra_ptr, const int64_t* extra_labels,
                            float* lse, float* entropy, float* logprob, float* extra_logprob,
                            int32_t R, int32_t V, int64_t row_stride, float temperature, int32_t dtype, float softcap, void* stream);
int dta_logprob_entropy_shard_stats(const void* logits, const int64_t* labels, const int32_t* extra_ptr, const int64_t* extra_labels,
                                    float* stats, float* extra_picked,
                                    int32_t R, int32_t V, int64_t row_stride, float temperature, int32_t dtype, float softcap, void* stream);
int dta_logprob_entropy_bwd(const void* logits, void* dlogits, const int64_t* labels, const int32_t* extra_ptr, const int64_t* extra_labels,
                            const float* lse, const float* entropy,
                            const float* g_logprob, const float* g_extra_logprob, const float* g_entropy,
                            int32_t R, int32_t V, int64_t row_stride, int64_t out_row_stride, float temperature, int32_t dtype,
                            float softcap, void* stream);

int dta_rmsnorm_fwd(const void* x, const void* delta, const void* w, void* x_out, void* y, float* rstd,
                    int32_t R, int32_t H, float eps, float w_offset, int32_t dtype, void* stream);
int dta_rmsnorm_bwd_blocks(int32_t R);
int dta_rmsnorm_bwd(const void* x, const void* w, const void* dy, const void* dres, const float* rstd, void* dx, float* dw_partial,
                    int32_t R, int32_t H, float w_offset, int32_t dtype, void* stream);
int dta_layernorm_fwd(const void* x, const void* delta_a, const void* delta_b, const void* w, void* x_out, void* y,
                      float* mean, float* rstd, int32_t R, int32_t H, float eps, int32_t dtype, void* stream);
int dta_layernorm_bwd_blocks(int32_t R);
int dta_layernorm_bwd(const void* x, const void* w, const void* dy, const void* dres, const float* mean, const float* rstd,
                      void* dx, float* dw_partial, int32_t R, int32_t H, int32_t dtype, void* stream);
int dta_qk_norm_rope_fwd(const void* x, const void* w, const float* cos_sin, void* y, float* rstd,
                         int32_t T, int32_t NH, int32_t head_dim, int64_t x_stride_t, float eps, int32_t dtype, void* stream);
int dta_qk_norm_rope_bwd_blocks(int64_t n_heads_total);
int dta_qk_norm_rope_bwd(const void* x, const void* w, const float* cos_sin, const void* dy, const float* rstd,
                         void* dx, float* dw_partial, int32_t T, int32_t NH, int32_t head_dim,
                         int64_t x_stride_t, int64_t dy_stride_t, int64_t dy_stride_h, int64_t dx_stride_t,
                         int32_t dtype, void* stream);
int dta_rope_partial_fwd(const void* x, const float* cos_sin, void* y, int32_t T, int32_t NH, int32_t head_dim, int32_t rotary_dim,
                         int32_t pairing, int64_t x_stride_t, int32_t dtype, void* stream);
int dta_rope_partial_bwd(const float* cos_sin, const void* dy, void* dx, int32_t T, int32_t NH, int32_t head_dim, int32_t rotary_dim,
                         int32_t pairing, int64_t dy_stride_t, int64_t dy_stride_h, int64_t dx_stride_t, int32_t dtype, void* stream);
int dta_wide_qk_norm_rope_fwd(const void* x, const void* w, const float* cos_sin, void* y, float* rstd,
                              int32_t T, int32_t NH, int32_t head_dim, int64_t x_stride_t, float eps, int32_t dtype, void* stream);
int dta_wide_qk_norm_rope_bwd_blocks(int32_t T);
int dta_wide_qk_norm_rope_bwd(const void* x, const void* w, const float* cos_sin, const void* dy, const float* rstd,
                              void* dx, float* dw_partial, int32_t T, int32_t NH, int32_t head_dim,
                              int64_t x_stride_t, int64_t dy_stride_t, int64_t dy_stride_h, int64_t dx_stride_t,
                              int32_t dtype, void* stream);
int dta_rmsnorm_add_fwd(const void* y, const void* w, const void* res, void* out, void* yn, float* rstd,
                        int32_t R, int32_t H, float eps, int32_t dtype, void* stream);
int dta_swiglu_fwd(const void* gate, const void* up, void* y, int64_t rows, int32_t cols, int64_t ld, int32_t dtype, void* stream);
int dta_swiglu_bwd(const void* gate, const void* up, const void* dy, void* dgate, void* dup,
                   int64_t rows, int32_t cols, int64_t ld, int64_t ld_grad, int32_t dtype, void* stream);
int dta_geglu_fwd(const void* gate, const void* up, void* y, int64_t rows, int32_t cols, int64_t ld, int32_t dtype, void* stream);
int dta_geglu_bwd(const void* gate, const void* up, const void* dy, void* dgate, void* dup,
                  int64_t rows, int32_t cols, int64_t ld, int64_t ld_grad, int32_t dtype, void* stream);

int dta_transpose(const void* in, void* out, int64_t rows, int64_t cols, int64_t ld_in, int64_t ld_out, int32_t elem_size, void* stream);

int dta_sum_slabs(const float* part, int64_t slabs, int64_t n, int64_t slab_stride, const float* extra, void* out, int32_t out_dtype, void* stream);

#define DTA_MOE_BM 128
#define DTA_MOE_FWD 0
#define DTA_MOE_DGRAD 1
#define DTA_MOE_WGRAD 2

int dta_moe_router_fwd(const void* logits, int32_t* topk_ids, void* topk_w, float* lse, int32_t T, int32_t E, int32_t k, int32_t norm_topk,
                       int32_t dtype, void* stream);
int dta_moe_router_bwd(const void* logits, const float* lse, const int32_t* topk_ids, const void* dtopk_w, void* dlogits,
                       int32_t T, int32_t E, int32_t k, int32_t norm_topk, int32_t dtype, void* stream);

int dta_moe_permute_workspace(int32_t n_pairs, int32_t E);
int dta_moe_tile_bound(int32_t n_pairs, int32_t E);
int dta_moe_permute(const int32_t* topk_ids, int32_t T, int32_t k, int32_t E, int32_t* workspace,
                    int32_t* expert_offsets, int32_t* row_of_pair, int32_t* src_token, int32_t* tiles, void* stream);

int dta_moe_grouped_gemm(int32_t mode, const void* x, const void* w, const void* dy, void* out, const int32_t* gather,
                         const int32_t* expert_offsets, const int32_t* tiles, int32_t n_rows, int32_t E, int32_t N, int32_t K,
                         int32_t dtype, void* stream);

int dta_moe_combine_fwd(const void* y, const void* topk_w, const int32_t* row_of_pair, void* out, int32_t T, int32_t k, int32_t H,
                        int32_t dtype, void* stream);
int dta_moe_combine_bwd(const void* dout, const void* y, const void* topk_w, const int32_t* row_of_pair, void* dy, void* dtopk_w,
                        int32_t T, int32_t k, int32_t H, int32_t dtype, void* stream);

int dta_lora_down(const void* x, int64_t ldx, const void* m, int64_t ldm, void* out, int64_t ldo, const float* rscale_host,
                  int32_t T, int32_t R, int32_t K, int32_t dtype, void* stream);
int dta_lora_wgrad_slabs(int32_t T, int32_t K);
int dta_lora_wgrad(const void* l, int64_t ldl, const void* x, int64_t ldx, float* part, const float* rscale_host,
                   int32_t T, int32_t R, int32_t K, int32_t dtype, void* stream);

int dta_policy_loss_blocks(int32_t T);
int dta_policy_loss(const float* lp, const float* ent, const int32_t* depth, const int32_t* row_seq_lo, const int32_t* row_seq_hi,
                    const int32_t* seq_ptr, const float* old_lp, const float* ref_lp, const float* mask, const float* adv,
                    int32_t adv_per_seq, float* w, float* dlp, float* dent, float* partial, float* stats, int32_t T, int32_t S,
                    float clip_low, float clip_high, float dual_clip, float kl_coef, int32_t kl_estimator, float entropy_coef,
                    int32_t agg, float scale, void* stream);

int dta_policy_loss_seq_blocks(int32_t T, int32_t S);
int dta_policy_loss_seq(const float* lp, const float* ent, const int32_t* depth, const int32_t* row_seq_lo, const int32_t* row_seq_hi,
                        const int32_t* seq_ptr, const int32_t* leaf_run_ptr, const int32_t* run_row0, const int32_t* run_depth0,
                        const int32_t* seq_leaf, const float* old_lp, const float* ref_lp, const float* mask, const float* adv,
                        int32_t adv_per_seq, float* w, float* c, float* dlp, float* dent, float* partial, float* stats, int32_t T,
                        int32_t S, int32_t M, int32_t R, float clip_low, float clip_high, float dual_clip, float kl_coef,
                        int32_t kl_estimator, float entropy_coef, int32_t agg, float scale, void* stream);

int dta_preference_loss_blocks(int32_t T, int32_t S, int32_t P);
int dta_preference_loss(const float* lp, const int32_t* depth, const int32_t* row_seq_lo, const int32_t* row_seq_hi,
                        const int32_t* seq_ptr, const int32_t* leaf_run_ptr, const int32_t* run_row0, const int32_t* run_depth0,
                        const int32_t* seq_leaf, const int32_t* pair_c, const int32_t* pair_r, const float* ref_lp,
                        const float* ref_sum, const float* mask, float* nhat, float* u, float* sft, float* g, float* dlp,
                        float* partial, float* stats, int32_t T, int32_t S, int32_t M, int32_t R, int32_t P, int32_t kind,
                        float beta, float label_smoothing, float gamma, int32_t length_normalize, int32_t reference_free,
                        float sft_coef, float scale, void* stream);

#ifdef __cplusplus
}
#endif
#endif
```

Baseline: 856,400.

## Batch weight stacking and transposes into one layout kernel, fuse slab-sum with transpose

Adds a batched layout kernel that builds the stacked QKV/gate-up weights and the transposed dgrad weights for all layers in a single launch before forward/backward, instead of building each cached layout lazily with separate kernels. Also adds a split-K wgrad reduction that sums fp32 slabs and writes the transposed result directly, which removes a separate transpose pass. Both target launch overhead and extra memory traffic in the training step. The cost is extra host-side job construction every call and prefilling caches that may not all be used, within the existing cache byte limits.

```diff
diff --git a/dynamictreeattn_amd/_lib.py b/dynamictreeattn_amd/_lib.py
--- a/dynamictreeattn_amd/_lib.py
+++ b/dynamictreeattn_amd/_lib.py
@@ -42,6 +42,8 @@
     "dta_geglu_bwd": ([_vp] * 5 + [_i64, _i32, _i64, _i64, _i32, _vp], C.c_int),
     "dta_transpose": ([_vp, _vp, _i64, _i64, _i64, _i64, _i32, _vp], C.c_int),
     "dta_sum_slabs": ([_vp, _i64, _i64, _i64, _vp, _vp, _i32, _vp], C.c_int),
+    "dta_sum_slabs_transposed": ([_vp, _i64, _i64, _i64, _i64, _vp, _vp, _i64, _i32, _vp], C.c_int),
+    "dta_layout_batch": ([_vp, _vp, _i32, _vp], C.c_int),
     "dta_moe_router_fwd": ([_vp] * 4 + [_i32] * 5 + [_vp], C.c_int),
     "dta_moe_router_bwd": ([_vp] * 5 + [_i32] * 5 + [_vp], C.c_int),
     "dta_moe_permute_workspace": ([_i32, _i32], C.c_int),
diff --git a/dynamictreeattn_amd/csrc/elementwise_kernels.hip b/dynamictreeattn_amd/csrc/elementwise_kernels.hip
--- a/dynamictreeattn_amd/csrc/elementwise_kernels.hip
+++ b/dynamictreeattn_amd/csrc/elementwise_kernels.hip
@@ -817,46 +817,88 @@
   }
 }
 
+typedef uint32_t u32x4 __attribute__((ext_vector_type(4)));
+constexpr int TR_TS = 64;
+template <int ESZ> constexpr int tr_pitch() { return (ESZ == 2 ? TR_TS / 2 : TR_TS) + 4; }
+
+template <bool NT> __device__ __forceinline__ u32x4 ld16(const char* p) {
+  if constexpr (NT) return DTA_SAVED_LOAD(reinterpret_cast<const u32x4*>(p));
+  else return *reinterpret_cast<const u32x4*>(p);
+}
+
 template <int ESZ>
-__global__ __launch_bounds__(256) void transpose_kernel(const char* __restrict__ in, char* __restrict__ out, int64_t rows, int64_t cols, int64_t ld_in, int64_t ld_out) {
-  constexpr int TS = 64;
-  constexpr int WPR = ESZ == 2 ? TS / 2 : TS;
-  constexpr int PITCH = WPR + 4;
-  __shared__ __attribute__((aligned(16))) uint32_t tile[TS * PITCH];
-  const int64_t r0 = (int64_t)blockIdx.y * TS, c0 = (int64_t)blockIdx.x * TS;
+__device__ __forceinline__ void transpose_tile_store(const uint32_t* tile, char* __restrict__ out, int64_t rows, int64_t cols, int64_t ld_out,
+                                                     int64_t r0, int64_t c0) {
+  constexpr int TS = TR_TS, PITCH = tr_pitch<ESZ>(), V = 16 / ESZ, CH = TS / V;
+  for (int i = threadIdx.x; i < TS * CH; i += 256) {
+    const int oc = i / CH, k = i % CH;
+    if (c0 + oc < cols && r0 + V * k < rows)
+      *reinterpret_cast<u32x4*>(out + ((c0 + oc) * ld_out + r0 + V * k) * ESZ) = *reinterpret_cast<const u32x4*>(&tile[oc * PITCH + 4 * k]);
+  }
+}
+
+template <int ESZ, bool NT>
+__device__ __forceinline__ void transpose_tile(uint32_t* tile, const char* __restrict__ in, char* __restrict__ out, int64_t rows, int64_t cols,
+                                               int64_t ld_in, int64_t ld_out, int64_t r0, int64_t c0) {
+  constexpr int TS = TR_TS, PITCH = tr_pitch<ESZ>();
   const int tid = threadIdx.x;
   if (ESZ == 2) {
     const int rp = tid >> 3, ch = tid & 7, r = 2 * rp, c = 8 * ch;
-    uint4 a = make_uint4(0, 0, 0, 0), b = make_uint4(0, 0, 0, 0);
+    u32x4 a = {0, 0, 0, 0}, b = {0, 0, 0, 0};
     if (c0 + c < cols) {
-      if (r0 + r < rows) a = *reinterpret_cast<const uint4*>(in + ((r0 + r) * ld_in + c0 + c) * 2);
-      if (r0 + r + 1 < rows) b = *reinterpret_cast<const uint4*>(in + ((r0 + r + 1) * ld_in + c0 + c) * 2);
-    }
-    const uint32_t aw[4] = {a.x, a.y, a.z, a.w}, bw[4] = {b.x, b.y, b.z, b.w};
+      if (r0 + r < rows) a = ld16<NT>(in + ((r0 + r) * ld_in + c0 + c) * 2);
+      if (r0 + r + 1 < rows) b = ld16<NT>(in + ((r0 + r + 1) * ld_in + c0 + c) * 2);
+    }
 #pragma unroll
     for (int j = 0; j < 4; ++j) {
-      tile[(c + 2 * j) * PITCH + rp] = (aw[j] & 0xffffu) | (bw[j] << 16);
-      tile[(c + 2 * j + 1) * PITCH + rp] = (aw[j] >> 16) | (bw[j] & 0xffff0000u);
-    }
-    __syncthreads();
-    for (int i = tid; i < TS * 8; i += 256) {
-      const int oc = i >> 3, k = i & 7;
-      if (c0 + oc < cols && r0 + 8 * k < rows)
-        *reinterpret_cast<uint4*>(out + ((c0 + oc) * ld_out + r0 + 8 * k) * 2) = *reinterpret_cast<const uint4*>(&tile[oc * PITCH + 4 * k]);
+      tile[(c + 2 * j) * PITCH + rp] = (a[j] & 0xffffu) | (b[j] << 16);
+      tile[(c + 2 * j + 1) * PITCH + rp] = (a[j] >> 16) | (b[j] & 0xffff0000u);
     }
   } else {
     for (int i = tid; i < TS * 16; i += 256) {
       const int r = i >> 4, c = 4 * (i & 15);
-      uint4 a = make_uint4(0, 0, 0, 0);
-      if (r0 + r < rows && c0 + c < cols) a = *reinterpret_cast<const uint4*>(in + ((r0 + r) * ld_in + c0 + c) * 4);
-      tile[(c + 0) * PITCH + r] = a.x; tile[(c + 1) * PITCH + r] = a.y; tile[(c + 2) * PITCH + r] = a.z; tile[(c + 3) * PITCH + r] = a.w;
-    }
-    __syncthreads();
-    for (int i = tid; i < TS * 16; i += 256) {
-      const int oc = i >> 4, k = i & 15;
-      if (c0 + oc < cols && r0 + 4 * k < rows)
-        *reinterpret_cast<uint4*>(out + ((c0 + oc) * ld_out + r0 + 4 * k) * 4) = *reinterpret_cast<const uint4*>(&tile[oc * PITCH + 4 * k]);
-    }
+      u32x4 a = {0, 0, 0, 0};
+      if (r0 + r < rows && c0 + c < cols) a = ld16<NT>(in + ((r0 + r) * ld_in + c0 + c) * 4);
+      tile[(c + 0) * PITCH + r] = a[0]; tile[(c + 1) * PITCH + r] = a[1]; tile[(c + 2) * PITCH + r] = a[2]; tile[(c + 3) * PITCH + r] = a[3];
+    }
+  }
+  __syncthreads();
+  transpose_tile_store<ESZ>(tile, out, rows, cols, ld_out, r0, c0);
+}
+
+template <int ESZ>
+__global__ __launch_bounds__(256) void transpose_kernel(const char* __restrict__ in, char* __restrict__ out, int64_t rows, int64_t cols, int64_t ld_in, int64_t ld_out) {
+  __shared__ __attribute__((aligned(16))) uint32_t tile[TR_TS * tr_pitch<ESZ>()];
+  transpose_tile<ESZ, false>(tile, in, out, rows, cols, ld_in, ld_out, (int64_t)blockIdx.y * TR_TS, (int64_t)blockIdx.x * TR_TS);
+}
+
+template <int ESZ, bool NT>
+__device__ __forceinline__ void copy_tile(const char* __restrict__ in, char* __restrict__ out, int64_t rows, int64_t cols, int64_t ld_in, int64_t ld_out,
+                                          int64_t r0, int64_t c0) {
+  constexpr int V = 16 / ESZ, CH = TR_TS / V;
+  for (int i = threadIdx.x; i < TR_TS * CH; i += 256) {
+    const int64_t r = r0 + i / CH, c = c0 + V * (i % CH);
+    if (r < rows && c < cols) *reinterpret_cast<u32x4*>(out + (r * ld_out + c) * ESZ) = ld16<NT>(in + (r * ld_in + c) * ESZ);
+  }
+}
+
+__global__ __launch_bounds__(256) void layout_batch_kernel(const DtaLayoutJob* __restrict__ jobs, int n_jobs) {
+  __shared__ __attribute__((aligned(16))) uint32_t tile[TR_TS * tr_pitch<4>()];
+  const int64_t b = blockIdx.x;
+  int lo = 0, hi = n_jobs;
+  while (hi - lo > 1) { const int mid = (lo + hi) >> 1; if (jobs[mid].tile0 <= b) lo = mid; else hi = mid; }
+  const DtaLayoutJob j = jobs[lo];
+  const int64_t tx = (j.cols + TR_TS - 1) / TR_TS, t = b - j.tile0;
+  const int64_t r0 = (t / tx) * TR_TS, c0 = (t % tx) * TR_TS;
+  const char* in = static_cast<const char*>(j.src);
+  char* out = static_cast<char*>(j.dst);
+  constexpr bool NT = DTA_EW_NT != 0;
+  if (j.kind == DTA_LAYOUT_COPY) {
+    if (j.elem_size == 2) copy_tile<2, NT>(in, out, j.rows, j.cols, j.ld_src, j.ld_dst, r0, c0);
+    else copy_tile<4, NT>(in, out, j.rows, j.cols, j.ld_src, j.ld_dst, r0, c0);
+  } else {
+    if (j.elem_size == 2) transpose_tile<2, NT>(tile, in, out, j.rows, j.cols, j.ld_src, j.ld_dst, r0, c0);
+    else transpose_tile<4, NT>(tile, in, out, j.rows, j.cols, j.ld_src, j.ld_dst, r0, c0);
   }
 }
 
@@ -901,6 +943,52 @@
     for (int j = 0; j < 4; ++j) o[j] = (e)t[j];
     *reinterpret_cast<e4*>(reinterpret_cast<e*>(out_) + 4 * i) = o;
   }
+}
+template <int DT>
+__global__ __launch_bounds__(256) void sum_slabs_transposed_kernel(const float* __restrict__ part, int slabs, int64_t rows, int64_t cols, int64_t stride,
+                                                                   const float* __restrict__ extra, void* __restrict__ out_, int64_t ld_out) {
+  using e = typename Ty<DT>::e;
+  typedef float f4 __attribute__((ext_vector_type(4)));
+  constexpr int ESZ = sizeof(e), TS = TR_TS, PITCH = tr_pitch<ESZ>();
+  __shared__ __attribute__((aligned(16))) uint32_t tile[TS * PITCH];
+  const int64_t r0 = (int64_t)blockIdx.y * TS, c0 = (int64_t)blockIdx.x * TS;
+  const int tid = threadIdx.x;
+  auto sum4 = [&](int64_t r, int64_t c) {
+    const int64_t i = r * cols + c;
+    f4 t = extra ? *reinterpret_cast<const f4*>(extra + i) : f4{0.f, 0.f, 0.f, 0.f};
+    for (int s2 = 0; s2 < slabs; ++s2) t += *reinterpret_cast<const f4*>(part + s2 * stride + i);
+    return t;
+  };
+  if constexpr (ESZ == 2) {
+    typedef e e8 __attribute__((ext_vector_type(8)));
+    auto row8 = [&](int64_t r, int64_t c) {
+      const f4 lo = sum4(r, c), hi = sum4(r, c + 4);
+      e8 v;
+#pragma unroll
+      for (int j = 0; j < 4; ++j) { v[j] = (e)lo[j]; v[4 + j] = (e)hi[j]; }
+      return __builtin_bit_cast(u32x4, v);
+    };
+    const int rp = tid >> 3, ch = tid & 7, r = 2 * rp, c = 8 * ch;
+    u32x4 a = {0, 0, 0, 0}, b = {0, 0, 0, 0};
+    if (c0 + c < cols) {
+      if (r0 + r < rows) a = row8(r0 + r, c0 + c);
+      if (r0 + r + 1 < rows) b = row8(r0 + r + 1, c0 + c);
+    }
+#pragma unroll
+    for (int j = 0; j < 4; ++j) {
+      tile[(c + 2 * j) * PITCH + rp] = (a[j] & 0xffffu) | (b[j] << 16);
+      tile[(c + 2 * j + 1) * PITCH + rp] = (a[j] >> 16) | (b[j] & 0xffff0000u);
+    }
+  } else {
+    for (int i = tid; i < TS * 16; i += 256) {
+      const int r = i >> 4, c = 4 * (i & 15);
+      u32x4 a = {0, 0, 0, 0};
+      if (r0 + r < rows && c0 + c < cols) a = __builtin_bit_cast(u32x4, sum4(r0 + r, c0 + c));
+      tile[(c + 0) * PITCH + r] = a[0]; tile[(c + 1) * PITCH + r] = a[1]; tile[(c + 2) * PITCH + r] = a[2]; tile[(c + 3) * PITCH + r] = a[3];
+    }
+  }
+  __syncthreads();
+  transpose_tile_store<ESZ>(tile, static_cast<char*>(out_), rows, cols, ld_out, r0, c0);
 }
 
 template <int N> using Int = std::integral_constant<int, N>;
@@ -1222,3 +1310,45 @@
   }
   return DTA_LAUNCH_STATUS();
 }
+
+extern "C" int dta_sum_slabs_transposed(const float* part, int64_t slabs, int64_t rows, int64_t cols, int64_t slab_stride, const float* extra,
+                                        void* out, int64_t ld_out, int32_t out_dtype, void* stream) {
+  if (!part || !out || slabs <= 0 || rows <= 0 || cols <= 0 || ld_out < rows) return DTA_EINVAL;
+  if (rows > (int64_t)1 << 31 || cols > (int64_t)1 << 31 || slab_stride < rows * cols) return DTA_EINVAL;
+  if (!row_dtype_ok(out_dtype)) return DTA_EUNSUPPORTED;
+  const int V = out_dtype == DTA_F32 ? 4 : 8;
+  if (slabs > 16 || rows % V || cols % V || ld_out % V || slab_stride % 4) return DTA_EUNSUPPORTED;
+  if (!aligned16(part) || !aligned16(out) || (extra && !aligned16(extra))) return DTA_EALIGN;
+  hipStream_t st_ = static_cast<hipStream_t>(stream);
+  DTA_REFUSE_IF_PRIOR_ERROR();
+  const dim3 grid((unsigned)((cols + 63) / 64), (unsigned)((rows + 63) / 64)), block(256);
+  if (grid.y > 65535) return DTA_EUNSUPPORTED;
+  dta_storage_type(out_dtype, [&](auto dt) {
+    hipLaunchKernelGGL(sum_slabs_transposed_kernel<decltype(dt)::value>, grid, block, 0, st_, part, (int)slabs, rows, cols, slab_stride, extra, out, ld_out);
+  });
+  return DTA_LAUNCH_STATUS();
+}
+
+static inline int64_t layout_job_tiles(const DtaLayoutJob& j) { return ((j.rows + 63) / 64) * ((j.cols + 63) / 64); }
+
+extern "C" int dta_layout_batch(const DtaLayoutJob* jobs_host, const DtaLayoutJob* jobs_dev, int32_t n_jobs, void* stream) {
+  if (n_jobs < 0 || (n_jobs > 0 && (!jobs_host || !jobs_dev))) return DTA_EINVAL;
+  int64_t tiles = 0;
+  for (int32_t i = 0; i < n_jobs; ++i) {
+    const DtaLayoutJob& j = jobs_host[i];
+    if (j.kind != DTA_LAYOUT_COPY && j.kind != DTA_LAYOUT_TRANSPOSE) return DTA_EINVAL;
+    if (!j.src || !j.dst || j.rows <= 0 || j.cols <= 0 || j.rows > (int64_t)1 << 31 || j.cols > (int64_t)1 << 31) return DTA_EINVAL;
+    if (j.ld_src < j.cols || j.ld_dst < (j.kind == DTA_LAYOUT_TRANSPOSE ? j.rows : j.cols) || j.tile0 != tiles) return DTA_EINVAL;
+    if (j.elem_size != 2 && j.elem_size != 4) return DTA_EUNSUPPORTED;
+    const int V = 16 / j.elem_size;
+    if (j.rows % V || j.cols % V || j.ld_src % V || j.ld_dst % V) return DTA_EUNSUPPORTED;
+    if (!aligned16(j.src) || !aligned16(j.dst)) return DTA_EALIGN;
+    tiles += layout_job_tiles(j);
+    if (tiles > 0x7fffffff) return DTA_EUNSUPPORTED;
+  }
+  hipStream_t st_ = static_cast<hipStream_t>(stream);
+  DTA_REFUSE_IF_PRIOR_ERROR();
+  if (n_jobs == 0) return DTA_OK;
+  hipLaunchKernelGGL(layout_batch_kernel, dim3((unsigned)tiles), dim3(256), 0, st_, jobs_dev, (int)n_jobs);
+  return DTA_LAUNCH_STATUS();
+}
diff --git a/dynamictreeattn_amd/dense.py b/dynamictreeattn_amd/dense.py
--- a/dynamictreeattn_amd/dense.py
+++ b/dynamictreeattn_amd/dense.py
@@ -5,7 +5,7 @@
 import torch
 
 from . import ops
-from .model import ensure_supported, final_softcap_of, head_weight, is_longrope, logit_scale_of, longrope_boundary, packed_hidden_states
+from .model import ensure_supported, final_softcap_of, head_weight, is_longrope, logit_scale_of, longrope_boundary, packed_hidden_states, weight_layouts
 from .tree_training_engine import packed_logprob_entropy
 
 
@@ -23,6 +23,7 @@
     out = []
     ensure_supported(model)
     with ops.weight_cache():
+        ops.prefill_weight_layouts(*weight_layouts(model))
         for ids in token_seqs:
             lp, _ = _one(model, ids.to(model.device), False, False)
             out.append(lp[1:])
@@ -33,6 +34,8 @@
     total = 0.0
     ensure_supported(model)
     with ops.weight_cache():
+        longest = max((int(ids.numel()) for ids in token_seqs), default=0)
+        ops.prefill_weight_layouts(*weight_layouts(model, longest))
         for ids, att in zip(token_seqs, attachs):
             lp, ent = _one(model, ids.to(model.device), True, act_ckpt)
             loss = loss_fn(lp[1:], ent, att)
diff --git a/dynamictreeattn_amd/model.py b/dynamictreeattn_amd/model.py
--- a/dynamictreeattn_amd/model.py
+++ b/dynamictreeattn_amd/model.py
@@ -439,6 +439,24 @@
     return ops.lora_linear(x, w, bias, adapters)
 
 
+def _split_projections(layer):
+    a, m = layer.self_attn, layer.mlp
+    groups = [(a.q_proj, a.k_proj, a.v_proj), (a.o_proj,)]
+    if hasattr(m, "gate_proj"):
+        groups += [(m.gate_proj, m.up_proj), (m.down_proj,)]
+    return groups
+
+
+def _phi3_projections(layer):
+    a, m = layer.self_attn, layer.mlp
+    return [(a.qkv_proj,), (a.o_proj,), (m.gate_up_proj,), (m.down_proj,)]
+
+
+def _glm4_projections(layer):
+    a, m = layer.self_attn, layer.mlp
+    return [(a.q_proj, a.k_proj, a.v_proj), (a.o_proj,), (m.gate_up_proj,), (m.down_proj,)]
+
+
 def _gemma2_layer_forward(layer, res, delta, cos_sin, attn, Hq, Hkv, D, eps):
     T = res.shape[0]
     a, m = layer.self_attn, layer.mlp
@@ -526,6 +544,33 @@
     return res, _project(act, m.down_proj)
 
 
+def _layer_forward_of(c):
+    return (_gemma2_layer_forward if is_gemma2(c) else _olmo_layer_forward if is_olmo(c) else _phi3_layer_forward if is_phi3(c)
+            else _glm4_layer_forward if is_glm4(c) else _cohere_layer_forward if is_cohere(c) else _layer_forward)
+
+
+def _projections_of(c):
+    return _phi3_projections if is_phi3(c) else _glm4_projections if is_glm4(c) else _split_projections
+
+
+def weight_layouts(model, rows: int = 0, head: torch.Tensor = None, head_rows: int = 0):
+    stacks, transposes = [], []
+    projections = _projections_of(model.config)
+    for layer in model.model.layers:
+        for mods in projections(layer):
+            bases, ads = zip(*(lora.resolve(m_) for m_ in mods))
+            if any(a_ is not None for a_ in ads):
+                continue
+            ws = tuple(b_.weight for b_ in bases)
+            if len(ws) > 1:
+                stacks.append(ws)
+            if rows > 0 and all(ops.dgrad_transposed(rows, w) for w in ws):
+                transposes.append(ws if len(ws) > 1 else ws[0])
+    if head is not None and rows > 0 and ops.dgrad_transposed(head_rows, head):
+        transposes.append(head)
+    return stacks, transposes
+
+
 class _ScaleRows(torch.autograd.Function):
 
     @staticmethod
@@ -587,8 +632,7 @@
     body = model.model
     gemma = is_gemma2(model.config)
     cohere = is_cohere(model.config)
-    layer_fwd = (_gemma2_layer_forward if gemma else _olmo_layer_forward if is_olmo(model.config) else _phi3_layer_forward if is_phi3(model.config)
-                 else _glm4_layer_forward if is_glm4(model.config) else _cohere_layer_forward if cohere else _layer_forward)
+    layer_fwd = _layer_forward_of(model.config)
     R = rotary_dim(model.config) if is_phi3(model.config) or is_glm4(model.config) else D
     akw = attn_args_of(model)
     res = embed(tokens) if embed is not None else F.embedding(tokens, body.embed_tokens.weight)
diff --git a/dynamictreeattn_amd/ops.py b/dynamictreeattn_amd/ops.py
--- a/dynamictreeattn_amd/ops.py
+++ b/dynamictreeattn_amd/ops.py
@@ -436,7 +436,7 @@
             logprob_entropy_bwd_raw(logits, next_loc[a:b], lse[a:b], ent[a:b] if ctx.want_entropy else None, g_next[a:b],
                                     g_ent[a:b] if ctx.want_entropy else None, ctx.temperature,
                                     xp[a:b + 1] if ctx.has_forks else None, fork_loc if ctx.has_forks else None, g_fork, softcap=ctx.softcap)
-            if W.dtype in (torch.bfloat16, torch.float16) and (b - a) >= 4096 and W.shape[0] % 8 == 0 and W.shape[1] % 8 == 0:
+            if dgrad_transposed(b - a, W):
                 torch.mm(logits, _TransposedWeights.get(W).t(), out=dh[a:b])
             else:
                 torch.mm(logits, W, out=dh[a:b])
@@ -988,11 +988,16 @@
     CACHE_BYTES = 8 << 30
     _cache: dict = {}
     _cached_bytes = 0
+    member_copies = 0
+
+    @staticmethod
+    def _key(ws):
+        return tuple((id(w), w.data_ptr(), w._version) for w in ws)
 
     @staticmethod
     def _fused(ws):
         rows = [w.shape[0] for w in ws]
-        key = tuple((id(w), w.data_ptr(), w._version) for w in ws)
+        key = _StackRows._key(ws)
         if weight_cache.depth > 0:
             hit = _StackRows._cache.get(key)
             if hit is not None:
@@ -1001,6 +1006,7 @@
         o = 0
         for w, r in zip(ws, rows):
             out[o:o + r].copy_(w); o += r
+        _StackRows.member_copies += len(ws)
         nbytes = out.numel() * out.element_size()
         if weight_cache.depth > 0 and _StackRows._cached_bytes + nbytes <= _StackRows.CACHE_BYTES:
             _StackRows._cache[key] = out; _StackRows._cached_bytes += nbytes
@@ -1027,16 +1033,24 @@
     _StackRows._cache.clear(); _StackRows._cached_bytes = 0
 
 
-def sum_slabs(part: torch.Tensor, out_dtype: torch.dtype, extra: torch.Tensor = None) -> torch.Tensor:
+def sum_slabs(part: torch.Tensor, out_dtype: torch.dtype, extra: torch.Tensor = None, transposed: bool = False) -> torch.Tensor:
     assert part.dtype == torch.float32 and part.is_contiguous() and (extra is None or (extra.dtype == torch.float32 and extra.is_contiguous()))
     S, n = part.shape[0], part[0].numel()
     assert extra is None or extra.numel() == n
+    if transposed:
+        return transpose_2d(part, out_dtype, extra)
     out = torch.empty(part.shape[1:], dtype=out_dtype, device=part.device)
     _launch("dta_sum_slabs", (part, extra, out), ptr(part), S, n, n, ptr(extra), ptr(out), _DT[out_dtype], nbytes=(S + (extra is not None)) * n * 4)
     return out
 
 
-def transpose_2d(w: torch.Tensor) -> torch.Tensor:
+def transpose_2d(w: torch.Tensor, summed_to: torch.dtype = None, extra: torch.Tensor = None) -> torch.Tensor:
+    if summed_to is not None:
+        S, R, C = w.shape
+        out = torch.empty((C, R), dtype=summed_to, device=w.device)
+        _launch("dta_sum_slabs_transposed", (w, extra, out), ptr(w), S, R, C, R * C, ptr(extra), ptr(out), R, _DT[summed_to],
+                nbytes=(S + (extra is not None)) * R * C * 4 + R * C * out.element_size())
+        return out
     R, C = w.shape
     if w.stride(1) != 1:
         w = w.contiguous()
@@ -1050,10 +1064,14 @@
     nbytes = 0
 
     @staticmethod
+    def _key(w: torch.Tensor):
+        return (w.data_ptr(), tuple(w.shape), tuple(w.stride()), w.dtype, w._version)
+
+    @staticmethod
     def get(w: torch.Tensor) -> torch.Tensor:
         if weight_cache.depth == 0:
             return transpose_2d(w)
-        key = (w.data_ptr(), tuple(w.shape), tuple(w.stride()), w.dtype, w._version)
+        key = _TransposedWeights._key(w)
         hit = _TransposedWeights.cache.get(key)
         if hit is not None:
             return hit
@@ -1064,18 +1082,118 @@
         return wt
 
 
+LAYOUT_COPY, LAYOUT_TRANSPOSE = 0, 1
+LAYOUT_TILE = 64
+
+
+def layout_table(jobs) -> np.ndarray:
+    tab = np.zeros((len(jobs), 8), np.int64)
+    tiles = 0
+    for i, (kind, src, ld_src, dst, ld_dst, rows, cols, esz) in enumerate(jobs):
+        tab[i] = (src, dst, ld_src, ld_dst, rows, cols, int(kind) | (int(esz) << 32), tiles)
+        tiles += -(-rows // LAYOUT_TILE) * -(-cols // LAYOUT_TILE)
+    return tab
+
+
+def layout_job_of_tile(tab: np.ndarray, tile: int):
+    j = int(np.searchsorted(tab[:, 7], tile, side="right")) - 1
+    tx = -(-int(tab[j, 5]) // LAYOUT_TILE)
+    t = tile - int(tab[j, 7])
+    return j, t // tx, t % tx
+
+
+def layout_batch(jobs, device) -> None:
+    from ._staging import upload
+    tab = layout_table(jobs)
+    dev_tab, = upload([tab.reshape(-1)], device, np.int64)
+    _launch("dta_layout_batch", (dev_tab,), tab.ctypes.data if len(jobs) else None, ptr(dev_tab) if len(jobs) else None, len(jobs),
+            nbytes=2 * sum(j[5] * j[6] * j[7] for j in jobs))
+
+
+PREFILL_WEIGHT_LAYOUTS = True
+
+
+def prefill_weight_layouts(stacks=(), transposes=()) -> int:
+    if not PREFILL_WEIGHT_LAYOUTS or weight_cache.depth == 0:
+        return 0
+    dev = None
+
+    def eligible(w):
+        nonlocal dev
+        if not (isinstance(w, torch.Tensor) and w.is_cuda and w.dim() == 2 and w.requires_grad and w.dtype in (torch.bfloat16, torch.float16)):
+            return False
+        if dev is None:
+            dev = w.device
+        return (w.device == dev and w.stride(1) == 1 and w.shape[0] % 8 == 0 and w.shape[1] % 8 == 0 and w.stride(0) % 8 == 0
+                and w.stride(0) >= w.shape[1] and w.data_ptr() % 16 == 0)
+
+    def group_ok(ws):
+        return len(ws) > 1 and all(eligible(w) for w in ws) and all(w.shape[1] == ws[0].shape[1] and w.dtype == ws[0].dtype for w in ws)
+
+    jobs, fused, new_stacks, new_transposes = [], {}, [], []
+    stack_bytes, transposed_bytes = _StackRows._cached_bytes, _TransposedWeights.nbytes
+    for ws in stacks:
+        ws = tuple(ws)
+        if not group_ok(ws):
+            continue
+        key = _StackRows._key(ws)
+        if key in fused or key in _StackRows._cache:
+            fused.setdefault(key, _StackRows._cache.get(key))
+            continue
+        R, C, esz = sum(w.shape[0] for w in ws), ws[0].shape[1], ws[0].element_size()
+        if stack_bytes + R * C * esz > _StackRows.CACHE_BYTES:
+            continue
+        out = torch.empty((R, C), dtype=ws[0].dtype, device=dev)
+        o = 0
+        for w in ws:
+            jobs.append((LAYOUT_COPY, w.data_ptr(), w.stride(0), out.data_ptr() + o * C * esz, C, w.shape[0], C, esz)); o += w.shape[0]
+        fused[key] = out; new_stacks.append((key, out)); stack_bytes += R * C * esz
+    for item in transposes:
+        if isinstance(item, torch.Tensor):
+            if not eligible(item):
+                continue
+            ws, whole = (item,), item
+        else:
+            ws = tuple(item)
+            whole = fused.get(_StackRows._key(ws)) if group_ok(ws) else None
+            if whole is None:
+                continue
+        key = _TransposedWeights._key(whole)
+        R, C, esz = whole.shape[0], whole.shape[1], whole.element_size()
+        if key in _TransposedWeights.cache or any(k == key for k, _ in new_transposes) or transposed_bytes + R * C * esz > _StackRows.CACHE_BYTES:
+            continue
+        wt = torch.empty((C, R), dtype=whole.dtype, device=dev)
+        o = 0
+        for w in ws:
+            jobs.append((LAYOUT_TRANSPOSE, w.data_ptr(), w.stride(0), wt.data_ptr() + o * esz, R, w.shape[0], C, esz)); o += w.shape[0]
+        new_transposes.append((key, wt)); transposed_bytes += R * C * esz
+    if jobs:
+        layout_batch(jobs, dev)
+        _StackRows._cache.update(new_stacks); _StackRows._cached_bytes = stack_bytes
+        _TransposedWeights.cache.update(new_transposes); _TransposedWeights.nbytes = transposed_bytes
+    return len(jobs)
+
+
 def clear_weight_caches() -> None:
     clear_stack_rows_cache()
     _TransposedWeights.cache.clear(); _TransposedWeights.nbytes = 0
 
 
+DGRAD_TRANSPOSED_MIN_ROWS = 4096
+
+
+def dgrad_transposed(rows: int, w: torch.Tensor) -> bool:
+    return w.is_cuda and w.dtype in (torch.bfloat16, torch.float16) and rows >= DGRAD_TRANSPOSED_MIN_ROWS and w.shape[0] % 8 == 0 and w.shape[1] % 8 == 0
+
+
 def _dgrad(dy: torch.Tensor, w: torch.Tensor) -> torch.Tensor:
-    if dy.is_cuda and w.dtype in (torch.bfloat16, torch.float16) and dy.shape[0] >= 4096 and w.shape[0] % 8 == 0 and w.shape[1] % 8 == 0:
+    if dy.is_cuda and dgrad_transposed(dy.shape[0], w):
         return dy @ _TransposedWeights.get(w).t()
     return dy @ w
 
 
 WGRAD_SPLIT_K = 4
+WGRAD_SPLIT_MIN_ROWS = 2048
 
 
 def _wgrad(x: torch.Tensor, dy: torch.Tensor, transposed: bool) -> torch.Tensor:
@@ -1084,17 +1202,20 @@
     S = WGRAD_SPLIT_K
     tiles = -(-a.shape[1] // 256) * -(-b.shape[1] // 256)
     per = (T // S) // 64 * 64
-    if tiles > 64 or per < 2048 or not x.is_cuda or x.dtype == torch.float32:
+    V = 16 // x.element_size()
+    vec = x.is_cuda and a.shape[1] % V == 0 and b.shape[1] % V == 0
+    if tiles > 64 or per < WGRAD_SPLIT_MIN_ROWS or not x.is_cuda or x.dtype == torch.float32:
         out = a.t() @ b
     else:
         body = per * S
         part = torch.bmm(a[:body].reshape(S, per, a.shape[1]).transpose(1, 2), b[:body].reshape(S, per, b.shape[1]), out_dtype=torch.float32)
         rest = torch.mm(a[body:].t(), b[body:], out_dtype=torch.float32) if body < T else None
+        if transposed and vec:
+            return sum_slabs(part, x.dtype, rest, transposed=True)
         out = sum_slabs(part, x.dtype, rest)
     if not transposed:
         return out
-    V = 16 // out.element_size()
-    return transpose_2d(out) if out.is_cuda and out.shape[0] % V == 0 and out.shape[1] % V == 0 else out.t()
+    return transpose_2d(out) if vec else out.t()
 
 
 class _Linear(torch.autograd.Function):
diff --git a/dynamictreeattn_amd/tree_training_engine.py b/dynamictreeattn_amd/tree_training_engine.py
--- a/dynamictreeattn_amd/tree_training_engine.py
+++ b/dynamictreeattn_amd/tree_training_engine.py
@@ -8,7 +8,7 @@
 from . import ops, packing
 from .losses import PREFERENCE_STATS, STATS as LOSS_STATS, PolicyLoss, PreferenceLoss
 from .model import (_head_dim, ensure_supported, final_softcap_of, head_weight, is_cohere, is_gemma2, is_glm4, is_longrope, is_moe_layer, logit_scale_of, moe_geometry,
-                    longrope_boundary, packed_hidden_states)
+                    longrope_boundary, packed_hidden_states, weight_layouts)
 from .trie import pop_block_starts
 
 __all__ = ["TreeTrainingEngine", "_get_forkpos", "packed_logprob_entropy"]
@@ -33,15 +33,21 @@
     return fc, fp, ptr
 
 
+def head_shard(W: torch.Tensor, tp_group):
+    if tp_group is None:
+        return W, 0
+    import torch.distributed as dist
+    tp, rk = dist.get_world_size(tp_group), dist.get_rank(tp_group)
+    Vp = W.shape[0] // tp
+    assert Vp * tp == W.shape[0], "vocabulary must divide by the tensor-parallel size"
+    return W[rk * Vp:(rk + 1) * Vp], rk * Vp
+
+
 def head_call_args(W: torch.Tensor, tp_group, softcap: float, logit_scale: float, pick_rows):
     kw = {}
     if tp_group is not None:
-        import torch.distributed as dist
-        tp, rk = dist.get_world_size(tp_group), dist.get_rank(tp_group)
-        Vp = W.shape[0] // tp
-        assert Vp * tp == W.shape[0], "vocabulary must divide by the tensor-parallel size"
-        W = W[rk * Vp:(rk + 1) * Vp]
-        kw.update(tp_group=tp_group, vocab_offset=rk * Vp)
+        W, offset = head_shard(W, tp_group)
+        kw.update(tp_group=tp_group, vocab_offset=offset)
     if softcap:
         kw.update(softcap=softcap, max_picks_per_row=int(np.bincount(pick_rows).max()) if len(pick_rows) else 0)
     if logit_scale != 1.0:
@@ -441,6 +447,7 @@
         if token_trie.n_sequences == 0:
             return self.returns
         with ops.weight_cache():
+            ops.prefill_weight_layouts(*weight_layouts(model))
             return self._forward(model, token_trie)
 
     def _forward(self, model, token_trie):
@@ -479,11 +486,14 @@
         if rows is not None:
             longest = max(token_trie.lens)
             assert longest <= self.max_seq_len, f"Exceeds max_seq_len: cur_len=0, new_tokens={longest}, max={self.max_seq_len}"
+            ops.prefill_weight_layouts(*weight_layouts(model, rows))
             if isinstance(loss_fn, PreferenceLoss):
                 return self._backward_stack_two_pass(model, token_trie, loss_fn, rows)
             return self._backward_stack(model, token_trie, loss_fn, rows)
         packed = self._pack(token_trie)
         chunk = min(self.head_chunk, block_size) if block_size else self.head_chunk
+        ops.prefill_weight_layouts(*weight_layouts(model, packed.plan.T, head_shard(head_weight(model), self.tp_group)[0],
+                                                   min(max(chunk, 1), packed.plan.T)))
         ckpt = self._should_checkpoint(model, packed.plan.T)
         self.last_mode = "packed+recompute" if ckpt else "packed"
         attn_keep = self._attn_keep_bytes() if ckpt else 0
diff --git a/include/dta.h b/include/dta.h
--- a/include/dta.h
+++ b/include/dta.h
@@ -117,6 +117,20 @@
 
 int dta_sum_slabs(const float* part, int64_t slabs, int64_t n, int64_t slab_stride, const float* extra, void* out, int32_t out_dtype, void* stream);
 
+int dta_sum_slabs_transposed(const float* part, int64_t slabs, int64_t rows, int64_t cols, int64_t slab_stride, const float* extra,
+                             void* out, int64_t ld_out, int32_t out_dtype, void* stream);
+
+enum { DTA_LAYOUT_COPY = 0, DTA_LAYOUT_TRANSPOSE = 1 };
+typedef struct DtaLayoutJob {
+  const void* src;
+  void* dst;
+  int64_t ld_src, ld_dst;
+  int64_t rows, cols;
+  int32_t kind, elem_size;
+  int64_t tile0;
+} DtaLayoutJob;
+int dta_layout_batch(const DtaLayoutJob* jobs_host, const DtaLayoutJob* jobs_dev, int32_t n_jobs, void* stream);
+
 #define DTA_MOE_BM 128
 #define DTA_MOE_FWD 0
 #define DTA_MOE_DGRAD 1
```

Result: no change. 855,700 (-0.1%).
